# TaceoLabs/collaborative-circom

Hardware: AMD Instinct MI355X
Metric: Groth16 constraints/sec (BN254, 2^22 R1CS), one REP3 party's prove (higher is better)
Workload: dtype u32; 1 GPU; synthetic R1CS 2^22 constraints-domain BN254, REP3 co-groth16 (configs[2]); num_constraints=4194302, domain_size=4194304, nnz=12582906, msm=8 G1 + 2 G2 of ~2^22 points, ntt=12

## Files before the change

### collaborative-circom_amd/csrc/capi.hip

```cpp
#include "capi_internal.hpp"


template <int OP>
int32_t vec_binary(cg_ctx* ctx, int32_t curve, void* d_out, const void* d_a, const void* d_b, size_t n) {
    if (!ctx || !d_out || !d_a || !d_b) return fail(CG_ERR_ARG, "null argument");
    HIPCHK(hipSetDevice(ctx->device));
    return with_fr(curve, [&](auto tag) -> int {
        typedef decltype(tag) Fr;
        StatScope ss(ctx, TAG_VEC);
        return launch_vec_binary<Fr>(ctx->stream, OP, (Fr*)d_out, (const Fr*)d_a, (const Fr*)d_b, n);
    });
}

template <class F> struct CurveB;
template <> struct CurveB<Bn254Fq> { static Bn254Fq get() { Bn254Fq t = Bn254Fq::one(); return t + t + t; } };
template <> struct CurveB<Fp2<Bn254Fq>> { static Fp2<Bn254Fq> get() {
    Bn254Fq one = Bn254Fq::one(), three = one + one + one, nine = three + three + three;
    Fp2<Bn254Fq> xi = {nine, one}; Fp2<Bn254Fq> inv = fp_inverse(xi); return {inv.c0 * three, inv.c1 * three}; } };
#if CG_WITH_BLS
template <> struct CurveB<Bls381Fq> { static Bls381Fq get() { Bls381Fq t = Bls381Fq::one(); t = t + t; return t + t; } };
template <> struct CurveB<Fp2<Bls381Fq>> { static Fp2<Bls381Fq> get() { Bls381Fq f = CurveB<Bls381Fq>::get(); return {f, f}; } };
#endif

namespace {
// ... 124 lines not shown
}
int32_t cg_bases_release(cg_bases* b) {
    if (!b) return 0;
    hipSetDevice(b->device);
    hipDeviceSynchronize();
    hipFree(b->d_pts);
    if (b->d_pre) hipFree(b->d_pre);
    if (b->d_live) hipFree(b->d_live);
    if (b->compact) { hipFree(b->compact->d_pts); if (b->compact->d_pre) hipFree(b->compact->d_pre); delete b->compact; }
    delete b;
    return 0;
}
int32_t cg_bases_check_on_curve(cg_ctx* ctx, const cg_bases* b, uint64_t* n_bad, uint64_t* first_bad) {
    if (!ctx || !b || !n_bad) return fail(CG_ERR_ARG, "null argument");
    if (b->device != ctx->device) return fail(CG_ERR_ARG, "bases live on another device");
    HIPCHK(hipSetDevice(ctx->device));
    return with_group(b->curve, b->group, [&](auto ftag, auto) -> int {
        typedef decltype(ftag) F;
        unsigned long long* d = nullptr; unsigned long long h[2] = {0ull, ~0ull};
        HIPCHK(hip_malloc_flush((void**)&d, 16));
        HIPCHK(hipMemcpyAsync(d, h, 16, hipMemcpyHostToDevice, ctx->stream));
        int rc = check_on_curve_launch<F>(ctx->stream, (const Affine<F>*)b->d_pts, b->n, CurveB<F>::get(), d);
        if (rc) return rc;
        HIPCHK(hipMemcpyAsync(h, d, 16, hipMemcpyDeviceToHost, ctx->stream));
        HIPCHK(hipStreamSynchronize(ctx->stream));
        HIPCHK(hipFree(d));
        *n_bad = h[0]; if (first_bad) *first_bad = h[1];
        return 0;
    });
}
int32_t cg_bases_check_subgroup(cg_ctx* ctx, const cg_bases* b, uint64_t* n_bad, uint64_t* first_bad) {
    if (!ctx || !b || !n_bad) return fail(CG_ERR_ARG, "null argument");
    if (b->device != ctx->device) return fail(CG_ERR_ARG, "bases live on another device");
    *n_bad = 0; if (first_bad) *first_bad = ~0ull;
    if (b->curve == CG_BN254 && b->group == CG_G1) return 0;
    HIPCHK(hipSetDevice(ctx->device));
    return with_group(b->curve, b->group, [&](auto ftag, auto frtag) -> int {
        typedef decltype(ftag) F; typedef decltype(frtag) Fr;
        unsigned long long* d = nullptr; unsigned long long h[2] = {0ull, ~0ull};
        HIPCHK(hip_malloc_flush((void**)&d, 16));
        HIPCHK(hipMemcpyAsync(d, h, 16, hipMemcpyHostToDevice, ctx->stream));
        const FastSubgroup<F>* fast = fast_subgroup<F>();
        int rc = fast ? check_subgroup_fast_launch<F>(ctx->stream, (const Affine<F>*)b->d_pts, b->n, *fast, d)
                      : check_subgroup_launch<F, Fr>(ctx->stream, (const Affine<F>*)b->d_pts, b->n, d);
        if (rc) return rc;
        HIPCHK(hipMemcpyAsync(h, d, 16, hipMemcpyDeviceToHost, ctx->stream));
        HIPCHK(hipStreamSynchronize(ctx->stream));
        HIPCHK(hipFree(d));
        *n_bad = h[0]; if (first_bad) *first_bad = h[1];
        return 0;
    });
}
int32_t cg_bases_precompute(cg_ctx* ctx, cg_bases* b, int32_t c) {
    if (!ctx || !b) return fail(CG_ERR_ARG, "null argument");
    if (b->compact) return cg_bases_precompute(ctx, b->compact, c);
    const bool auto_window = c == 0;
    if (c == 0) c = b->n > ((size_t)3 << (b->group == CG_G1 ? 20 : 19)) ? 20 : (b->n <= ((size_t)1 << 18) ? 16 : 17);
    if (c < 8 || c > 22) return fail(CG_ERR_ARG, "precompute window must be 0 (auto) or in [8, 22]");
    if (b->device != ctx->device) return fail(CG_ERR_ARG, "bases live on another device");
    if (b->n > ((size_t)1 << 24)) return fail(CG_ERR_ARG, "precomputed tables support at most 2^24 points");
    HIPCHK(hipSetDevice(ctx->device));
    if (b->d_pre) { HIPCHK(hipStreamSynchronize(ctx->stream)); HIPCHK(hipFree(b->d_pre)); b->d_pre = nullptr; b->pre_c = b->pre_nwin = 0; }
    return with_group(b->curve, b->group, [&](auto ftag, auto frtag) -> int {
        typedef decltype(ftag) F; typedef decltype(frtag) Fr;
        const int nwin = Fr::Params::BITS / c + 1;
        const size_t n = std::max<size_t>(b->n, 1);
        const hipError_t e_pre = hip_malloc_flush(&b->d_pre, (size_t)nwin * n * sizeof(Affine<F>));
        if (e_pre == hipErrorOutOfMemory && auto_window) {
            (void)hipGetLastError(); b->d_pre = nullptr;
            return 0;
        }
        HIPCHK(e_pre);
        Affine<F>* tab = (Affine<F>*)b->d_pre;
        HIPCHK(hipMemcpyAsync(tab, b->d_pts, b->n * sizeof(Affine<F>), hipMemcpyDeviceToDevice, ctx->stream));
        for (int j = 1; j < nwin; j++) { int rc = precompute_window_launch<F>(ctx->stream, tab + (size_t)(j - 1) * b->n, tab + (size_t)j * b->n, b->n, c); if (rc) return rc; }
        HIPCHK(hipStreamSynchronize(ctx->stream));
        b->pre_c = c; b->pre_nwin = nwin;
        return 0;
    });
}
size_t cg_bases_len(const cg_bases* b) { return b ? b->n : 0; }

int32_t cg_bases_synth_multiples(cg_ctx* ctx, int32_t curve, int32_t group, uint64_t first, size_t n, cg_bases** out) {
    if (!ctx || !out) return fail(CG_ERR_ARG, "null argument");
    HIPCHK(hipSetDevice(ctx->device));
    return with_group(curve, group, [&](auto ftag, auto) -> int {
        typedef decltype(ftag) F;
        const uint32_t* src = curve == CG_BN254 ? (group == CG_G1 ? Bn254G1_GEN : Bn254G2_GEN) : (group == CG_G1 ? Bls381G1_GEN : Bls381G2_GEN);
        Affine<F> ga; memcpy(&ga, src, sizeof ga);
        const XYZZ<F> G = XYZZ<F>::from_affine(ga);
        int log_t = 0; while (((size_t)1 << (2 * log_t)) < n) log_t++;
        const size_t T = (size_t)1 << log_t, H = std::max<size_t>(1, (n + T - 1) >> log_t);
        std::vector<XYZZ<F>> lo(T), hi(H);
        uint32_t k[2] = {(uint32_t)first, (uint32_t)(first >> 32)};
        XYZZ<F> acc = xyzz_scalar_mul(G, k, 2);
        for (size_t j = 0; j < T; j++) { lo[j] = acc; acc = xyzz_add(acc, G); }
        uint32_t kt[2] = {(uint32_t)T, (uint32_t)((uint64_t)T >> 32)};
        const XYZZ<F> step = xyzz_scalar_mul(G, kt, 2);
        acc = XYZZ<F>::infinity();
        for (size_t j = 0; j < H; j++) { hi[j] = acc; acc = xyzz_add(acc, step); }
        XYZZ<F>*d_lo = nullptr, *d_hi = nullptr;
        HIPCHK(hip_malloc_flush((void**)&d_lo, T * sizeof(XYZZ<F>))); HIPCHK(hip_malloc_flush((void**)&d_hi, H * sizeof(XYZZ<F>)));
        HIPCHK(hipMemcpy(d_lo, lo.data(), T * sizeof(XYZZ<F>), hipMemcpyHostToDevice));
        HIPCHK(hipMemcpy(d_hi, hi.data(), H * sizeof(XYZZ<F>), hipMemcpyHostToDevice));
        cg_bases* b = new cg_bases{ctx->device, curve, group, n, sizeof(Affine<F>), nullptr};
        b->no_inf = first >= 1 && first + n > first;
        HIPCHK(hip_malloc_flush(&b->d_pts, std::max<size_t>(n * sizeof(Affine<F>), 16)));
        int rc = synth_points_launch<F>(ctx->stream, d_lo, d_hi, log_t, n, (Affine<F>*)b->d_pts);
        if (rc) return rc;
        HIPCHK(hipStreamSynchronize(ctx->stream));
        HIPCHK(hipFree(d_lo)); HIPCHK(hipFree(d_hi));
        *out = b;
        return 0;
    });
}
int32_t cg_bases_from_scalars(cg_ctx* ctx, int32_t curve, int32_t group, const void* d_scalars, size_t n, cg_bases** out) {
    if (!ctx || !out || (!d_scalars && n)) return fail(CG_ERR_ARG, "null argument");
    HIPCHK(hipSetDevice(ctx->device));
    return with_group(curve, group, [&](auto ftag, auto frtag) -> int {
        typedef decltype(ftag) F; typedef decltype(frtag) Fr;
        const uint32_t* src = curve == CG_BN254 ? (group == CG_G1 ? Bn254G1_GEN : Bn254G2_GEN) : (group == CG_G1 ? Bls381G1_GEN : Bls381G2_GEN);
        Affine<F> ga; memcpy(&ga, src, sizeof ga);
        const int nwin = (Fr::Params::BITS + 7) / 8;
        Affine<F>* d_tab = nullptr;
        HIPCHK(hip_malloc_flush((void**)&d_tab, (size_t)nwin * 255 * sizeof(Affine<F>)));
        cg_bases* b = new cg_bases{ctx->device, curve, group, n, sizeof(Affine<F>), nullptr};
        hipError_t e = hip_malloc_flush(&b->d_pts, std::max<size_t>(n * sizeof(Affine<F>), 16));
        if (e != hipSuccess) { hipFree(d_tab); delete b; return fail(CG_ERR_OOM, "cg_bases_from_scalars: out of device memory"); }
        int rc = fixed_base_mul_launch<F, Fr>(ctx->stream, ga, (const Fr*)d_scalars, n, d_tab, (Affine<F>*)b->d_pts);
        hipError_t e2 = hipStreamSynchronize(ctx->stream);
        hipFree(d_tab);
        if (rc || e2 != hipSuccess) { hipFree(b->d_pts); delete b; return rc ? rc : fail(CG_ERR_HIP, std::string("cg_bases_from_scalars: ") + hipGetErrorString(e2)); }
        *out = b;
        return 0;
    });
}
int32_t cg_bases_download(cg_ctx* ctx, const cg_bases* bases, size_t offset, size_t n, void* h_out_packed) {
    if (!ctx || !bases || !h_out_packed) return fail(CG_ERR_ARG, "null argument");
    if (offset + n > bases->n) return fail(CG_ERR_ARG, "slice out of range");
    HIPCHK(hipMemcpyAsync(h_out_packed, (const char*)bases->d_pts + offset * bases->pt_bytes, n * bases->pt_bytes, hipMemcpyDeviceToHost, ctx->stream));
    HIPCHK(hipStreamSynchronize(ctx->stream));
    return 0;
}

int32_t cg_ctx_set_option(cg_ctx* ctx, int32_t option, int64_t value) {
    if (!ctx) return fail(CG_ERR_ARG, "null ctx");
    switch (option) {
        case CG_OPT_MSM_CHUNK: return cg_msm_set_chunk(ctx, (int32_t)value);
        case CG_OPT_MSM_WINDOW: return cg_msm_set_window(ctx, (int32_t)value);
        case CG_OPT_MSM_SCATTER_CAP: return cg_msm_set_scatter_capacity(ctx, (int32_t)value);
        case CG_OPT_MSM_TABLE_ORDER: if (value < 0 || value > 2) break; ctx->table_order = (int)value; return 0;
        case CG_OPT_MSM_G2_AFTER: if (value < -1 || value > 64) break; ctx->g2_after = (int)value; return 0;
        case CG_OPT_MSM_G2_SLICES: if (value < 0 || value > 1) break; ctx->g2_slices = (int)value; return 0;
        case CG_OPT_MSM_REDUCE_BATCH: if (value < 0 || value > 3) break; ctx->red_batch = (int)value; return 0;
        case CG_OPT_MSM_ACC_SLOTS: if (value < 2 || value > cg_ctx::ACC_SLOTS_MAX) break; ctx->acc_slots = (int)value; return 0;
        case CG_OPT_MSM_WIDE_SMALL: if (value < 0 || value > 30 || (value > 1 && value < 10)) break; ctx->wide_small = (int)value; return 0;
        case CG_OPT_MSM_ONE_STREAM_LOG: if (value < 0 || value > 30) break; ctx->one_stream_log = (int)value; return 0;
        case CG_OPT_MSM_OFF_MAIN_LOG: if (value < 0 || value > 30) break; ctx->off_main_log = (int)value; return 0;
        case CG_OPT_MSM_SOLO_LOG: if (value < 0 || value > 30) break; ctx->solo_log = (int)value; return 0;
        default: return fail(CG_ERR_ARG, "cg_ctx_set_option: unknown option");
    }
    return fail(CG_ERR_ARG, "cg_ctx_set_option: value out of range");
}
int32_t cg_ctx_get_option(const cg_ctx* ctx, int32_t option, int64_t* value) {
    if (!ctx || !value) return fail(CG_ERR_ARG, "null argument");
    switch (option) {
        case CG_OPT_MSM_CHUNK: *value = ctx->msm_chunk; return 0;
        case CG_OPT_MSM_WINDOW: *value = ctx->msm_window; return 0;
        case CG_OPT_MSM_SCATTER_CAP: *value = ctx->scatter_cap; return 0;
        case CG_OPT_MSM_TABLE_ORDER: *value = ctx->table_order; return 0;
        case CG_OPT_MSM_G2_AFTER: *value = ctx->g2_after; return 0;
        case CG_OPT_MSM_G2_SLICES: *value = ctx->g2_slices; return 0;
        case CG_OPT_MSM_REDUCE_BATCH: *value = ctx->red_batch; return 0;
        case CG_OPT_MSM_ACC_SLOTS: *value = ctx->acc_slots; return 0;
        case CG_OPT_MSM_WIDE_SMALL: *value = ctx->wide_small; return 0;
        case CG_OPT_MSM_ONE_STREAM_LOG: *value = ctx->one_stream_log; return 0;
        case CG_OPT_MSM_OFF_MAIN_LOG: *value = ctx->off_main_log; return 0;
        case CG_OPT_MSM_SOLO_LOG: *value = ctx->solo_log; return 0;
        default: return fail(CG_ERR_ARG, "cg_ctx_get_option: unknown option");
    }
}
int32_t cg_set_option(int32_t option, int64_t value) {
    if (option < 1 || option >= CG_GOPT_COUNT) return fail(CG_ERR_ARG, "cg_set_option: unknown option");
    if (value < 0 || (option != CG_GOPT_COMPACT_MIN_LOG && value > 1) || value > 64) return fail(CG_ERR_ARG, "cg_set_option: value out of range");
    g_options.v[option].store(value); return 0;
}
int32_t cg_get_option(int32_t option, int64_t* value) {
    if (option < 1 || option >= CG_GOPT_COUNT || !value) return fail(CG_ERR_ARG, "cg_get_option: unknown option");
    *value = g_options.v[option].load(); return 0;
}
int32_t cg_vec_add_dev(cg_ctx* ctx, int32_t curve, void* o, const void* a, const void* b, size_t n) { return vec_binary<0>(ctx, curve, o, a, b, n); }
int32_t cg_vec_sub_dev(cg_ctx* ctx, int32_t curve, void* o, const void* a, const void* b, size_t n) { return vec_binary<1>(ctx, curve, o, a, b, n); }
int32_t cg_vec_mul_dev(cg_ctx* ctx, int32_t curve, void* o, const void* a, const void* b, size_t n) { return vec_binary<2>(ctx, curve, o, a, b, n); }

int32_t cg_vec_rep3_mul_local_dev(cg_ctx* ctx, int32_t curve, void* d_out, const void* d_aa, const void* d_ab, const void* d_ba, const void* d_bb, const void* d_mask, size_t n) {
    if (!ctx || !d_out || !d_aa || !d_ab || !d_ba || !d_bb) return fail(CG_ERR_ARG, "null argument");
    HIPCHK(hipSetDevice(ctx->device));
    return with_fr(curve, [&](auto tag) -> int {
        typedef decltype(tag) Fr;
        StatScope ss(ctx, TAG_VEC);
        return launch_rep3_mul_local<Fr>(ctx->stream, (Fr*)d_out, (const Fr*)d_aa, (const Fr*)d_ab, (const Fr*)d_ba, (const Fr*)d_bb, (const Fr*)d_mask, n);
    });
}
static int rand_draw_begin(cg_ctx* ctx, int32_t curve, const uint8_t* seed32, uint64_t word_pos, size_t n, void* d_out, double margin, int* slot_out) {
    int slot = -1;
    for (int i = 0; i < cg_ctx::RAND_DRAWS; i++) if (!ctx->rand_draw[i].live) { slot = i; break; }
    if (slot < 0) return fail(CG_ERR_ARG, "cg_chacha12_fr_rand_dev_begin: too many draws in flight (finish one first)");
    if (!ctx->rand_result) HIPCHK(hipHostMalloc((void**)&ctx->rand_result, sizeof(unsigned long long) * 2 * cg_ctx::RAND_DRAWS, hipHostMallocDefault));
    cg_ctx::RandDraw& d = ctx->rand_draw[slot];
    if (!d.ev) HIPCHK(hipEventCreateWithFlags(&d.ev, hipEventDisableTiming));
    return with_fr(curve, [&](auto tag) -> int {
        typedef decltype(tag) Fr;
        typedef typename Fr::Params P;
        StatScope ss(ctx, TAG_VEC);
        uint32_t key[8];
        for (int i = 0; i < 8; i++) key[i] = (uint32_t)seed32[4 * i] | (uint32_t)seed32[4 * i + 1] << 8 | (uint32_t)seed32[4 * i + 2] << 16 | (uint32_t)seed32[4 * i + 3] << 24;
        const double accept = (double)P::P[7] / (double)(1ull << (P::BITS - 224));
        const uint64_t n_cand = (uint64_t)(((double)n + margin) / accept) + 2;
        const uint64_t n_pairs = n_cand / 2 + 2;
        const uint64_t tiles = (n_pairs + 255) / 256;
        d.d_cand = d.d_small = nullptr;
        if (int rc = cg_dev_alloc(ctx, n_pairs * 64, &d.d_cand)) return rc;
        if (int rc = cg_dev_alloc(ctx, tiles * 4 + 16, &d.d_small)) { cg_dev_free(ctx, d.d_cand); return rc; }
        unsigned long long* h = ctx->rand_result + 2 * slot; h[0] = h[1] = 0;
        int rc = chacha12_fr_rand_launch(ctx->stream, key, P::P, P::BITS, word_pos, n_pairs, n, d.d_cand, (uint32_t*)((char*)d.d_small + 16), (unsigned long long*)d.d_small, d_out);
        hipError_t e = rc ? hipSuccess : hipMemcpyAsync(h, d.d_small, 2 * sizeof(unsigned long long), hipMemcpyDeviceToHost, ctx->stream);
        if (!rc && e == hipSuccess) e = hipEventRecord(d.ev, ctx->stream);
        if (rc || e != hipSuccess) { hipStreamSynchronize(ctx->stream); cg_dev_free(ctx, d.d_cand); cg_dev_free(ctx, d.d_small); if (rc) return rc; HIPCHK(e); }
        d.live = true; d.word_pos = word_pos; d.n = n;
        *slot_out = slot;
        return 0;
    });
}
static int rand_draw_finish(cg_ctx* ctx, int slot, bool* enough, uint64_t* word_pos_after) {
    cg_ctx::RandDraw& d = ctx->rand_draw[slot];
    hipError_t e = hipEventSynchronize(d.ev);
    { void* two[2] = {d.d_cand, d.d_small}; cg_dev_free_many(ctx, two, 2); }
    d.live = false;
    HIPCHK(e);
    const unsigned long long* h = ctx->rand_result + 2 * slot;
    *enough = h[0] >= d.n;
    if (*enough && word_pos_after) *word_pos_after = d.word_pos + 8 * ((uint64_t)h[1] + 1);
    return 0;
}
static int rand_draw_args(cg_ctx* ctx, const uint8_t* seed32, uint64_t word_pos, size_t n, void* d_out, const char* who) {
    if (!ctx || !seed32 || (n && !d_out)) return fail(CG_ERR_ARG, "null argument");
    if (n >= ((size_t)1 << 31) || word_pos > (~0ull >> 1)) return fail(CG_ERR_ARG, std::string(who) + ": size or position out of range");
    return 0;
}
int32_t cg_chacha12_fr_rand_dev(cg_ctx* ctx, int32_t curve, const uint8_t* seed32, uint64_t word_pos, size_t n, void* d_out, uint64_t* word_pos_after) {
    if (int rc = rand_draw_args(ctx, seed32, word_pos, n, d_out, "cg_chacha12_fr_rand_dev")) return rc;
    if (n == 0) { if (word_pos_after) *word_pos_after = word_pos; return 0; }
    HIPCHK(hipSetDevice(ctx->device));
    double margin = 8.0 * std::sqrt((double)n) + 64.0;
    for (int attempt = 0; attempt < 4; attempt++, margin *= 4.0) {
        int slot = -1; bool enough = false;
        if (int rc = rand_draw_begin(ctx, curve, seed32, word_pos, n, d_out, margin, &slot)) return rc;
        if (int rc = rand_draw_finish(ctx, slot, &enough, word_pos_after)) return rc;
        if (enough) return 0;
    }
    return fail(CG_ERR_HIP, "cg_chacha12_fr_rand_dev: too few accepted candidates");
}
int32_t cg_chacha12_fr_rand_dev_begin(cg_ctx* ctx, int32_t curve, const uint8_t* seed32, uint64_t word_pos, size_t n, void* d_out, int32_t* ticket) {
    if (!ticket) return fail(CG_ERR_ARG, "null argument");
    if (int rc = rand_draw_args(ctx, seed32, word_pos, n, d_out, "cg_chacha12_fr_rand_dev_begin")) return rc;
    if (n == 0) return fail(CG_ERR_ARG, "cg_chacha12_fr_rand_dev_begin: nothing to draw");
    HIPCHK(hipSetDevice(ctx->device));
    int slot = -1;
    if (int rc = rand_draw_begin(ctx, curve, seed32, word_pos, n, d_out, 12.0 * std::sqrt((double)n) + 64.0, &slot)) return rc;
    *ticket = slot;
    return 0;
}
int32_t cg_chacha12_fr_rand_dev_finish(cg_ctx* ctx, int32_t ticket, uint64_t* word_pos_after) {
    if (!ctx) return fail(CG_ERR_ARG, "null argument");
    if (ticket < 0 || ticket >= cg_ctx::RAND_DRAWS || !ctx->rand_draw[ticket].live) return fail(CG_ERR_ARG, "cg_chacha12_fr_rand_dev_finish: no such draw in flight");
    HIPCHK(hipSetDevice(ctx->device));
    bool enough = false;
    if (int rc = rand_draw_finish(ctx, ticket, &enough, word_pos_after)) return rc;
    if (!enough) return fail(CG_ERR_HIP, "cg_chacha12_fr_rand_dev_finish: too few accepted candidates (d_out is incomplete: draw again with cg_chacha12_fr_rand_dev)");
    return 0;
}
int32_t cg_vec_check_canonical_dev(cg_ctx* ctx, int32_t curve, const void* d_vec, size_t n, void* d_count) {
    if (!ctx || !d_vec || !d_count) return fail(CG_ERR_ARG, "null argument");
    HIPCHK(hipSetDevice(ctx->device));
    return with_fr(curve, [&](auto tag) -> int {
        typedef decltype(tag) Fr;
        StatScope ss(ctx, TAG_VEC);
        return launch_vec_count_noncanonical<Fr>(ctx->stream, (const Fr*)d_vec, n, (unsigned long long*)d_count);
    });
}
int32_t cg_vec_affine_dev(cg_ctx* ctx, int32_t curve, void* d_out, const void* d_a, size_t n, const void* h_c, const void* h_d) {
    if (!ctx || !d_out || !d_a || !h_c) return fail(CG_ERR_ARG, "null argument");
    HIPCHK(hipSetDevice(ctx->device));
    return with_fr(curve, [&](auto tag) -> int {
        typedef decltype(tag) Fr;
        Fr c, d = Fr::zero(); copy_in(c, h_c); if (h_d) copy_in(d, h_d);
        StatScope ss(ctx, TAG_VEC);
        return launch_vec_affine<Fr>(ctx->stream, (Fr*)d_out, (const Fr*)d_a, n, c, d);
    });
}
int32_t cg_vec_fill_dev(cg_ctx* ctx, int32_t curve, void* d_v, size_t n, const void* h_value) {
    if (!ctx || !d_v || !h_value) return fail(CG_ERR_ARG, "null argument");
    HIPCHK(hipSetDevice(ctx->device));
    return with_fr(curve, [&](auto tag) -> int {
        typedef decltype(tag) Fr;
        Fr v; copy_in(v, h_value);
        StatScope ss(ctx, TAG_VEC);
// ... 570 lines not shown
```

### collaborative-circom_amd/csrc/capi_msm.hip

```cpp
#include "capi_internal.hpp"

namespace {
int auto_window(size_t n, int bits) {
    const int lg = log2_floor(std::max<size_t>(n, 1));
    int c = lg <= 12 ? 8 : lg == 13 ? 13 : lg <= 18 ? 15 : 16;
    auto ok = [&](int w) { const int t = bits % w; return t != 0 && t >= w - 3 - (w >= 13 ? 6 : 0); };
    if (!ok(c)) for (int d : {1, -1, 2, -2, 3, -3}) { if (c + d >= 3 && c + d <= 17 && ok(c + d)) { c += d; break; } }
    return c;
}

template <class F>
Jacobian<F> msm_fold_windows(const XYZZ<F>* w, int nwin, int c) {
    XYZZ<F> acc = w[nwin - 1];
    for (int i = nwin - 2; i >= 0; i--) {
        for (int d = 0; d < c; d++) acc = xyzz_dbl(acc);
        acc = xyzz_add(acc, w[i]);
    }
    return xyzz_to_jacobian(acc);
}

int ticket_slot(cg_ctx* ctx) {
    for (size_t i = 0; i < ctx->tickets.size(); i++) if (!ctx->tickets[i].live) return (int)i;
    ctx->tickets.emplace_back();
    return (int)ctx->tickets.size() - 1;
// ... 10 lines not shown
int msm_begin_multi_impl_(cg_ctx* ctx, int nb, const cg_bases* const* bases, const size_t* offsets, size_t n, const void* const* d_scalars, int k, int* tickets_out, bool force_exact) {
    const uint32_t chunk_request = ctx ? ctx->msm_chunk : 0;
    if (!ctx || !bases || !tickets_out || (n && !d_scalars)) return fail(CG_ERR_ARG, "null argument");
    if (nb < 1 || nb > 16) return fail(CG_ERR_ARG, "number of base tables out of range");
    if (k < 1 || k > 8) return fail(CG_ERR_ARG, "k out of range");
    for (int b = 0; b < nb; b++) {
        if (!bases[b]) return fail(CG_ERR_ARG, "null bases");
        if ((offsets ? offsets[b] : 0) + n > bases[b]->n) return fail(CG_ERR_ARG, "bases slice out of range");
        if (bases[b]->device != ctx->device) return fail(CG_ERR_ARG, "bases live on another device");
        if (bases[b]->curve != bases[0]->curve) return fail(CG_ERR_ARG, "all tables of one call must be on the same curve");
    }
    HIPCHK(hipSetDevice(ctx->device));
    {
        bool any = false;
        for (int b = 0; b < nb; b++) any = any || bases[b]->compact != nullptr;
        if (any) {
            struct Grp { uint64_t sig; size_t off, cnt, caller_off; std::vector<int> members; };
            std::vector<Grp> groups;
            std::vector<size_t> off_c(nb), cnt_c(nb);
            for (int b = 0; b < nb; b++) {
                const size_t off = offsets ? offsets[b] : 0;
                uint64_t sig = 0; size_t o = off, cn = n;
                if (bases[b]->compact) {
                    const auto& lv = bases[b]->h_live;
                    o = (size_t)(std::lower_bound(lv.begin(), lv.end(), (uint32_t)off) - lv.begin());
                    cn = (size_t)(std::lower_bound(lv.begin(), lv.end(), (uint32_t)std::min<size_t>(off + n, 0xffffffffu)) - lv.begin()) - o;
                    sig = bases[b]->live_sig;
                }
                off_c[b] = o; cnt_c[b] = cn;
                bool placed = false;
                for (auto& g : groups) {
                    if (g.sig != sig || g.cnt != cn) continue;
                    if (sig != 0) {
                        if (g.off != o || g.caller_off != off) continue;
                        const auto& la = bases[g.members[0]]->h_live; const auto& lb = bases[b]->h_live;
                        if (memcmp(la.data() + o, lb.data() + o, cn * sizeof(uint32_t)) != 0) continue;
                    }
                    g.members.push_back(b); placed = true; break;
                }
                if (!placed) groups.push_back(Grp{sig, o, cn, off, {b}});
            }
            size_t need = 0;
            for (auto& g : groups) if (g.sig) need += align_up((size_t)k * g.cnt * 32);
            if (need > ctx->gather_cap) {
                HIPCHK(hipStreamSynchronize(ctx->stream)); HIPCHK(hipStreamSynchronize(ctx->sortst));
                if (ctx->gather_buf) HIPCHK(hipFree(ctx->gather_buf));
                ctx->gather_buf = nullptr; ctx->gather_cap = 0;
                HIPCHK(hip_malloc_flush(&ctx->gather_buf, need)); ctx->gather_cap = need;
            }
            if (ctx->sorts_unordered) { for (int j = 0; j < 2; j++) HIPCHK(hipStreamWaitEvent(ctx->stream, ctx->ev_sorted[j], 0)); ctx->sorts_unordered = false; }
            size_t used = 0;
            for (auto& g : groups) {
                std::vector<const cg_bases*> gb; std::vector<size_t> go; std::vector<const void*> gs(k);
                const int first = g.members[0];
                for (int m : g.members) { gb.push_back(bases[m]->compact ? bases[m]->compact : bases[m]); go.push_back(bases[m]->compact ? off_c[m] : (offsets ? offsets[m] : 0)); }
                if (g.sig) {
                    const size_t off = offsets ? offsets[first] : 0;
                    for (int j = 0; j < k; j++) {
                        void* dst = (char*)ctx->gather_buf + used + (size_t)j * g.cnt * 32;
                        int rc = with_fr(bases[first]->curve, [&](auto tag) -> int {
                            typedef decltype(tag) Fr;
                            return launch_vec_gather_idx<Fr>(ctx->stream, (Fr*)dst, (const Fr*)d_scalars[j], bases[first]->d_live + g.off, g.cnt, (uint32_t)off);
                        });
                        if (rc) return rc;
                        gs[j] = dst;
                    }
                    used += align_up((size_t)k * g.cnt * 32);
                } else for (int j = 0; j < k; j++) gs[j] = d_scalars[j];
                std::vector<int> tk(g.members.size());
                int rc = msm_begin_multi_impl(ctx, (int)g.members.size(), gb.data(), go.data(), g.cnt, gs.data(), k, tk.data(), true);
                if (rc) return rc;
                for (size_t i = 0; i < g.members.size(); i++) tickets_out[g.members[i]] = tk[i];
            }
            return 0;
        }
    }
    {
        bool mixed = false;
        for (int b = 1; b < nb; b++) mixed = mixed || bases[b]->pre_c != bases[0]->pre_c;
        if (mixed) {
            std::vector<char> done(nb, 0);
            for (int b = 0; b < nb; b++) {
                if (done[b]) continue;
                std::vector<const cg_bases*> gb; std::vector<size_t> go; std::vector<int> idx;
                for (int m = b; m < nb; m++) if (!done[m] && bases[m]->pre_c == bases[b]->pre_c) { gb.push_back(bases[m]); go.push_back(offsets ? offsets[m] : 0); idx.push_back(m); done[m] = 1; }
                std::vector<int> tk(idx.size());
                int rc = msm_begin_multi_impl(ctx, (int)idx.size(), gb.data(), go.data(), n, d_scalars, k, tk.data(), force_exact);
                if (rc) return rc;
                for (size_t i = 0; i < idx.size(); i++) tickets_out[idx[i]] = tk[i];
            }
            return 0;
        }
    }
    const int curve = bases[0]->curve;
    const bool shared = bases[0]->pre_c != 0;
    if (shared && n > ((size_t)1 << 24)) return fail(CG_ERR_ARG, "precomputed-table MSM supports at most 2^24 points per call");
    int bits = 0;
    { int rc = with_fr(curve, [&](auto tag) -> int { bits = decltype(tag)::Params::BITS; return 0; }); if (rc) return rc; }
    const int c = shared ? bases[0]->pre_c : (n ? (ctx->msm_window ? ctx->msm_window : auto_window(n, bits)) : 2);
    const int nwin = bits / c + 1;
    if (shared && nwin != bases[0]->pre_nwin) return fail(CG_ERR_ARG, "internal: window count mismatch");
    if ((uint64_t)nwin * n >= ((uint64_t)1 << 32))
        return fail(CG_ERR_ARG, "MSM of more than 2^32 / windows points in one call (about 2^27): pass the table in slices and add the partial sums");
    uint32_t cap = 0;
    if (n && !force_exact && ctx->scatter_cap >= 0) {
        if (ctx->scatter_cap > 0) cap = (uint32_t)ctx->scatter_cap;
        else {
            const int t = bits % c;
            const double nbk = (double)((size_t)1 << (c - 1));
            const double top = t == 0 ? (double)n : (double)n / (double)((size_t)1 << std::min(c - 1, t));
            const double avg = shared ? (double)(nwin - 1) * (double)n / nbk + top : std::max((double)n / nbk, top);
            const double want = 1.25 * avg + 6.0 * std::sqrt(avg) + 16.0;
            if (want <= 4096.0) { cap = 16; while ((double)cap < want) cap <<= 1; }
        }
    }
    const MsmGeom geom = msm_geom(std::max<size_t>(n, 1), c, nwin, shared, 0, chunk_request);
    const int nsums = geom.ngroups;
    std::vector<int> slots(nb);
    size_t acc_bytes = 0;
    for (int b = 0; b < nb; b++) {
        slots[b] = ticket_slot(ctx);
        MsmTicket& t = ctx->tickets[slots[b]];
        t.live = true;
        t.curve = curve; t.group = bases[b]->group; t.k = k; t.c = c; t.nwin = nwin; t.nsums = nsums; t.plain_fold = shared && !geom.bitsum && !geom.grid; t.bit_fold = geom.bitsum;
        t.grid_fold = geom.grid; t.log_l = geom.log_l; t.log_h = geom.log_h; t.gc = geom.gc; t.gr = geom.gr;
        t.optimistic = cap != 0; t.bases = bases[b]; t.offset = offsets ? offsets[b] : 0; t.n = n; t.scalars.assign(d_scalars, d_scalars + (n ? k : 0));
        if (!t.h_flags) HIPCHK(hipHostMalloc((void**)&t.h_flags, 8 * sizeof(uint32_t), hipHostMallocDefault));
        for (int i = 0; i < 8; i++) t.h_flags[i] = 0;
        int rc = with_coord_field(curve, t.group, [&](auto ftag) -> int {
            typedef decltype(ftag) F;
            const size_t need = (size_t)k * nsums * sizeof(XYZZ<F>);
            if (t.pinned_bytes < need) {
                if (t.h_pinned) HIPCHK(hipHostFree(t.h_pinned));
                t.h_pinned = nullptr; t.pinned_bytes = 0;
                HIPCHK(hipHostMalloc(&t.h_pinned, need, hipHostMallocDefault));
                t.pinned_bytes = need;
            }
            if (n == 0) { XYZZ<F>* h = (XYZZ<F>*)t.h_pinned; for (int i = 0; i < k * nsums; i++) h[i] = XYZZ<F>::infinity(); }
            else acc_bytes = std::max(acc_bytes, msm_acc_scratch_bytes<F>(n, c, nwin, shared, chunk_request));
            return 0;
        });
        if (rc) return rc;
        if (!t.done) HIPCHK(hipEventCreateWithFlags(&t.done, hipEventDisableTiming));
    }
    if (n) {
        StatScope ss(ctx, TAG_MSM);
        const size_t sort_bytes = align_up(cap ? msm_sort_direct_scratch_bytes(n, c, nwin, shared ? 1 : 0, cap) : msm_sort_scratch_bytes(n, c, nwin));
        const size_t acc_slot = align_up(acc_bytes);
        const int nsched = k > 1 ? 2 : 1;
        const int acc_slots_min = std::min((int)cg_ctx::ACC_SLOTS_MAX, std::max(2, ctx->acc_slots));
        const int red_batch = ctx->red_batch;
        const uint64_t wide_max = ctx->wide_small == 0 ? 0 : (uint64_t)1 << (ctx->wide_small == 1 ? 20 : ctx->wide_small);
        const bool small_call = k <= 2 && (uint64_t)nwin * n <= wide_max;
        bool single_field = true;
        for (int b = 1; b < nb; b++) single_field = single_field && bases[b]->group == bases[0]->group;
        const int acc_slots = red_batch || small_call ? std::min((int)cg_ctx::ACC_SLOTS_MAX, std::max(acc_slots_min, red_batch >= 2 || small_call ? nb * k : nb + 1)) : acc_slots_min;
        const bool wide = k <= 2 && nb * k <= std::min(acc_slots, (int)ACC_MAX_SETS) && (uint64_t)nwin * n <= wide_max;
        const bool solo = wide && small_call && single_field && ctx->solo_log > 0 && (uint64_t)nwin * n <= ((uint64_t)1 << ctx->solo_log);
        const bool one_stream = solo || (small_call && ctx->one_stream_log > 0 && (uint64_t)nwin * n <= ((uint64_t)1 << ctx->one_stream_log));
        const hipStream_t sortst = one_stream ? ctx->stream : ctx->sortst, auxst = one_stream ? ctx->stream : ctx->aux;
        { int rc = solo ? ensure_main_stream_block(ctx, ctx->solo_arena, nsched * sort_bytes + (size_t)acc_slots * acc_slot) : ensure_arena(ctx, nsched * sort_bytes + (size_t)acc_slots * acc_slot); if (rc) return rc; }
        char* const arena_base = solo ? ctx->solo_arena.base : ctx->arena.base;
        char* acc_scratch = arena_base + nsched * sort_bytes;
        if (!solo) {
        HIPCHK(hipEventRecord(ctx->ev_in, ctx->stream));
        HIPCHK(hipStreamWaitEvent(sortst, ctx->ev_in, 0));
        for (int rs = 0; rs < 2; rs++) for (int i = 0; i < 2; i++) if (ctx->merged_pending[rs][i]) { HIPCHK(hipStreamWaitEvent(sortst, ctx->ev_merged[rs][i], 0)); ctx->merged_pending[rs][i] = false; }
        }
        std::vector<MsmSortPtrs> sps(k);
        auto launch_sort = [&](int j) -> int {
            const int ss_ = j % nsched;
            if (j < 4 && ctx->comp_after[j]) HIPCHK(hipStreamWaitEvent(sortst, ctx->comp_after[j], 0));
            if (j >= nsched && !solo) {
                HIPCHK(hipStreamWaitEvent(sortst, ctx->ev_sched_free[ss_], 0));
                for (int rs = 0; rs < 2; rs++) if (ctx->merged_pending[rs][ss_]) HIPCHK(hipStreamWaitEvent(sortst, ctx->ev_merged[rs][ss_], 0));
            }
            hipEvent_t evs[2]; hipEvent_t* pev = nullptr;
            if (ctx->stats_on) { const int i0 = ev_open(ctx, TAG_SORT); evs[0] = ctx->ev_live[i0].a; evs[1] = ctx->ev_live[i0].b; pev = evs; }
            char* sort_scratch = arena_base + (size_t)ss_ * sort_bytes;
            int rc = with_fr(curve, [&](auto tag) -> int {
                typedef decltype(tag) Fr;
                return cap ? msm_sort_direct_launch<Fr>(sortst, (const Fr*)d_scalars[j], n, c, nwin, shared ? 1 : 0, cap, sort_scratch, sort_bytes, &sps[j], pev)
                           : msm_sort_launch<Fr>(sortst, (const Fr*)d_scalars[j], n, c, nwin, shared ? 1 : 0, sort_scratch, sort_bytes, &sps[j], pev);
            });
            if (rc) return rc;
            if (cap) for (int b = 0; b < nb; b++) HIPCHK(hipMemcpyAsync(ctx->tickets[slots[b]].h_flags + j, sps[j].overflow, 4, hipMemcpyDeviceToHost, sortst));
            if (!solo) HIPCHK(hipEventRecord(ctx->ev_sorted[ss_], sortst));
            return 0;
        };
        int iter = 0;
        { int rc = launch_sort(0); if (rc) return rc; }
        struct PendSet { MsmRedSet set; int slot, sched, table, comp; };
        std::vector<PendSet> pend[2];
        int tables_of_group[2] = {0, 0};
        for (int b = 0; b < nb; b++) tables_of_group[bases[b]->group == CG_G1 ? 0 : 1]++;
        std::vector<int> comps_left(nb, k);
        hipStream_t red_stream[2] = {auxst, auxst};
        hipStream_t acc_stream[2] = {ctx->stream, ctx->stream};
        hipEvent_t last_acc[2] = {nullptr, nullptr};
        auto flush = [&](int gi) -> int {
            std::vector<PendSet>& pd = pend[gi];
            if (pd.empty()) return 0;
            hipStream_t rst = red_stream[gi];
            hipEvent_t ea = ctx->ev_acc[pd.back().slot];
            if (!solo) {
                HIPCHK(hipEventRecord(ea, acc_stream[gi]));
                if (rst != acc_stream[gi]) HIPCHK(hipStreamWaitEvent(rst, ea, 0));
                last_acc[gi] = ea;
            }
            hipEvent_t evs[2]; hipEvent_t* pev = nullptr;
            if (ctx->stats_on) { const int i2 = ev_open(ctx, TAG_REDUCE); evs[0] = ctx->ev_live[i2].a; evs[1] = ctx->ev_live[i2].b; pev = evs; }
            hipEvent_t evm[2]; int nm = 0; bool seen[2] = {false, false};
            std::vector<MsmRedSet> sets;
            const int rs = rst == sortst ? 1 : 0;
            for (const PendSet& ps : pd) { sets.push_back(ps.set); if (!solo && !seen[ps.sched]) { seen[ps.sched] = true; evm[nm++] = ctx->ev_merged[rs][ps.sched]; } }
            int rc = with_coord_field(curve, gi == 0 ? CG_G1 : CG_G2, [&](auto ftag) -> int {
                typedef decltype(ftag) F;
                return msm_reduce_batch<F>(rst, sets.data(), (int)sets.size(), n, c, nwin, shared, sps[pd[0].comp].cap, evm, nm, pev, chunk_request);
            });
            if (rc) return rc;
            if (!solo) for (const PendSet& ps : pd) {
                HIPCHK(hipEventRecord(ctx->ev_red[ps.slot], rst));
                ctx->slot_busy[ps.slot] = true; ctx->aux_pending = true; ctx->last_slot = ps.slot; ctx->merged_pending[rs][ps.sched] = true;
            }
            for (const PendSet& ps : pd) if (--comps_left[ps.table] == 0) HIPCHK(hipEventRecord(ctx->tickets[slots[ps.table]].done, rst));
            pd.clear();
            return 0;
        };
        auto acc_set = [&](int b, int j, char* scratch) -> MsmAccSet {
            const char* pts = (const char*)(shared ? bases[b]->d_pre : bases[b]->d_pts) + (offsets ? offsets[b] : 0) * bases[b]->pt_bytes;
            return MsmAccSet{pts, shared ? bases[b]->n : 0, sps[j].sorted, sps[j].offsets, sps[j].counts, scratch, !bases[b]->no_inf};
        };
        auto red_set = [&](int b, int j, char* scratch) -> MsmRedSet {
            const MsmTicket& t = ctx->tickets[slots[b]];
            const size_t pinned_stride = (size_t)(t.group == CG_G1 ? 4 : 8) * (bases[b]->pt_bytes / (t.group == CG_G1 ? 2 : 4));
            return MsmRedSet{scratch, sps[j].offsets, sps[j].counts, (char*)t.h_pinned + (size_t)j * nsums * pinned_stride};
        };
        const bool off_main = wide && !one_stream && ctx->off_main_log > 0 && (uint64_t)nwin * n <= ((uint64_t)1 << ctx->off_main_log);
        if (wide) {
            if (k == 2) { int rc = launch_sort(1); if (rc) return rc; }
            if (off_main) { acc_stream[0] = sortst; acc_stream[1] = auxst; }
            if (!solo) for (int j = 0; j < k; j++) HIPCHK(hipStreamWaitEvent(acc_stream[1], ctx->ev_sorted[j], 0));
            red_stream[0] = sortst;
            for (int gi : {1, 0}) {
                std::vector<MsmAccSet> sets;
                for (int j = 0; j < k; j++) for (int b = 0; b < nb; b++) {
                    if ((bases[b]->group == CG_G1 ? 0 : 1) != gi) continue;
                    const int slot = iter++ % acc_slots;
                    if (!solo && ctx->slot_busy[slot]) HIPCHK(hipStreamWaitEvent(acc_stream[gi], ctx->ev_red[slot], 0));
                    char* scratch = acc_scratch + (size_t)slot * acc_slot;
                    sets.push_back(acc_set(b, j, scratch));
                    pend[gi].push_back(PendSet{red_set(b, j, scratch), slot, j, b, j});
                }
                if (sets.empty()) continue;
                hipEvent_t evs[2]; hipEvent_t* pev = nullptr;
                if (ctx->stats_on) { const int i1 = ev_open(ctx, gi == 0 ? TAG_ACC_G1 : TAG_ACC_G2); evs[0] = ctx->ev_live[i1].a; evs[1] = ctx->ev_live[i1].b; pev = evs; }
                int rc = with_coord_field(curve, gi == 0 ? CG_G1 : CG_G2, [&](auto ftag) -> int {
                    typedef decltype(ftag) F;
                    return msm_accumulate_batch<F>(acc_stream[gi], sets.data(), (int)sets.size(), n, c, nwin, shared, sps[0].cap, pev, chunk_request, false);
                });
                if (rc) return rc;
                if (gi == 0 && !solo) HIPCHK(hipStreamWaitEvent(sortst, ctx->ev_sorted[k - 1], 0));
                { int rc2 = flush(gi); if (rc2) return rc2; }
            }
            if (off_main && last_acc[1]) HIPCHK(hipStreamWaitEvent(sortst, last_acc[1], 0));
            if (off_main) ctx->sorts_unordered = true;
            if (!solo) for (int j = 0; j < k; j++) HIPCHK(hipEventRecord(ctx->ev_sched_free[j], off_main ? sortst : ctx->stream));
        }
        auto do_acc = [&](int b, int j) -> int {
            const MsmSortPtrs& sp = sps[j];
            MsmTicket& t = ctx->tickets[slots[b]];
            const int gi = t.group == CG_G1 ? 0 : 1;
            hipEvent_t evs[2]; hipEvent_t* pev = nullptr;
            if (ctx->stats_on) { const int i1 = ev_open(ctx, t.group == CG_G1 ? TAG_ACC_G1 : TAG_ACC_G2); evs[0] = ctx->ev_live[i1].a; evs[1] = ctx->ev_live[i1].b; pev = evs; }
            const int slot = iter++ % acc_slots;
            for (int g2 = 0; g2 < 2; g2++) {
                bool held = false;
                for (const PendSet& ps : pend[g2]) held = held || ps.slot == slot;
                if (held) { int rc = flush(g2); if (rc) return rc; }
            }
            if (ctx->slot_busy[slot]) HIPCHK(hipStreamWaitEvent(ctx->stream, ctx->ev_red[slot], 0));
            char* scratch = acc_scratch + (size_t)slot * acc_slot;
            const MsmAccSet as = acc_set(b, j, scratch);
            int rc = with_coord_field(curve, t.group, [&](auto ftag) -> int {
                typedef decltype(ftag) F;
                return msm_accumulate_batch<F>(ctx->stream, &as, 1, n, c, nwin, shared, sp.cap, pev, chunk_request, ctx->g2_slices != 0);
            });
            if (rc) return rc;
            pend[gi].push_back(PendSet{red_set(b, j, scratch), slot, j % nsched, b, j});
            return 0;
        };
        if (wide) {}
        else if (k <= 2 && ctx->table_order == 2) {
            if (k == 2) { int rc = launch_sort(1); if (rc) return rc; }
            std::vector<std::pair<int, int>> g1o, g2o, order;
            for (int j = 0; j < k; j++) for (int bi = 0; bi < nb; bi++) {
                const int b = (j & 1) ? nb - 1 - bi : bi;
                (bases[b]->group == CG_G1 ? g1o : g2o).push_back({b, j});
            }
            const size_t at = ctx->g2_after < 0 ? g1o.size() : std::min<size_t>((size_t)ctx->g2_after, g1o.size());
            order.insert(order.end(), g1o.begin(), g1o.begin() + at); order.insert(order.end(), g2o.begin(), g2o.end()); order.insert(order.end(), g1o.begin() + at, g1o.end());
            bool waited[2] = {false, false};
            int left[2] = {(int)g1o.size(), (int)g2o.size()}, left_sched[2] = {0, 0};
            for (auto& pr : order) left_sched[pr.second]++;
            for (size_t i = 0; i < order.size(); i++) {
                const int b = order[i].first, j = order[i].second, gi = bases[b]->group == CG_G1 ? 0 : 1;
                if (!waited[j]) { HIPCHK(hipStreamWaitEvent(ctx->stream, ctx->ev_sorted[j], 0)); waited[j] = true; }
                { int rc = do_acc(b, j); if (rc) return rc; }
                const bool last_of_field = --left[gi] == 0;
                const bool comp_changes = i + 1 == order.size() || order[i + 1].second != j || (bases[order[i + 1].first]->group == CG_G1 ? 0 : 1) != gi;
                if (red_batch == 0 || (red_batch == 1 && comp_changes) || (last_of_field && red_batch != 3) || (int)pend[gi].size() == RED_MAX_SETS) { int rc3 = flush(gi); if (rc3) return rc3; }
                if (--left_sched[j] == 0) HIPCHK(hipEventRecord(ctx->ev_sched_free[j], ctx->stream));
            }
        } else
        for (int j = 0; j < k; j++) {
            HIPCHK(hipStreamWaitEvent(ctx->stream, ctx->ev_sorted[j % nsched], 0));
            if (j + 1 < k && nsched == 2 && j + 1 < nsched) { int rc = launch_sort(j + 1); if (rc) return rc; }
            int left_in_comp[2] = {tables_of_group[0], tables_of_group[1]};
            for (int bi = 0; bi < nb; bi++) {
                const int b = (ctx->table_order >= 1 && (j & 1)) ? nb - 1 - bi : bi;
                const int gi = bases[b]->group == CG_G1 ? 0 : 1;
                { int rc = do_acc(b, j); if (rc) return rc; }
                const bool last_here = --left_in_comp[gi] == 0;
                if (red_batch == 0 || (red_batch == 1 && last_here) || (last_here && j == k - 1 && red_batch != 3) || (int)pend[gi].size() == RED_MAX_SETS) { int rc3 = flush(gi); if (rc3) return rc3; }
            }
            HIPCHK(hipEventRecord(ctx->ev_sched_free[j % nsched], ctx->stream));
            if (j + 2 < k && nsched == 2) {
                for (int g2 = 0; g2 < 2; g2++) { int rc = flush(g2); if (rc) return rc; }
                int rc = launch_sort(j + 2); if (rc) return rc;
            }
        }
        for (int g2 = 0; g2 < 2; g2++) { int rc = flush(g2); if (rc) return rc; }
    }
    for (int b = 0; b < nb; b++) { if (n == 0) HIPCHK(hipEventRecord(ctx->tickets[slots[b]].done, ctx->stream)); tickets_out[b] = slots[b]; }
    return 0;
}

int msm_begin_impl(cg_ctx* ctx, const cg_bases* bases, size_t offset, size_t n, const void* const* d_scalars, int k, int* ticket_out) {
    if (!ticket_out) return fail(CG_ERR_ARG, "null argument");
    return msm_begin_multi_impl(ctx, 1, &bases, &offset, n, d_scalars, k, ticket_out);
}

int msm_end_impl(cg_ctx* ctx, int ticket, void* h_out);
int msm_end_impl(cg_ctx* ctx, int ticket, void* h_out) {
    if (!ctx || !h_out) return fail(CG_ERR_ARG, "null argument");
    if (ticket < 0 || ticket >= (int)ctx->tickets.size() || !ctx->tickets[ticket].live) return fail(CG_ERR_ARG, "bad MSM ticket");
    MsmTicket& t = ctx->tickets[ticket];
    HIPCHK(hipEventSynchronize(t.done));
    t.live = false;
    if (t.optimistic) {
        bool over = false;
        for (int j = 0; j < t.k; j++) over = over || t.h_flags[j] != 0;
        if (over) {
            const cg_bases* b = t.bases; const size_t off = t.offset, n = t.n; const int k = t.k;
            std::vector<const void*> sc = t.scalars;
            int t2 = -1;
            int rc = msm_begin_multi_impl(ctx, 1, &b, &off, n, sc.data(), k, &t2, true);
            if (rc) return rc;
            return msm_end_impl(ctx, t2, h_out);
        }
    }
    return with_group64(t.curve, t.group, [&](auto ftag, auto) -> int {
        typedef decltype(ftag) F;
        typedef cg64::Xyzz<F> X;
        const X* h = (const X*)t.h_pinned;
        cg64::Jac<F>* out = (cg64::Jac<F>*)h_out;
        for (int j = 0; j < t.k; j++) {
            const X* hs = h + (size_t)j * t.nsums;
            X acc;
            if (t.grid_fold) {
                std::vector<X> U((size_t)t.log_l + t.log_h + 1, X::inf());
                size_t at = 0;
                for (int kk = 0; kk <= t.log_l; kk++) for (uint32_t g = 0; g < t.gc; g++) U[kk] = cg64::add(U[kk], hs[at++]);
                for (int kk = 0; kk < t.log_h; kk++) for (uint32_t g = 0; g < t.gr; g++) U[t.log_l + kk] = cg64::add(U[t.log_l + kk], hs[at++]);
                acc = U.back();
                for (size_t i = U.size() - 1; i-- > 0;) acc = cg64::add(cg64::dbl(acc), U[i]);
            } else if (t.bit_fold) {
                acc = hs[t.nsums - 1];
                for (int i = t.nsums - 2; i >= 0; i--) acc = cg64::add(cg64::dbl(acc), hs[i]);
            } else if (t.plain_fold) { acc = hs[0]; for (int i = 1; i < t.nsums; i++) acc = cg64::add(acc, hs[i]); }
            else {
                acc = hs[t.nsums - 1];
                for (int i = t.nsums - 2; i >= 0; i--) { for (int d = 0; d < t.c; d++) acc = cg64::dbl(acc); acc = cg64::add(acc, hs[i]); }
            }
            const cg64::Jac<F> r = cg64::to_jac(acc);
            memcpy(out + j, &r, sizeof r);
        }
        return 0;
    });
}

}

extern "C" {
int32_t cg_msm_set_scatter_capacity(cg_ctx* ctx, int32_t cap) {
    if (!ctx) return fail(CG_ERR_ARG, "null ctx");
    if (cap > 65536) return fail(CG_ERR_ARG, "capacity out of range");
    ctx->scatter_cap = cap;
    return 0;
}
int32_t cg_msm_set_chunk(cg_ctx* ctx, int32_t entries_per_lane) {
    if (!ctx) return fail(CG_ERR_ARG, "null ctx");
    if (entries_per_lane < 0 || entries_per_lane > 4096) return fail(CG_ERR_ARG, "chunk length out of range");
    ctx->msm_chunk = (uint32_t)entries_per_lane;
    return 0;
}
int32_t cg_msm_set_window(cg_ctx* ctx, int32_t c) {
    if (!ctx) return fail(CG_ERR_ARG, "null ctx");
    if (c != 0 && (c < 2 || c > 20)) return fail(CG_ERR_ARG, "window size must be 0 (auto) or in [2, 20]");
    ctx->msm_window = c;
    return 0;
}
int32_t cg_msm_scalars_after(cg_ctx* ctx, int32_t component, cg_ctx* owner, int32_t copy_ticket) {
    if (!ctx || !owner || component < 0 || component >= 4) return fail(CG_ERR_ARG, "bad argument");
    if (copy_ticket < 0 || !owner->copy_ev[copy_ticket % cg_ctx::COPY_TICKETS]) return fail(CG_ERR_ARG, "bad copy ticket");
    const int slot = copy_ticket % cg_ctx::COPY_TICKETS;
    ctx->comp_after[component] = owner->copy_id[slot] == (uint32_t)copy_ticket ? owner->copy_ev[slot] : nullptr;
    return 0;
}
int32_t cg_msm_dev_begin(cg_ctx* ctx, const cg_bases* bases, size_t offset, size_t n, const void* const* d_scalars, int32_t k, int32_t* ticket) {
    const int rc = msm_begin_impl(ctx, bases, offset, n, d_scalars, k, ticket);
    if (ctx) for (hipEvent_t& e : ctx->comp_after) e = nullptr;
    return rc;
}
int32_t cg_msm_dev_begin_multi(cg_ctx* ctx, int32_t n_tables, const cg_bases* const* bases, const size_t* offsets, size_t n,
                               const void* const* d_scalars, int32_t k, int32_t* tickets) {
    const int rc = msm_begin_multi_impl(ctx, n_tables, bases, offsets, n, d_scalars, k, tickets);
    if (ctx) for (hipEvent_t& e : ctx->comp_after) e = nullptr;
    return rc;
}
int32_t cg_msm_end(cg_ctx* ctx, int32_t ticket, void* h_out_jacobian) { return msm_end_impl(ctx, ticket, h_out_jacobian); }
int32_t cg_msm_dev(cg_ctx* ctx, const cg_bases* bases, size_t offset, size_t n, const void* const* d_scalars, int32_t k, void* h_out) {
    int32_t t = -1;
    int rc = msm_begin_impl(ctx, bases, offset, n, d_scalars, k, &t);
    if (rc) return rc;
    return msm_end_impl(ctx, t, h_out);
}
int32_t cg_msm(cg_ctx* ctx, const cg_bases* bases, size_t offset, size_t n, const void* const* h_scalars, int32_t k, void* h_out) {
    if (!ctx || !bases || !h_scalars) return fail(CG_ERR_ARG, "null argument");
    if (k < 1 || k > 8) return fail(CG_ERR_ARG, "k out of range");
    HIPCHK(hipSetDevice(ctx->device));
    std::vector<void*> d(k, nullptr);
    const size_t bytes = std::max<size_t>(n * 32, 16);
    for (int j = 0; j < k; j++) {
        HIPCHK(hip_malloc_flush(&d[j], bytes));
        if (n) HIPCHK(hipMemcpyAsync(d[j], h_scalars[j], n * 32, hipMemcpyHostToDevice, ctx->stream));
    }
    int rc = cg_msm_dev(ctx, bases, offset, n, (const void* const*)d.data(), k, h_out);
    hipStreamSynchronize(ctx->stream);
    for (int j = 0; j < k; j++) hipFree(d[j]);
    return rc;
}

int32_t cg_msm_schedule_dev(cg_ctx* ctx, int32_t curve, const void* d_scalars, size_t n, int32_t c, int32_t shared, int32_t path, uint32_t cap,
                            uint32_t* h_counts, uint32_t* h_offsets, uint32_t* h_sorted, int32_t* path_taken, uint32_t* overflow) {
    if (!ctx || !d_scalars || !h_counts || !h_offsets || !h_sorted || !path_taken || !overflow) return fail(CG_ERR_ARG, "null argument");
    if (c < 2 || c > 22) return fail(CG_ERR_ARG, "cg_msm_schedule_dev: window size out of range (2 .. 22)");
    if (n == 0) return fail(CG_ERR_ARG, "cg_msm_schedule_dev: no scalars");
    if (shared < 0 || shared > 1 || path < 0 || path > CG_MSM_PATH_DIRECT) return fail(CG_ERR_ARG, "cg_msm_schedule_dev: shared is 0 or 1, path 0 .. 4");
    int bits = 0;
    { int rc = with_fr(curve, [&](auto tag) -> int { bits = decltype(tag)::Params::BITS; return 0; }); if (rc) return rc; }
    const int nwin = bits / c + 1;
    if (shared && n > ((size_t)1 << 24)) return fail(CG_ERR_ARG, "cg_msm_schedule_dev: one bucket set takes at most 2^24 points (the window shares the entry with the index)");
    if ((uint64_t)nwin * n >= ((uint64_t)1 << 32)) return fail(CG_ERR_ARG, "cg_msm_schedule_dev: schedule positions are 32-bit");
    const bool direct = path == CG_MSM_PATH_DIRECT;
    const size_t nbuckets = (size_t)(shared ? 1 : nwin) << (c - 1);
    if (direct && (cap < 1 || (uint64_t)nbuckets * cap >= ((uint64_t)1 << 32))) return fail(CG_ERR_ARG, "cg_msm_schedule_dev: the one-pass scatter takes 1 <= cap < 2^32 / buckets");
    const size_t sorted_len = direct ? nbuckets * cap : (size_t)nwin * n;
    const size_t bytes = align_up(direct ? msm_sort_direct_scratch_bytes(n, c, nwin, shared, cap) : msm_sort_scratch_bytes(n, c, nwin));
    HIPCHK(hipSetDevice(ctx->device));
    char* scratch = nullptr;
    HIPCHK(hip_malloc_flush(&scratch, bytes));
    MsmSortPtrs sp{};
    uint32_t ov = 0;
    int rc = [&]() -> int {
        HIPCHK(hipMemsetAsync(scratch, 0xFF, bytes, ctx->stream));
        int r = with_fr(curve, [&](auto tag) -> int {
// ... 21 lines not shown
```

### collaborative-circom_amd/csrc/capi_streams.hip

```cpp
#include "capi_internal.hpp"

extern "C" {
namespace {
std::mutex g_stream_pool_mu;
constexpr int HWQ = 4;
struct StreamClassPool { std::vector<std::pair<hipStream_t, int>> idle; int created = 0; int out[HWQ] = {0, 0, 0, 0}; };
std::map<std::pair<int, int>, StreamClassPool> g_stream_pool;
std::map<hipStream_t, int> g_stream_slot;
thread_local int g_group_depth = 0;
thread_local std::map<int, std::array<uint8_t, 3>> g_group_used_by_device;
#define g_group_used (g_group_used_by_device[device])
int new_stream(int cls, hipStream_t* out) {
    if (cls == 0) { HIPCHK(hipStreamCreateWithFlags(out, hipStreamNonBlocking)); return 0; }
    int prio_least = 0, prio_greatest = 0;
    HIPCHK(hipDeviceGetStreamPriorityRange(&prio_least, &prio_greatest));
    HIPCHK(hipStreamCreateWithPriority(out, hipStreamNonBlocking, cls > 0 ? prio_greatest : prio_least));
    return 0;
}
int measured_pipe(int device, int cls, hipStream_t st);
thread_local int g_group_rot = 0;
}
}
int pooled_stream(int device, int cls, hipStream_t* out, int want) {
    std::lock_guard<std::mutex> l(g_stream_pool_mu);
// ... 33 lines not shown
        }
        hipStream_t st = nullptr;
        if (int rc = new_stream(cls, &st)) return rc;
        const int model = p.created++ % HWQ, seen = measured_pipe(device, cls, st);
        const int slot = seen >= 0 ? seen : model;
        g_stream_slot[st] = slot; p.idle.push_back({st, slot});
    }
    return fail(CG_ERR_HIP, "internal: stream pool");
}
namespace {
void park_stream(int device, int cls, hipStream_t st) {
    if (!st) return;
    std::lock_guard<std::mutex> l(g_stream_pool_mu);
    StreamClassPool& p = g_stream_pool[{device, cls}];
    auto it = g_stream_slot.find(st);
    if (it == g_stream_slot.end()) { hipStreamDestroy(st); return; }
    if (p.out[it->second] > 0) p.out[it->second]--;
    if (p.idle.size() < 32) p.idle.push_back({st, it->second}); else { g_stream_slot.erase(it); hipStreamDestroy(st); }
}
}
int make_copy_streams(cg_ctx* c, int want_h2d, int want_d2h) {
    { int rc = pooled_stream(c->device, c->prio_copy, &c->h2d, want_h2d); if (rc) return rc; }
    { int rc = pooled_stream(c->device, c->prio_copy, &c->d2h, want_d2h); if (rc) return rc; }
    HIPCHK(hipEventCreateWithFlags(&c->ev_copy_order, hipEventDisableTiming));
    return 0;
}
extern "C" {

__global__ void k_probe_spin(unsigned long long ticks) { const unsigned long long t0 = wall_clock64(); while (wall_clock64() - t0 < ticks) { } }
namespace {
unsigned long long probe_ticks() {
    static std::atomic<unsigned long long> cached[64] = {};
    int dev = 0; if (hipGetDevice(&dev) != hipSuccess || dev < 0 || dev >= 64) { (void)hipGetLastError(); return 12000ull; }
    unsigned long long t = cached[dev].load(std::memory_order_relaxed);
    if (!t) {
        int khz = 0;
        if (hipDeviceGetAttribute(&khz, hipDeviceAttributeWallClockRate, dev) != hipSuccess || khz <= 0) { (void)hipGetLastError(); khz = 100000; }
        t = (unsigned long long)khz * 120ull / 1000ull;
        cached[dev].store(t, std::memory_order_relaxed);
    }
    return t;
}
bool streams_share_queue(hipStream_t a, hipStream_t b) {
    if (!a || !b || a == b) return false;
    double best = 1e9;
    for (int rep = 0; rep < 2 && best > 190.0; rep++) {
        if (hipStreamSynchronize(a) != hipSuccess || hipStreamSynchronize(b) != hipSuccess) { (void)hipGetLastError(); return false; }
        const auto t0 = std::chrono::steady_clock::now();
        hipLaunchKernelGGL(k_probe_spin, dim3(1), dim3(64), 0, a, probe_ticks());
        hipLaunchKernelGGL(k_probe_spin, dim3(1), dim3(64), 0, b, probe_ticks());
        if (hipStreamSynchronize(a) != hipSuccess || hipStreamSynchronize(b) != hipSuccess) { (void)hipGetLastError(); return false; }
        best = std::min(best, std::chrono::duration<double, std::micro>(std::chrono::steady_clock::now() - t0).count());
    }
    return best > 190.0 && best < 420.0;
}
struct PipeRefs { hipStream_t low[HWQ] = {nullptr, nullptr, nullptr, nullptr}, high[HWQ] = {nullptr, nullptr, nullptr, nullptr}; bool ok = false; int attempts = 0; };
std::map<int, PipeRefs> g_pipe_refs;
std::mutex g_pipe_mu;
double spin_pair_us(hipStream_t a, hipStream_t b) {
    double best = 1e9;
    for (int rep = 0; rep < 3; rep++) {
        if (hipStreamSynchronize(a) != hipSuccess || hipStreamSynchronize(b) != hipSuccess) { (void)hipGetLastError(); return -1.0; }
        const auto t0 = std::chrono::steady_clock::now();
        hipLaunchKernelGGL(k_probe_spin, dim3(1), dim3(64), 0, a, probe_ticks());
        hipLaunchKernelGGL(k_probe_spin, dim3(1), dim3(64), 0, b, probe_ticks());
        if (hipStreamSynchronize(a) != hipSuccess || hipStreamSynchronize(b) != hipSuccess) { (void)hipGetLastError(); return -1.0; }
        best = std::min(best, std::chrono::duration<double, std::micro>(std::chrono::steady_clock::now() - t0).count());
    }
    return best;
}
int coupled_reference(const hipStream_t* refs, hipStream_t st) {
    int found = -1;
    for (int i = 0; i < HWQ; i++) {
        const double us = spin_pair_us(refs[i], st);
        if (us < 0 || us > 420.0) return -1;
        if (us >= 152.0) { if (found >= 0) return -1; found = i; }
    }
    return found;
}
int measured_pipe(int device, int cls, hipStream_t st) {
    static const bool off = tune_env("CG_NO_PIPE_MAP") != nullptr || tune_env("CG_NO_STREAM_PROBE") != nullptr;
    if (off || !global_option(CG_GOPT_STREAM_PROBES) || cls < -1 || cls > 1) return -1;
    std::lock_guard<std::mutex> l(g_pipe_mu);
    PipeRefs& r = g_pipe_refs[device];
    if (!r.ok && r.attempts < 3) {
        r.attempts++;
        for (hipStream_t& x : r.low) if (x) { hipStreamDestroy(x); x = nullptr; }
        for (hipStream_t& x : r.high) if (x) { hipStreamDestroy(x); x = nullptr; }
        bool ok = true;
        for (int i = 0; i < HWQ && ok; i++) ok = new_stream(-1, &r.low[i]) == 0;
        for (int i = 0; i < HWQ && ok; i++) ok = new_stream(1, &r.high[i]) == 0;
        for (int i = 0; i < HWQ && ok; i++) for (int j = i + 1; j < HWQ && ok; j++) {
            const double a = spin_pair_us(r.low[i], r.low[j]), b = spin_pair_us(r.high[i], r.high[j]);
            ok = a > 0 && a < 152.0 && b > 0 && b < 152.0;
        }
        hipStream_t matched[HWQ] = {nullptr, nullptr, nullptr, nullptr};
        for (int j = 0; j < HWQ && ok; j++) {
            const int pipe = coupled_reference(r.low, r.high[j]);
            ok = pipe >= 0 && !matched[pipe];
            if (ok) matched[pipe] = r.high[j];
        }
        if (ok) for (int i = 0; i < HWQ; i++) r.high[i] = matched[i];
        r.ok = ok;
        if (getenv("CG_DEBUG_STREAMS")) fprintf(stderr, "pipe map of device %d: %s\n", device, ok ? "references in place" : "not available (the pool keeps its creation-order model)");
    }
    if (!r.ok) return -1;
    int pipe = coupled_reference(cls == -1 ? r.high : r.low, st);
    if (pipe < 0) pipe = coupled_reference(cls == -1 ? r.high : r.low, st);
    return pipe;
}
thread_local std::vector<hipStream_t> g_group_busy[3];
int separate_stream(int device, int cls, hipStream_t* moving, std::vector<hipStream_t> fixed) {
    static const bool off = tune_env("CG_NO_STREAM_PROBE") != nullptr;
    if (off || !global_option(CG_GOPT_STREAM_PROBES)) return 0;
    std::vector<hipStream_t> rejected;
    for (int tries = 0; tries < 6; tries++) {
        bool clash = false;
        for (hipStream_t f : fixed) clash = clash || streams_share_queue(f, *moving);
        if (!clash) break;
        if (getenv("CG_DEBUG_STREAMS")) fprintf(stderr, "stream probe: class %d stream shares a hardware queue with another stream of its context: replaced (try %d)\n", cls, tries);
        rejected.push_back(*moving);
        hipStream_t st = nullptr;
        if (int rc = pooled_stream(device, cls, &st)) { for (hipStream_t r : rejected) park_stream(device, cls, r); return rc; }
        *moving = st;
    }
    for (hipStream_t r : rejected) park_stream(device, cls, r);
    return 0;
}
}

int32_t cg_stream_group_begin(void) {
    static std::atomic<int> groups{0};
    if (g_group_depth++ == 0) { g_group_used_by_device.clear(); for (auto& v : g_group_busy) v.clear(); g_group_rot = groups.fetch_add(1) % HWQ; }
    return 0;
}
int32_t cg_stream_group_end(void) { if (g_group_depth > 0) g_group_depth--; return 0; }
int32_t cg_ctx_create(int32_t device, cg_ctx** out) { return cg_ctx_create_ex(device, 0, out); }
int32_t cg_ctx_create_ex(int32_t device, uint32_t flags, cg_ctx** out) {
    if (!out) return fail(CG_ERR_ARG, "null out");
    int count = 0;
    if (hipGetDeviceCount(&count) != hipSuccess || count == 0)
        return fail(CG_ERR_NODEVICE, "no HIP device visible: this backend has no CPU fallback");
    if (device < 0 || device >= count) return fail(CG_ERR_ARG, "device index out of range");
    HIPCHK(hipSetDevice(device));
    {
        int ws = 0; HIPCHK(hipDeviceGetAttribute(&ws, hipDeviceAttributeWarpSize, device));
        if (ws != 64) return fail(CG_ERR_NODEVICE, "device " + std::to_string(device) + " has " + std::to_string(ws) + "-lane wavefronts: this backend is written for wave64 (gfx950)");
    }
    cg_ctx* c = new cg_ctx();
    c->device = device;
    {
        auto seed = [](const char* name, int lo, int hi, int& field) { if (const char* e = tune_env(name)) { const int v = atoi(e); if (v >= lo && v <= hi) field = v; } };
        seed("CG_MSM_TABLE_ORDER", 0, 2, c->table_order); seed("CG_MSM_G2_AFTER", -1, 64, c->g2_after); seed("CG_MSM_G2_SLICES", 0, 1, c->g2_slices);
        seed("CG_MSM_REDUCE_BATCH", 0, 3, c->red_batch); seed("CG_MSM_ACC_SLOTS", 2, cg_ctx::ACC_SLOTS_MAX, c->acc_slots); seed("CG_MSM_WIDE_SMALL", 0, 30, c->wide_small); seed("CG_MSM_ONE_STREAM_LOG", 0, 30, c->one_stream_log); seed("CG_MSM_OFF_MAIN_LOG", 0, 30, c->off_main_log); seed("CG_MSM_SOLO_LOG", 0, 30, c->solo_log);
    }
    if (flags & 1u) { c->prio_main = 1; c->prio_copy = 1; c->prio_side = 0; }
    else if (flags & 2u) { static const int bulk_cls = tune_env("CG_BULK_CLASS") ? atoi(tune_env("CG_BULK_CLASS")) : -1; c->prio_main = bulk_cls; c->prio_side = 0; }
    const bool piped = g_group_depth > 0;
    auto pipe = [&](int k) { return piped ? (k + g_group_rot) % HWQ : -1; };
    const int w_main = (flags & 1u) ? pipe(0) : (flags & 2u) ? pipe(1) : pipe(0), w_aux = (flags & 1u) ? pipe(1) : (flags & 2u) ? pipe(3) : pipe(1), w_sort = (flags & 1u) ? pipe(0) : pipe(2);
    const int w_join = (flags & 1u) ? pipe(3) : (flags & 2u) ? pipe(2) : pipe(3);
    { int rc = pooled_stream(device, c->prio_main, &c->stream, w_main); if (rc) return rc; }
    if (flags & 1u) { int rc = make_copy_streams(c, pipe(3), pipe(2)); if (rc) return rc; }
    { int rc = pooled_stream(device, c->prio_side, &c->aux, w_aux); if (rc) return rc; }
    { int rc = pooled_stream(device, c->prio_side, &c->sortst, w_sort); if (rc) return rc; }
    { int rc = pooled_stream(device, -1, &c->joinst, w_join); if (rc) return rc; }
    {
        static std::mutex probe_mu;
        std::lock_guard<std::mutex> probing(probe_mu);
        const bool grp = g_group_depth > 0;
        auto others = [&](int cls, std::initializer_list<hipStream_t> own) {
            std::vector<hipStream_t> v;
            for (hipStream_t o : own) if (o) v.push_back(o);
            if (grp && cls >= -1 && cls <= 1) for (hipStream_t o : g_group_busy[cls + 1]) if (v.size() < (size_t)HWQ - 1) v.push_back(o);
            return v;
        };
        auto placed = [&](int cls, hipStream_t st) { if (grp && cls >= -1 && cls <= 1) g_group_busy[cls + 1].push_back(st); };
        if (int rc = separate_stream(device, c->prio_main, &c->stream, others(c->prio_main, {}))) return rc;
        placed(c->prio_main, c->stream);
        if (int rc = separate_stream(device, c->prio_side, &c->aux, others(c->prio_side, {c->prio_side == c->prio_main ? c->stream : nullptr}))) return rc;
        placed(c->prio_side, c->aux);
        if (int rc = separate_stream(device, c->prio_side, &c->sortst, others(c->prio_side, {c->aux, c->prio_side == c->prio_main ? c->stream : nullptr}))) return rc;
        placed(c->prio_side, c->sortst);
        if (c->h2d) {
            if (int rc = separate_stream(device, c->prio_copy, &c->h2d, others(c->prio_copy, {c->prio_copy == c->prio_main ? c->stream : nullptr}))) return rc;
            placed(c->prio_copy, c->h2d);
            if (int rc = separate_stream(device, c->prio_copy, &c->d2h, others(c->prio_copy, {c->h2d, c->prio_copy == c->prio_main ? c->stream : nullptr}))) return rc;
            placed(c->prio_copy, c->d2h);
        }
        if (int rc = separate_stream(device, -1, &c->joinst, others(-1, {c->prio_main == -1 ? c->stream : nullptr}))) return rc;
        placed(-1, c->joinst);
    }
    for (hipEvent_t& e : c->park_ev) HIPCHK(hipEventCreateWithFlags(&e, hipEventDisableTiming));
    HIPCHK(hipEventCreateWithFlags(&c->ev_in, hipEventDisableTiming));
    for (int i = 0; i < 2; i++) { HIPCHK(hipEventCreateWithFlags(&c->ev_sorted[i], hipEventDisableTiming)); HIPCHK(hipEventCreateWithFlags(&c->ev_sched_free[i], hipEventDisableTiming)); for (int rs = 0; rs < 2; rs++) HIPCHK(hipEventCreateWithFlags(&c->ev_merged[rs][i], hipEventDisableTiming)); }
    for (int i = 0; i < cg_ctx::ACC_SLOTS_MAX; i++) { HIPCHK(hipEventCreateWithFlags(&c->ev_acc[i], hipEventDisableTiming)); HIPCHK(hipEventCreateWithFlags(&c->ev_red[i], hipEventDisableTiming)); }
    *out = c;
    return 0;
}
int32_t cg_ctx_destroy(cg_ctx* ctx) {
    if (!ctx) return 0;
    hipSetDevice(ctx->device);
    hipStreamSynchronize(ctx->stream);
    hipStreamSynchronize(ctx->aux);
    hipStreamSynchronize(ctx->sortst);
    for (int i = 0; i < cg_ctx::ACC_SLOTS_MAX; i++) { hipEventDestroy(ctx->ev_acc[i]); hipEventDestroy(ctx->ev_red[i]); }
    for (hipEvent_t e : ctx->mark_ev) if (e) hipEventDestroy(e);
    for (auto& d : ctx->rand_draw) { if (d.live) { cg_dev_free(ctx, d.d_cand); cg_dev_free(ctx, d.d_small); d.live = false; } if (d.ev) hipEventDestroy(d.ev); }
    if (ctx->rand_result) hipHostFree(ctx->rand_result);
    for (int i = 0; i < 2; i++) { hipEventDestroy(ctx->ev_sorted[i]); hipEventDestroy(ctx->ev_sched_free[i]); for (int rs = 0; rs < 2; rs++) hipEventDestroy(ctx->ev_merged[rs][i]); }
    hipEventDestroy(ctx->ev_in);
    if (ctx->h2d) {
        hipStreamSynchronize(ctx->h2d); hipStreamSynchronize(ctx->d2h);
        for (hipEvent_t e : ctx->copy_ev) if (e) hipEventDestroy(e);
        if (ctx->ev_peer) hipEventDestroy(ctx->ev_peer);
        hipEventDestroy(ctx->ev_copy_order);
        park_stream(ctx->device, ctx->prio_copy, ctx->h2d); park_stream(ctx->device, ctx->prio_copy, ctx->d2h);
    }
    park_stream(ctx->device, ctx->prio_side, ctx->aux);
    park_stream(ctx->device, ctx->prio_side, ctx->sortst);
    if (ctx->joinst) { hipStreamSynchronize(ctx->joinst); for (hipEvent_t e : ctx->park_ev) if (e) hipEventDestroy(e); park_stream(ctx->device, -1, ctx->joinst); }
    for (auto& kv : ctx->twiddles) shared_twiddles_release(ctx->device, kv.first);
    for (auto& kv : ctx->cosets) { hipFree(kv.second.lo); hipFree(kv.second.hi); }
    for (auto& t : ctx->tickets) { if (t.h_pinned) hipHostFree(t.h_pinned); if (t.h_flags) hipHostFree(t.h_flags); if (t.done) hipEventDestroy(t.done); }
    if (ctx->arena.base) hipFree(ctx->arena.base);
    if (ctx->ntt_arena.base) hipFree(ctx->ntt_arena.base);
    if (ctx->solo_arena.base) hipFree(ctx->solo_arena.base);
    for (void* p : ctx->retired) hipFree(p);
    if (ctx->gather_buf) hipFree(ctx->gather_buf);
    for (auto& p : ctx->ev_live) { if (p.a) hipEventDestroy(p.a); if (p.b) hipEventDestroy(p.b); }
    for (auto& p : ctx->ev_free) { if (p.a) hipEventDestroy(p.a); if (p.b) hipEventDestroy(p.b); }
    if (ctx->owns_stream) park_stream(ctx->device, ctx->prio_main, ctx->stream);
    delete ctx;
    return 0;
}
int32_t cg_ctx_sync(cg_ctx* ctx) {
    if (!ctx) return fail(CG_ERR_ARG, "null ctx");
    HIPCHK(hipStreamSynchronize(ctx->sortst)); HIPCHK(hipStreamSynchronize(ctx->stream)); HIPCHK(hipStreamSynchronize(ctx->aux));
    if (ctx->h2d) { HIPCHK(hipStreamSynchronize(ctx->h2d)); HIPCHK(hipStreamSynchronize(ctx->d2h)); }
    return 0;
}
void* cg_ctx_stream(cg_ctx* ctx) { return ctx ? (void*)ctx->stream : nullptr; }
int32_t cg_ctx_set_stream(cg_ctx* ctx, void* hip_stream) {
    if (!ctx) return fail(CG_ERR_ARG, "null ctx");
    HIPCHK(hipStreamSynchronize(ctx->sortst));
    HIPCHK(hipStreamSynchronize(ctx->stream));
    HIPCHK(hipStreamSynchronize(ctx->aux));
    if (ctx->owns_stream) park_stream(ctx->device, ctx->prio_main, ctx->stream);
    ctx->stream = (hipStream_t)hip_stream;
    ctx->owns_stream = false;
    return 0;
}

}
```

### collaborative-circom_amd/csrc/fr_impl.hpp

```cpp
#pragma once
#include "launchers.hpp"
#include "ntt_kernels.hpp"
#include "vec_kernels.hpp"
#include "plonk_kernels.hpp"
#include "r1cs_kernels.hpp"
#include "plonk_setup_kernels.hpp"
#include "msm_sort_kernels.hpp"

namespace cg {

template <class Fr> int launch_vec_binary(hipStream_t st, int op, Fr* out, const Fr* a, const Fr* b, size_t n) {
    if (!n) return 0;
    if (op == 0) hipLaunchKernelGGL((k_vec_binary<Fr, 0>), dim3(grid_for(n)), dim3(256), 0, st, out, a, b, n);
    else if (op == 1) hipLaunchKernelGGL((k_vec_binary<Fr, 1>), dim3(grid_for(n)), dim3(256), 0, st, out, a, b, n);
    else hipLaunchKernelGGL((k_vec_binary<Fr, 2>), dim3(grid_for(n)), dim3(256), 0, st, out, a, b, n);
    HIPCHK(hipGetLastError());
    return 0;
}
template <class Fr> int launch_rep3_mul_local(hipStream_t st, Fr* out, const Fr* aa, const Fr* ab, const Fr* ba, const Fr* bb, const Fr* mask, size_t n) {
    if (!n) return 0;
    hipLaunchKernelGGL((k_rep3_mul_local<Fr>), dim3(grid_for(n)), dim3(256), 0, st, out, aa, ab, ba, bb, mask, n);
    HIPCHK(hipGetLastError());
    return 0;
}
// ... 46 lines not shown
    HIPCHK(hipGetLastError());
    return 0;
}
template <class Fr> int launch_plonk_additions(hipStream_t st, const uint32_t* order, size_t n, const uint32_t* ids, const Fr* coeffs, const Fr* pub, uint32_t n_inputs, int pc,
                                               Fr* ext_a, Fr* ext_b, size_t n_priv) {
    if (!n) return 0;
    hipLaunchKernelGGL((k_plonk_additions<Fr>), dim3(grid_for(n)), dim3(256), 0, st, order, n, ids, coeffs, pub, n_inputs, pc, ext_a, ext_b, n_priv);
    HIPCHK(hipGetLastError());
    return 0;
}
#define CG_PLONK_LAUNCH(NAME, KERNEL, ARGS)                                                                                  \
    template <class Fr> int NAME(hipStream_t st, const ARGS<Fr>& g, size_t n) {                                             \
        if (!n) return 0;                                                                                                   \
        hipLaunchKernelGGL((KERNEL<Fr>), dim3(grid_for(n)), dim3(256), 0, st, g, n);                                         \
        HIPCHK(hipGetLastError());                                                                                          \
        return 0;                                                                                                           \
    }
CG_PLONK_LAUNCH(launch_plonk_r2_factors, k_plonk_r2_factors, PlonkR2Args)
CG_PLONK_LAUNCH(launch_plonk_r3_blind, k_plonk_r3_blind, PlonkBlindArgs)
CG_PLONK_LAUNCH(launch_plonk_r3_perm, k_plonk_r3_perm, PlonkPermArgs)
CG_PLONK_LAUNCH(launch_plonk_r3_gate, k_plonk_r3_gate, PlonkGateArgs)
CG_PLONK_LAUNCH(launch_plonk_mul4_tail, k_plonk_mul4_tail, PlonkMul4Args)
CG_PLONK_LAUNCH(launch_plonk_r3_t, k_plonk_r3_t, PlonkTArgs)
CG_PLONK_LAUNCH(launch_plonk_r3_divide, k_plonk_r3_divide, PlonkDivArgs)
#undef CG_PLONK_LAUNCH
template <class Fr, int OP> int launch_prefix_op(hipStream_t st, Fr* out, const Fr* in, size_t n, Fr* scratch) {
    const size_t tile = (size_t)256 * SCAN_ITEMS, ntiles = (n + tile - 1) / tile;
    hipLaunchKernelGGL((k_prefix_tiles<Fr, OP>), dim3((unsigned)ntiles), dim3(256), 0, st, out, in, n, scratch);
    if (ntiles > 1) {
        hipLaunchKernelGGL((k_prefix_totals<Fr, OP>), dim3(1), dim3(256), 0, st, scratch, ntiles);
        hipLaunchKernelGGL((k_prefix_fixup<Fr, OP>), dim3(grid_for(n)), dim3(256), 0, st, out, n, scratch);
    }
    HIPCHK(hipGetLastError());
    return 0;
}
template <class Fr> int launch_prefix_scan(hipStream_t st, int op, Fr* out, const Fr* in, size_t n, Fr* scratch) {
    if (!n) return 0;
    return op == 0 ? launch_prefix_op<Fr, 0>(st, out, in, n, scratch) : launch_prefix_op<Fr, 1>(st, out, in, n, scratch);
}
template <class Fr> int launch_vec_inverse(hipStream_t st, Fr* out, const Fr* in, size_t n) {
    if (!n) return 0;
    const size_t lanes = (n + INV_ITEMS - 1) / INV_ITEMS;
    hipLaunchKernelGGL((k_vec_inverse<Fr>), dim3((unsigned)((lanes + 127) / 128)), dim3(128), 0, st, out, in, n);
    HIPCHK(hipGetLastError());
    return 0;
}
template <class Fr> int launch_spmv_csr(hipStream_t st, const uint32_t* row_ptr, const uint32_t* col, const Fr* coeff, size_t n_rows, const Fr* pub,
                                        uint32_t n_inputs, int party, const Fr* wit_a, const Fr* wit_b, Fr* out_a, Fr* out_b) {
    if (!n_rows) return 0;
    if (n_rows <= ((size_t)1 << 13)) hipLaunchKernelGGL((k_spmv_csr_wave<Fr>), dim3(grid_for(n_rows * 64)), dim3(256), 0, st, row_ptr, col, coeff, n_rows, pub, n_inputs, party, wit_a, wit_b, out_a, out_b);
    else hipLaunchKernelGGL((k_spmv_csr<Fr>), dim3(grid_for(n_rows)), dim3(256), 0, st, row_ptr, col, coeff, n_rows, pub, n_inputs, party, wit_a, wit_b, out_a, out_b);
    HIPCHK(hipGetLastError());
    return 0;
}
template <class Fr> int launch_r1cs_check(hipStream_t st, const R1csMat& A, const R1csMat& B, const R1csMat& C, size_t n_rows, size_t nnz_total, int form, const Fr* w,
                                          unsigned long long* result) {
    static const unsigned long long init[2] = {0ull, ~0ull};
    HIPCHK(hipMemcpyAsync(result, init, sizeof init, hipMemcpyHostToDevice, st));
    if (!n_rows) return 0;
    const bool wave = form == 2 || (form == 0 && (n_rows <= ((size_t)1 << 13) || nnz_total / n_rows >= 96));
    if (wave) hipLaunchKernelGGL((k_r1cs_check_wave<Fr>), dim3(grid_for(n_rows * 64)), dim3(256), 0, st, A, B, C, n_rows, w, result);
    else hipLaunchKernelGGL((k_r1cs_check<Fr>), dim3(grid_for(n_rows)), dim3(256), 0, st, A, B, C, n_rows, w, result);
    HIPCHK(hipGetLastError());
    return 0;
}
template <class Fr> int launch_qap_columns(hipStream_t st, const uint32_t* col_ptr, const uint32_t* row, const Fr* coeff, size_t n_cols, const Fr* L, Fr* out, uint32_t long_min) {
    if (!n_cols) return 0;
    hipLaunchKernelGGL((k_qap_columns<Fr>), dim3(grid_for(n_cols)), dim3(256), 0, st, col_ptr, row, coeff, n_cols, L, out, long_min ? long_min : QAP_LONG_COLUMN);
    HIPCHK(hipGetLastError());
    return 0;
}
template <class Fr> int launch_plonk_gate_count(hipStream_t st, const R1csMat& A, const R1csMat& B, const R1csMat& C, size_t n_rows, uint32_t* counts, uint32_t* offsets, uint32_t* tile_sums) {
    const size_t total = n_rows + 1, ntiles = (total + SCAN_TILE - 1) / SCAN_TILE;
    HIPCHK(hipMemsetAsync(counts + n_rows, 0, 4, st));
    if (n_rows) hipLaunchKernelGGL((k_plonk_gate_count<Fr>), dim3(grid_for(n_rows)), dim3(256), 0, st, A, B, C, n_rows, counts);
    hipLaunchKernelGGL(k_scan_tile_sums, dim3((unsigned)ntiles), dim3(256), 0, st, counts, tile_sums, total, 0xffffffffu);
    hipLaunchKernelGGL(k_scan_exclusive, dim3(1), dim3(1024), 0, st, tile_sums, tile_sums, ntiles);
    hipLaunchKernelGGL(k_scan_tiles, dim3((unsigned)ntiles), dim3(256), 0, st, counts, tile_sums, offsets, total, 0xffffffffu);
    HIPCHK(hipGetLastError());
    return 0;
}
template <class Fr> int launch_plonk_gate_emit(hipStream_t st, const R1csMat& A, const R1csMat& B, const R1csMat& C, size_t n_rows, uint32_t n_wires, uint32_t n_public,
                                               const uint32_t* counts, const uint32_t* offsets, size_t n_constraints, size_t n, const PlonkGateOut& o) {
    for (int i = 0; i < 5; i++) if (n > n_constraints) HIPCHK(hipMemsetAsync((Fr*)o.q[i] + n_constraints, 0, (n - n_constraints) * sizeof(Fr), st));
    if (n_rows + n_public) hipLaunchKernelGGL((k_plonk_gate_emit<Fr>), dim3(grid_for(n_rows + n_public)), dim3(256), 0, st, A, B, C, n_rows, n_wires, n_public, counts, offsets, o);
    HIPCHK(hipGetLastError());
    return 0;
}
template <class Fr> int launch_plonk_sigma_labels(hipStream_t st, const uint32_t* prev, const Fr* wpow, int log_n, const Fr& k1, const Fr& k2, Fr* sigma) {
    hipLaunchKernelGGL((k_plonk_sigma_labels<Fr>), dim3(grid_for((size_t)3 << log_n)), dim3(256), 0, st, prev, wpow, log_n, k1, k2, sigma);
    HIPCHK(hipGetLastError());
    return 0;
}
template <class Fr> int launch_build_twiddles_lazy(hipStream_t st, void* tw, size_t m, int log_m, const Fr* lo, const Fr* hi, int log_lo, const Fr& c32) {
    if (m > 1) hipLaunchKernelGGL((k_build_twiddles_lazy<Fr>), dim3(grid_for(m / 2)), dim3(256), 0, st, tw, m / 2, log_m, lo, hi, log_lo, c32);
    HIPCHK(hipGetLastError());
    return 0;
}
template <class Fr> int launch_ntt_ct_pass(hipStream_t st, bool first, NttVecs src, NttVecs dst, int nvec, size_t n, int log_m, int s0, int k, int t, const void* tw) {
    static PerDeviceOnce attr_set;
    if (attr_set.pending()) {
        HIPCHK(hipFuncSetAttribute((const void*)k_ntt_ct_pass<Fr, true>, hipFuncAttributeMaxDynamicSharedMemorySize, 36 << NTT_TILE_LOG));
        HIPCHK(hipFuncSetAttribute((const void*)k_ntt_ct_pass<Fr, false>, hipFuncAttributeMaxDynamicSharedMemorySize, 36 << NTT_TILE_LOG));
        attr_set.mark();
    }
    const int E = 1 << (k + t);
    if (first) hipLaunchKernelGGL((k_ntt_ct_pass<Fr, true>), dim3((unsigned)(n / E), nvec), dim3(NTT_THREADS), (size_t)E * 36, st, src, dst, log_m, s0, k, t, tw);
    else hipLaunchKernelGGL((k_ntt_ct_pass<Fr, false>), dim3((unsigned)(n / E), nvec), dim3(NTT_THREADS), (size_t)E * 36, st, src, dst, log_m, s0, k, t, tw);
    HIPCHK(hipGetLastError());
    return 0;
}
template <class Fr> int launch_build_twiddles_lazy_natural(hipStream_t st, void* tw, size_t m, const Fr* lo, const Fr* hi, int log_lo, const Fr& c32) {
    if (m > 1) hipLaunchKernelGGL((k_build_twiddles_lazy_natural<Fr>), dim3(grid_for(m / 2)), dim3(256), 0, st, tw, m / 2, lo, hi, log_lo, c32);
    HIPCHK(hipGetLastError());
    return 0;
}
template <class Fr> int launch_ntt_dit_pass(hipStream_t st, bool first, bool last, NttVecs out, NttVecs tmp, int nvec, size_t n, int log_m, int s0, int k, int t, const void* tw,
                                            const Fr* c_lo, const Fr* c_hi, int log_lo, const Fr& c32) {
    static PerDeviceOnce attr_set;
    if (attr_set.pending()) {
        HIPCHK(hipFuncSetAttribute((const void*)k_ntt_dit_pass<Fr, true, true>, hipFuncAttributeMaxDynamicSharedMemorySize, 36 << NTT_TILE_LOG));
        HIPCHK(hipFuncSetAttribute((const void*)k_ntt_dit_pass<Fr, true, false>, hipFuncAttributeMaxDynamicSharedMemorySize, 36 << NTT_TILE_LOG));
        HIPCHK(hipFuncSetAttribute((const void*)k_ntt_dit_pass<Fr, false, true>, hipFuncAttributeMaxDynamicSharedMemorySize, 36 << NTT_TILE_LOG));
        HIPCHK(hipFuncSetAttribute((const void*)k_ntt_dit_pass<Fr, false, false>, hipFuncAttributeMaxDynamicSharedMemorySize, 36 << NTT_TILE_LOG));
        attr_set.mark();
    }
    const int E = 1 << (k + t);
    const dim3 grid((unsigned)(n / E), nvec); const size_t lds = (size_t)E * 36;
    if (first && last) hipLaunchKernelGGL((k_ntt_dit_pass<Fr, true, true>), grid, dim3(NTT_THREADS), lds, st, out, tmp, log_m, s0, k, t, tw, c_lo, c_hi, log_lo, c32);
    else if (first) hipLaunchKernelGGL((k_ntt_dit_pass<Fr, true, false>), grid, dim3(NTT_THREADS), lds, st, out, tmp, log_m, s0, k, t, tw, c_lo, c_hi, log_lo, c32);
    else if (last) hipLaunchKernelGGL((k_ntt_dit_pass<Fr, false, true>), grid, dim3(NTT_THREADS), lds, st, out, tmp, log_m, s0, k, t, tw, c_lo, c_hi, log_lo, c32);
    else hipLaunchKernelGGL((k_ntt_dit_pass<Fr, false, false>), grid, dim3(NTT_THREADS), lds, st, out, tmp, log_m, s0, k, t, tw, c_lo, c_hi, log_lo, c32);
    HIPCHK(hipGetLastError());
    return 0;
}
template <class Fr> int launch_bitrev_finish_lazy(hipStream_t st, NttVecs dst, NttVecs src, int nvec, size_t n, int log_m, const Fr* scale, const Fr* c_lo, const Fr* c_hi, int log_lo) {
    if (log_m >= 2 * BITREV_B_LAZY)
        hipLaunchKernelGGL((k_bitrev_finish_lazy<Fr>), dim3((unsigned)(n >> (2 * BITREV_B_LAZY)), nvec), dim3(256), 0, st, dst, src, log_m, scale, c_lo, c_hi, log_lo);
    else
        hipLaunchKernelGGL((k_bitrev_finish_lazy_small<Fr>), dim3(grid_for(n), nvec), dim3(256), 0, st, dst, src, log_m, scale, c_lo, c_hi, log_lo);
    HIPCHK(hipGetLastError());
    return 0;
}

inline bool msm_sort_use_partition(size_t n, int c, int nwin, int shared, bool any_size = false) {
    const size_t nbuckets = (size_t)(shared ? 1 : nwin) << (c - 1);
    const size_t nregions = (nbuckets + ((size_t)1 << PART_REGION_LOG) - 1) >> PART_REGION_LOG;
    return (any_size || (size_t)nwin * n >= ((size_t)1 << 21)) && nregions >= 8 && nregions <= PART_MAX_REGIONS;
}
template <class Fr> int msm_sort_launch(hipStream_t st, const Fr* d_scalars, size_t n, int c, int nwin, int shared, char* scratch, size_t scratch_bytes, MsmSortPtrs* out, hipEvent_t* evs,
                                        int force) {
    if (force != 0 && force != CG_MSM_PATH_GENERAL && force != CG_MSM_PATH_SMALL && force != CG_MSM_PATH_PARTITION) return fail(CG_ERR_ARG, "msm_sort_launch: not a path of the dense schedule");
    const size_t nbuckets = (size_t)(shared ? 1 : nwin) << (c - 1);
    size_t off = 0;
    auto take = [&](size_t bytes) { void* p = scratch + off; off += align_up(bytes); return p; };
    int32_t* digits = (int32_t*)take((size_t)nwin * n * 4);
    uint32_t* sorted = (uint32_t*)take((size_t)nwin * n * 4);
    uint32_t* counts = (uint32_t*)take(nbuckets * 4);
    uint32_t* cursors = (uint32_t*)take(nbuckets * 4);
    uint32_t* offsets = (uint32_t*)take(nbuckets * 4);
    const size_t ntiles = (nbuckets + SCAN_TILE - 1) / SCAN_TILE;
    uint32_t* tile_sums = (uint32_t*)take(ntiles * 4);
    const size_t entries = (size_t)nwin * n;
    const bool no_small = !global_option(CG_GOPT_SORT_SMALL);
    const bool small_fits = shared && nbuckets <= SORT_SMALL_MAX_BUCKETS && entries <= SORT_SMALL_MAX_ENTRIES && n <= (1u << 24);
    if (force == CG_MSM_PATH_SMALL && (!small_fits || no_small))
        return fail(CG_ERR_ARG, "the one-workgroup schedule takes one shared bucket set of at most 2^13 buckets and at most 2^15 entries, with CG_GOPT_SORT_SMALL on");
    if (force == CG_MSM_PATH_PARTITION && !msm_sort_use_partition(n, c, nwin, shared, true)) return fail(CG_ERR_ARG, "the partition sort takes 8 to 4096 regions of 512 buckets");
    static PerDeviceOnce attr_small; static std::atomic<bool> small_unavailable{false};
    const bool may_small = shared && !no_small && (force == 0 || force == CG_MSM_PATH_SMALL);
    if (may_small && !small_unavailable.load(std::memory_order_relaxed) && attr_small.pending()) {
        if (hipFuncSetAttribute((const void*)k_msm_sort_small<Fr>, hipFuncAttributeMaxDynamicSharedMemorySize, (int)((2 * SORT_SMALL_MAX_BUCKETS + 1024) * 4)) == hipSuccess) attr_small.mark();
        else { (void)hipGetLastError(); small_unavailable.store(true); }
    }
    const bool small = may_small && !small_unavailable.load(std::memory_order_relaxed) && small_fits;
    if (force == CG_MSM_PATH_SMALL && !small) return fail(CG_ERR_HIP, "the one-workgroup schedule is not available on this device");
    const bool partition = !small && (force == CG_MSM_PATH_PARTITION || (force == 0 && msm_sort_use_partition(n, c, nwin, shared)));
    uint64_t* items = nullptr; uint32_t* region_total = nullptr; uint32_t* region_cursor = nullptr; uint32_t* total_items = nullptr;
    if (partition) {
        items = (uint64_t*)take(entries * 8);
        region_total = (uint32_t*)take(PART_MAX_REGIONS * 4);
        region_cursor = (uint32_t*)take(PART_MAX_REGIONS * 4);
        total_items = (uint32_t*)take(4);
    }
    if (off > scratch_bytes) return fail(CG_ERR_ARG, "msm_sort_launch: the layout of the schedule exceeds its scratch");
    if (evs) HIPCHK(hipEventRecord(evs[0], st));
    if (small) {
        const size_t lds = (2 * nbuckets + 1024) * 4;
        hipLaunchKernelGGL((k_msm_sort_small<Fr>), dim3(1), dim3(1024), lds, st, d_scalars, (uint32_t)n, c, nwin, counts, offsets, sorted);
        if (evs) HIPCHK(hipEventRecord(evs[1], st));
        HIPCHK(hipGetLastError());
        out->sorted = sorted; out->offsets = offsets; out->counts = counts; out->cap = 0; out->overflow = nullptr; out->path = CG_MSM_PATH_SMALL;
        return 0;
    }
    HIPCHK(hipMemsetAsync(counts, 0, align_up(nbuckets * 4) * 2, st));
    if (partition) {
        const size_t ptiles = (entries + PART_TILE - 1) / PART_TILE;
        const uint32_t nregions = (uint32_t)((nbuckets + ((size_t)1 << PART_REGION_LOG) - 1) >> PART_REGION_LOG);
        const unsigned itiles = (unsigned)(((entries + ITEM_TILE - 1) / ITEM_TILE + 7) / 8 * 8);
        HIPCHK(hipMemsetAsync(region_total, 0, nregions * 4, st));
        hipLaunchKernelGGL((k_msm_digits_only<Fr>), dim3(grid_for(n)), dim3(256), 0, st, d_scalars, n, c, nwin, digits);
        hipLaunchKernelGGL(k_part_hist, dim3((unsigned)ptiles), dim3(256), nregions * 4, st, digits, n, c, nwin, shared, nregions, region_total);
        hipLaunchKernelGGL(k_part_region_scan, dim3(1), dim3(1024), 0, st, region_total, nregions, region_cursor, total_items);
        const bool staged = global_option(CG_GOPT_SORT_STAGING) != 0;
        if (staged && nregions <= STAGE_MAX_REGIONS) {
            static PerDeviceOnce attr_set;
            if (attr_set.pending()) {
                HIPCHK(hipFuncSetAttribute((const void*)k_part_scatter_staged, hipFuncAttributeMaxDynamicSharedMemorySize, (int)part_staged_lds(STAGE_MAX_REGIONS)));
                HIPCHK(hipFuncSetAttribute((const void*)k_items_scatter_staged, hipFuncAttributeMaxDynamicSharedMemorySize, (int)ITEMS_STAGED_LDS));
                attr_set.mark();
            }
            hipLaunchKernelGGL(k_part_scatter_staged, dim3((unsigned)ptiles), dim3(STAGE_THREADS), part_staged_lds(nregions), st, digits, n, c, nwin, shared, nregions, region_cursor, items);
        } else
        hipLaunchKernelGGL(k_part_scatter, dim3((unsigned)ptiles), dim3(256), nregions * 4, st, digits, n, c, nwin, shared, nregions, region_cursor, items);
        hipLaunchKernelGGL(k_items_hist, dim3(itiles), dim3(256), 0, st, items, total_items, counts);
        hipLaunchKernelGGL(k_scan_tile_sums, dim3((unsigned)ntiles), dim3(256), 0, st, counts, tile_sums, nbuckets, 0xffffffffu);
        hipLaunchKernelGGL(k_scan_exclusive, dim3(1), dim3(1024), 0, st, tile_sums, tile_sums, ntiles);
        hipLaunchKernelGGL(k_scan_tiles, dim3((unsigned)ntiles), dim3(256), 0, st, counts, tile_sums, offsets, nbuckets, 0xffffffffu);
        if (staged && nregions <= STAGE_MAX_REGIONS) hipLaunchKernelGGL(k_items_scatter_staged, dim3(itiles), dim3(STAGE_THREADS), ITEMS_STAGED_LDS, st, items, total_items, offsets, cursors, sorted);
        else hipLaunchKernelGGL(k_items_scatter, dim3(itiles), dim3(256), 0, st, items, total_items, offsets, cursors, sorted);
        if (evs) HIPCHK(hipEventRecord(evs[1], st));
        HIPCHK(hipGetLastError());
        out->sorted = sorted; out->offsets = offsets; out->counts = counts; out->cap = 0; out->overflow = nullptr;
        out->path = staged && nregions <= STAGE_MAX_REGIONS ? CG_MSM_PATH_PARTITION : CG_MSM_PATH_PARTITION_UNSTAGED;
        return 0;
    }
    hipLaunchKernelGGL((k_msm_digits<Fr>), dim3(grid_for(n)), dim3(256), 0, st, d_scalars, n, c, nwin, shared, digits, counts);
    hipLaunchKernelGGL(k_scan_tile_sums, dim3((unsigned)ntiles), dim3(256), 0, st, counts, tile_sums, nbuckets, 0xffffffffu);
    hipLaunchKernelGGL(k_scan_exclusive, dim3(1), dim3(1024), 0, st, tile_sums, tile_sums, ntiles);
    hipLaunchKernelGGL(k_scan_tiles, dim3((unsigned)ntiles), dim3(256), 0, st, counts, tile_sums, offsets, nbuckets, 0xffffffffu);
    hipLaunchKernelGGL(k_msm_scatter, dim3(grid_for((size_t)nwin * n)), dim3(256), 0, st, digits, n, c, nwin, shared, offsets, cursors, sorted);
    if (evs) HIPCHK(hipEventRecord(evs[1], st));
    HIPCHK(hipGetLastError());
    out->sorted = sorted; out->offsets = offsets; out->counts = counts; out->cap = 0; out->overflow = nullptr; out->path = CG_MSM_PATH_GENERAL;
    return 0;
}
template <class Fr> int msm_sort_direct_launch(hipStream_t st, const Fr* d_scalars, size_t n, int c, int nwin, int shared, uint32_t cap, char* scratch, size_t scratch_bytes,
                                               MsmSortPtrs* out, hipEvent_t* evs, int force) {
    if (force != 0 && force != CG_MSM_PATH_DIRECT) return fail(CG_ERR_ARG, "msm_sort_direct_launch: the one-pass scatter is the only path here");
    if (cap < 1) return fail(CG_ERR_ARG, "the one-pass scatter takes a capacity of at least one entry per bucket");
    const size_t nbuckets = (size_t)(shared ? 1 : nwin) << (c - 1);
    size_t off = 0;
    auto take = [&](size_t bytes) { void* p = scratch + off; off += align_up(bytes); return p; };
    uint32_t* sorted = (uint32_t*)take(nbuckets * cap * 4);
    uint32_t* counts = (uint32_t*)take(nbuckets * 4);
    uint32_t* offsets = (uint32_t*)take(nbuckets * 4);
    const size_t ntiles = (nbuckets + SCAN_TILE - 1) / SCAN_TILE;
    uint32_t* tile_sums = (uint32_t*)take(ntiles * 4);
    uint32_t* overflow = (uint32_t*)take(4);
    if (off > scratch_bytes) return fail(CG_ERR_ARG, "msm_sort_direct_launch: the layout of the schedule exceeds its scratch");
    if (evs) HIPCHK(hipEventRecord(evs[0], st));
    HIPCHK(hipMemsetAsync(counts, 0, nbuckets * 4, st));
    HIPCHK(hipMemsetAsync(overflow, 0, 4, st));
    hipLaunchKernelGGL((k_msm_scatter_direct<Fr>), dim3(grid_for(n)), dim3(256), 0, st, d_scalars, n, c, nwin, shared, cap, counts, sorted, overflow);
    hipLaunchKernelGGL(k_scan_tile_sums, dim3((unsigned)ntiles), dim3(256), 0, st, counts, tile_sums, nbuckets, cap);
    hipLaunchKernelGGL(k_scan_exclusive, dim3(1), dim3(1024), 0, st, tile_sums, tile_sums, ntiles);
    hipLaunchKernelGGL(k_scan_tiles, dim3((unsigned)ntiles), dim3(256), 0, st, counts, tile_sums, offsets, nbuckets, cap);
    if (evs) HIPCHK(hipEventRecord(evs[1], st));
    HIPCHK(hipGetLastError());
    out->sorted = sorted; out->offsets = offsets; out->counts = counts; out->cap = cap; out->overflow = overflow; out->path = CG_MSM_PATH_DIRECT;
    return 0;
}

}

#define CG_INSTANTIATE_FR(Fr)                                                                                              \
    namespace cg {                                                                                                         \
    template decltype(launch_vec_binary<Fr>) launch_vec_binary<Fr>;                                                        \
    template decltype(launch_rep3_mul_local<Fr>) launch_rep3_mul_local<Fr>;                                                \
    template decltype(launch_distribute_powers<Fr>) launch_distribute_powers<Fr>;                                          \
    template decltype(launch_vec_count_noncanonical<Fr>) launch_vec_count_noncanonical<Fr>;                                \
    template decltype(launch_vec_fill<Fr>) launch_vec_fill<Fr>;                                                            \
    template decltype(launch_vec_gather_idx<Fr>) launch_vec_gather_idx<Fr>;                                                \
    template decltype(launch_vec_affine<Fr>) launch_vec_affine<Fr>;                                                        \
    template decltype(launch_vec_gather_strided<Fr>) launch_vec_gather_strided<Fr>;                                        \
    template decltype(launch_vec_lincomb<Fr>) launch_vec_lincomb<Fr>;                                                      \
    template decltype(launch_shamir_share<Fr>) launch_shamir_share<Fr>;                                                    \
    template decltype(launch_plonk_r2_factors<Fr>) launch_plonk_r2_factors<Fr>;                                            \
    template decltype(launch_prefix_scan<Fr>) launch_prefix_scan<Fr>;                                                      \
    template decltype(launch_vec_inverse<Fr>) launch_vec_inverse<Fr>;                                                      \
    template decltype(launch_plonk_additions<Fr>) launch_plonk_additions<Fr>;                                              \
    template decltype(launch_plonk_r3_blind<Fr>) launch_plonk_r3_blind<Fr>;                                                \
    template decltype(launch_plonk_r3_perm<Fr>) launch_plonk_r3_perm<Fr>;                                                  \
    template decltype(launch_plonk_r3_gate<Fr>) launch_plonk_r3_gate<Fr>;                                                  \
    template decltype(launch_plonk_mul4_tail<Fr>) launch_plonk_mul4_tail<Fr>;                                              \
    template decltype(launch_plonk_r3_t<Fr>) launch_plonk_r3_t<Fr>;                                                        \
    template decltype(launch_plonk_r3_divide<Fr>) launch_plonk_r3_divide<Fr>;                                              \
    template decltype(launch_spmv_csr<Fr>) launch_spmv_csr<Fr>;                                                            \
    template decltype(launch_r1cs_check<Fr>) launch_r1cs_check<Fr>;                                                        \
    template decltype(launch_qap_columns<Fr>) launch_qap_columns<Fr>;                                                      \
    template decltype(launch_plonk_gate_count<Fr>) launch_plonk_gate_count<Fr>;                                            \
    template decltype(launch_plonk_gate_emit<Fr>) launch_plonk_gate_emit<Fr>;                                              \
    template decltype(launch_plonk_sigma_labels<Fr>) launch_plonk_sigma_labels<Fr>;                                        \
    template decltype(launch_build_twiddles_lazy<Fr>) launch_build_twiddles_lazy<Fr>;                                      \
    template decltype(launch_ntt_ct_pass<Fr>) launch_ntt_ct_pass<Fr>;                                                      \
    template decltype(launch_build_twiddles_lazy_natural<Fr>) launch_build_twiddles_lazy_natural<Fr>;                      \
    template decltype(launch_ntt_dit_pass<Fr>) launch_ntt_dit_pass<Fr>;                                                    \
    template decltype(launch_bitrev_finish_lazy<Fr>) launch_bitrev_finish_lazy<Fr>;                                        \
    template decltype(msm_sort_launch<Fr>) msm_sort_launch<Fr>;                                                            \
    template decltype(msm_sort_direct_launch<Fr>) msm_sort_direct_launch<Fr>;                                              \
    }
```

### collaborative-circom_amd/csrc/launchers.hpp

```cpp
#pragma once
#include "common.hpp"

namespace cg {

template <class F> struct Affine;
template <class F> struct XYZZ;
template <class F> struct FastSubgroup;
struct NttVecs;
template <class F> struct PlonkR2Args;
template <class F> struct PlonkBlindArgs;
template <class F> struct PlonkPermArgs;
template <class F> struct PlonkGateArgs;
template <class F> struct PlonkMul4Args;
template <class F> struct PlonkTArgs;
template <class F> struct PlonkDivArgs;

constexpr int SCAN_TILE = 2048;
constexpr int PART_TILE = 16384;
constexpr int PART_REGION_LOG = 9;
constexpr int PART_MAX_REGIONS = 4096;
struct MsmSortPtrs { const uint32_t* sorted; const uint32_t* offsets; const uint32_t* counts; uint32_t cap; const uint32_t* overflow; int path; };
inline size_t msm_sort_scratch_bytes(size_t n, int c, int nwin) {
    const size_t nbuckets = (size_t)nwin << (c - 1);
    const size_t entries = (size_t)nwin * n;
    return 2 * align_up(entries * 4) + 3 * align_up(nbuckets * 4) + align_up(((nbuckets + SCAN_TILE - 1) / SCAN_TILE) * 4) +
           align_up(entries * 8) + 2 * align_up(PART_MAX_REGIONS * 4) + 256;
}
inline size_t msm_sort_direct_scratch_bytes(size_t n, int c, int nwin, int shared, uint32_t cap) {
    const size_t nbuckets = (size_t)(shared ? 1 : nwin) << (c - 1);
    return align_up(nbuckets * cap * 4) + 2 * align_up(nbuckets * 4) + align_up(((nbuckets + SCAN_TILE - 1) / SCAN_TILE) * 4) + 256;
}
template <class Fr> int msm_sort_launch(hipStream_t st, const Fr* d_scalars, size_t n, int c, int nwin, int shared, char* scratch, size_t scratch_bytes, MsmSortPtrs* out, hipEvent_t* evs,
                                        int force = 0);
template <class Fr> int msm_sort_direct_launch(hipStream_t st, const Fr* d_scalars, size_t n, int c, int nwin, int shared, uint32_t cap, char* scratch, size_t scratch_bytes,
                                               MsmSortPtrs* out, hipEvent_t* evs, int force = 0);

template <class F> int msm_accumulate_batch(hipStream_t st, const MsmAccSet* sets, int nsets, size_t n, int c, int nwin, bool shared, uint32_t cap, hipEvent_t* evs, uint32_t chunk_request, bool g2_slices);
template <class F> int msm_reduce_batch(hipStream_t st2, const MsmRedSet* sets, int nsets, size_t n, int c, int nwin, bool shared, uint32_t cap, hipEvent_t* ev_merged, int n_merged,
                                        hipEvent_t* evs, uint32_t chunk_request);
template <class F> size_t msm_acc_scratch_bytes(size_t n, int c, int nwin, bool shared, uint32_t chunk_request);
template <class F> int precompute_window_launch(hipStream_t st, const Affine<F>* d_src, Affine<F>* d_dst, size_t n, int c);
template <class F> int check_on_curve_launch(hipStream_t st, const Affine<F>* d_pts, size_t n, const F& b, unsigned long long* d_counters);
template <class F, class Fr> int check_subgroup_launch(hipStream_t st, const Affine<F>* d_pts, size_t n, unsigned long long* d_counters);
template <class F> int check_subgroup_fast_launch(hipStream_t st, const Affine<F>* d_pts, size_t n, const FastSubgroup<F>& c, unsigned long long* d_counters);
template <class F> int pack_bases_launch(hipStream_t st, const uint8_t* d_raw, size_t n, size_t stride, long inf_off, Affine<F>* d_dst);
template <class F> int gather_points_launch(hipStream_t st, Affine<F>* d_dst, const Affine<F>* d_src, const uint32_t* d_idx, size_t n);
template <class F> int synth_points_launch(hipStream_t st, const XYZZ<F>* d_lo, const XYZZ<F>* d_hi, int log_t, size_t n, Affine<F>* d_out);
template <class F, class Fr> int fixed_base_mul_launch(hipStream_t st, const Affine<F>& g, const Fr* d_scalars, size_t n, Affine<F>* d_tab, Affine<F>* d_out);

template <class Fr> int launch_vec_binary(hipStream_t st, int op, Fr* out, const Fr* a, const Fr* b, size_t n);
template <class Fr> int launch_rep3_mul_local(hipStream_t st, Fr* out, const Fr* aa, const Fr* ab, const Fr* ba, const Fr* bb, const Fr* mask, size_t n);
template <class Fr> int launch_vec_count_noncanonical(hipStream_t st, const Fr* v, size_t n, unsigned long long* n_bad);
template <class Fr> int launch_distribute_powers(hipStream_t st, Fr* v, size_t n, const Fr* lo, const Fr* hi, int log_lo);
template <class Fr> int launch_vec_affine(hipStream_t st, Fr* out, const Fr* a, size_t n, const Fr& c, const Fr& d);
template <class Fr> int launch_vec_lincomb(hipStream_t st, Fr* out, long long out_off, long long out_stride, size_t n, const LincombArgs<Fr>& a);
template <class Fr> int launch_shamir_share(hipStream_t st, const Fr* secrets, const Fr* coeffs, long long coeff_off, long long coeff_stride, size_t n, int degree,
                                            const ShareOuts<Fr>& o, long long out_off, long long out_stride);
template <class Fr> int launch_vec_gather_idx(hipStream_t st, Fr* out, const Fr* in, const uint32_t* idx, size_t n, uint32_t base);
template <class Fr> int launch_vec_fill(hipStream_t st, Fr* v, size_t n, const Fr& value);
template <class Fr> int launch_vec_gather_strided(hipStream_t st, Fr* out, const Fr* in, size_t n, size_t offset, size_t stride);
template <class Fr> int launch_prefix_scan(hipStream_t st, int op, Fr* out, const Fr* in, size_t n, Fr* scratch);
template <class Fr> int launch_vec_inverse(hipStream_t st, Fr* out, const Fr* in, size_t n);
template <class Fr> int launch_spmv_csr(hipStream_t st, const uint32_t* row_ptr, const uint32_t* col, const Fr* coeff, size_t n_rows, const Fr* pub,
                                        uint32_t n_inputs, int party, const Fr* wit_a, const Fr* wit_b, Fr* out_a, Fr* out_b);
struct R1csMat { const uint32_t* row_ptr; const uint32_t* col; const void* coeff; };
constexpr uint32_t QAP_LONG_COLUMN = 64;
template <class Fr> int launch_r1cs_check(hipStream_t st, const R1csMat& A, const R1csMat& B, const R1csMat& C, size_t n_rows, size_t nnz_total, int form, const Fr* w,
                                          unsigned long long* result);
template <class Fr> int launch_qap_columns(hipStream_t st, const uint32_t* col_ptr, const uint32_t* row, const Fr* coeff, size_t n_cols, const Fr* L, Fr* out, uint32_t long_min);
struct PlonkGateOut {
    uint32_t* map[3];
    void* q[5];
    uint32_t* add_ids;
    void* add_f;
};
template <class Fr> int launch_plonk_gate_count(hipStream_t st, const R1csMat& A, const R1csMat& B, const R1csMat& C, size_t n_rows, uint32_t* counts, uint32_t* offsets, uint32_t* tile_sums);
template <class Fr> int launch_plonk_gate_emit(hipStream_t st, const R1csMat& A, const R1csMat& B, const R1csMat& C, size_t n_rows, uint32_t n_wires, uint32_t n_public,
                                               const uint32_t* counts, const uint32_t* offsets, size_t n_constraints, size_t n, const PlonkGateOut& o);
template <class Fr> int launch_plonk_sigma_labels(hipStream_t st, const uint32_t* prev, const Fr* wpow, int log_n, const Fr& k1, const Fr& k2, Fr* sigma);
template <class Fr> int launch_plonk_additions(hipStream_t st, const uint32_t* order, size_t n, const uint32_t* ids, const Fr* coeffs, const Fr* pub, uint32_t n_inputs, int pc,
                                               Fr* ext_a, Fr* ext_b, size_t n_priv);
template <class Fr> int launch_plonk_r2_factors(hipStream_t st, const PlonkR2Args<Fr>& g, size_t n);
template <class Fr> int launch_plonk_r3_blind(hipStream_t st, const PlonkBlindArgs<Fr>& g, size_t n);
template <class Fr> int launch_plonk_r3_perm(hipStream_t st, const PlonkPermArgs<Fr>& g, size_t n);
template <class Fr> int launch_plonk_r3_gate(hipStream_t st, const PlonkGateArgs<Fr>& g, size_t n);
template <class Fr> int launch_plonk_mul4_tail(hipStream_t st, const PlonkMul4Args<Fr>& g, size_t n);
template <class Fr> int launch_plonk_r3_t(hipStream_t st, const PlonkTArgs<Fr>& g, size_t n);
template <class Fr> int launch_plonk_r3_divide(hipStream_t st, const PlonkDivArgs<Fr>& g, size_t n);
template <class Fr> int launch_build_twiddles_lazy(hipStream_t st, void* tw, size_t m, int log_m, const Fr* lo, const Fr* hi, int log_lo, const Fr& c32);
template <class Fr> int launch_build_twiddles_lazy_natural(hipStream_t st, void* tw, size_t m, const Fr* lo, const Fr* hi, int log_lo, const Fr& c32);
template <class Fr> int launch_ntt_ct_pass(hipStream_t st, bool first, NttVecs src, NttVecs dst, int nvec, size_t n, int log_m, int s0, int k, int t, const void* tw);
template <class Fr> int launch_ntt_dit_pass(hipStream_t st, bool first, bool last, NttVecs out, NttVecs tmp, int nvec, size_t n, int log_m, int s0, int k, int t, const void* tw,
                                            const Fr* c_lo, const Fr* c_hi, int log_lo, const Fr& c32);
template <class Fr> int launch_bitrev_finish_lazy(hipStream_t st, NttVecs dst, NttVecs src, int nvec, size_t n, int log_m, const Fr* scale, const Fr* c_lo, const Fr* c_hi, int log_lo);

int chacha12_fr_rand_launch(hipStream_t st, const uint32_t* key8, const uint32_t* mod8, int modulus_bits, uint64_t word_pos, uint64_t n_pairs, uint64_t n,
                            void* d_cand, uint32_t* d_tiles, unsigned long long* d_result, void* d_out);

}
```

### collaborative-circom_amd/csrc/msm_impl.hpp

```cpp
#pragma once
#include <cstdlib>
#include "launchers.hpp"
#include "msm_kernels.hpp"

namespace cg {

constexpr int bitsum_items() { return BITSUM_ITEMS; }
inline int bitsum_items_for(uint32_t nb) { return nb <= 1024u ? 1 : BITSUM_ITEMS; }
inline uint32_t bitsum_groups(uint32_t nb) { const uint32_t it = (uint32_t)bitsum_items_for(nb); return std::max<uint32_t>(1, (nb / 2 + 256 * it - 1) / (256 * it)); }

template <class F> struct IsFp2 { static constexpr bool value = false; };
template <class B> struct IsFp2<Fp2<B>> { static constexpr bool value = true; };
template <class F> constexpr size_t acc_resident_lanes() { return IsFp2<F>::value ? 0 : (size_t)256 * (sizeof(F) == 32 ? 3 : 2) * 256; }

template <class F>
MsmGeom msm_geom_of(size_t n, int c, int nwin, bool shared, uint32_t chunk_request) {
    MsmGeom g = msm_geom(n, c, nwin, shared, acc_resident_lanes<F>(), chunk_request, IsFp2<F>::value);
    g.bit_groups = bitsum_groups(g.nb);
    return g;
}

template <class F>
struct AccScratch {
    typedef typename BucketOf<F>::type B;
    B* buckets; B* cont; uint32_t* cont_bucket; B* partials; XYZZ<F>* wsums;
    size_t bytes;
    AccScratch(char* scratch, const MsmGeom& g) {
        size_t off = 0;
        auto take = [&](size_t size) { void* p = scratch ? scratch + off : nullptr; off += align_up(size); return p; };
        buckets = (B*)take(g.nbuckets * sizeof(B));
        cont = (B*)take((size_t)g.nchunks * sizeof(B));
        cont_bucket = (uint32_t*)take((size_t)g.nchunks * 4);
        partials = (B*)take(std::max({(size_t)g.nsets * g.segs, (size_t)64 * g.bit_groups, g.grid_partials()}) * sizeof(B));
        wsums = (XYZZ<F>*)take((size_t)std::max(g.ngroups, 64) * sizeof(XYZZ<F>));
        bytes = off;
    }
};
template <class F>
size_t msm_acc_scratch_bytes(size_t n, int c, int nwin, bool shared, uint32_t chunk_request) {
    return AccScratch<F>(nullptr, msm_geom_of<F>(n, c, nwin, shared, chunk_request)).bytes;
}

template <class F>
int msm_accumulate_batch(hipStream_t st, const MsmAccSet* sets, int nsets, size_t n, int c, int nwin, bool shared, uint32_t cap, hipEvent_t* evs, uint32_t chunk_request, bool g2_slices) {
    if (nsets < 1 || nsets > ACC_MAX_SETS) return fail(CG_ERR_ARG, "internal: accumulation batch size");
    const MsmGeom g = msm_geom_of<F>(n, c, nwin, shared, chunk_request);
    typedef typename BucketOf<F>::type B;
    AccSets<F> S{};
    for (int i = 0; i < nsets; i++) {
        const AccScratch<F> sc(sets[i].scratch, g);
        S.bases[i] = (const Affine<F>*)sets[i].bases; S.sorted[i] = sets[i].sorted; S.offsets[i] = sets[i].offsets; S.counts[i] = sets[i].counts;
        S.buckets[i] = sc.buckets; S.cont[i] = sc.cont; S.cont_bucket[i] = sc.cont_bucket;
        S.table_stride[i] = (uint32_t)sets[i].table_stride; S.may_have_inf[i] = sets[i].may_have_inf ? 1u : 0u;
    }
    const ptrdiff_t stride = nsets > 1 ? sets[1].scratch - sets[0].scratch : 0;
    bool one_fill = stride > 0 && (size_t)(nsets - 1) * (size_t)stride + g.nbuckets * sizeof(B) <= ((size_t)8 << 20);
    for (int i = 2; i < nsets && one_fill; i++) one_fill = sets[i].scratch - sets[i - 1].scratch == stride;
    if (one_fill) HIPCHK(hipMemsetAsync(S.buckets[0], 0, (size_t)(nsets - 1) * (size_t)stride + g.nbuckets * sizeof(B), st));
    else for (int i = 0; i < nsets; i++) HIPCHK(hipMemsetAsync(S.buckets[i], 0, g.nbuckets * sizeof(B), st));
    if (evs) HIPCHK(hipEventRecord(evs[0], st));
    auto launch_acc = [&](auto kern, int T, size_t lds) -> int {
        if (lds > 0) { if (int rc = ensure_dynamic_lds((const void*)kern, lds)) return rc; }
        for (int i = 0; i < nsets; i++)
            hipLaunchKernelGGL(kern, dim3((g.nchunks + T - 1) / T), dim3(T), lds, st, S.bases[i], S.sorted[i], S.offsets[i], S.counts[i],
                               (uint32_t)g.nbuckets, g.chunk_len, g.nchunks, S.table_stride[i], cap, S.buckets[i], S.cont[i], S.cont_bucket[i], S.may_have_inf[i]);
        return 0;
    };
    auto launch_pf = [&](auto kern, int T, size_t lds) -> int {
        if (lds > 0) { if (int rc = ensure_dynamic_lds((const void*)kern, lds)) return rc; }
        const uint32_t groups = (g.nchunks + T - 1) / T;
        const uint32_t slice = lds > 0 && g2_slices ? 256u * (uint32_t)std::max<size_t>(1, ((size_t)160 << 10) / lds) : groups;
        for (uint32_t first = 0; first < groups; first += slice)
            hipLaunchKernelGGL(kern, dim3(std::min(slice, groups - first), (unsigned)nsets), dim3(T), lds, st, S, (uint32_t)g.nbuckets, g.chunk_len, g.nchunks, first * (uint32_t)T);
        return 0;
    };
    constexpr bool g2 = IsFp2<F>::value;
    constexpr int MINW1 = sizeof(F) == 32 ? 3 : 2;
    const size_t lds2 = g2 ? (size_t)128 * 4 * sizeof(typename LazyOf<F>::type) : 0;
    int rc_acc;
    if (cap == 0) {
        if constexpr (!g2) rc_acc = launch_pf(k_msm_accumulate_pf<F, RegAcc29<F>, 256, MINW1>, 256, 0);
        else rc_acc = launch_pf(k_msm_accumulate_pf<F, LdsAcc29<F>, 128, 1>, 128, lds2);
    } else if constexpr (!g2) rc_acc = launch_acc(k_msm_accumulate<F, RegAcc29<F>, 256>, 256, 0);
    else rc_acc = launch_acc(k_msm_accumulate<F, LdsAcc29<F>, 128>, 128, lds2);
    if (rc_acc) return rc_acc;
    if (evs) HIPCHK(hipEventRecord(evs[1], st));
    HIPCHK(hipGetLastError());
    return 0;
}

template <class F>
int msm_reduce_batch(hipStream_t st2, const MsmRedSet* sets, int nsets, size_t n, int c, int nwin, bool shared, uint32_t cap, hipEvent_t* ev_merged, int n_merged,
                     hipEvent_t* evs, uint32_t chunk_request) {
    if (nsets < 1 || nsets > RED_MAX_SETS) return fail(CG_ERR_ARG, "internal: reduction batch size");
    const MsmGeom g = msm_geom_of<F>(n, c, nwin, shared, chunk_request);
    typedef typename BucketOf<F>::type B;
    RedSets<B> S{};
    XYZZ<F>* wsums[RED_MAX_SETS];
    const bool direct_out = !global_option(CG_GOPT_MSM_STAGED_OUT);
    for (int i = 0; i < nsets; i++) {
        const AccScratch<F> sc(sets[i].scratch, g);
        S.buckets[i] = sc.buckets; S.cont[i] = sc.cont; S.cont_bucket[i] = sc.cont_bucket; S.partials[i] = sc.partials;
        wsums[i] = direct_out ? (XYZZ<F>*)sets[i].h_out : sc.wsums; S.wsums[i] = wsums[i];
        S.offsets[i] = sets[i].offsets; S.counts[i] = sets[i].counts;
    }
    const unsigned ys = (unsigned)nsets;
    if (evs) HIPCHK(hipEventRecord(evs[0], st2));
    auto merged = [&]() -> int { for (int i = 0; i < n_merged; i++) HIPCHK(hipEventRecord(ev_merged[i], st2)); return 0; };
    auto deliver = [&](size_t count) -> int {
        if (evs) HIPCHK(hipEventRecord(evs[1], st2));
        HIPCHK(hipGetLastError());
        if (!direct_out) for (int i = 0; i < nsets; i++) HIPCHK(hipMemcpyAsync(sets[i].h_out, wsums[i], count * sizeof(XYZZ<F>), hipMemcpyDeviceToHost, st2));
        return 0;
    };
#ifdef CG_DEBUG_KNOBS
    static const int skip_reduce = getenv("CG_DEBUG_NO_REDUCE") ? atoi(getenv("CG_DEBUG_NO_REDUCE")) : 0;
#else
    constexpr int skip_reduce = 0;
#endif
    auto fake_reduce = [&]() -> int {
        for (int i = 0; i < nsets; i++) HIPCHK(hipMemsetAsync(wsums[i], 0, (size_t)g.ngroups * sizeof(XYZZ<F>), st2));
        return deliver((size_t)g.ngroups);
    };
    if (skip_reduce == 1) { if (int rc = merged()) return rc; return fake_reduce(); }
    hipLaunchKernelGGL((k_msm_merge_direct<B>), dim3((unsigned)((g.nbuckets + 63) / 64), ys), dim3(64), 0, st2, S, (uint32_t)g.nbuckets, g.chunk_len, g.nchunks, cap);
    hipLaunchKernelGGL((k_msm_merge_cont_l1<B>), dim3((g.nchunks + 63) / 64, ys), dim3(64), 0, st2, S, g.nchunks);
    hipLaunchKernelGGL((k_msm_merge_cont<B>), dim3((g.nchunks + 63) / 64, ys), dim3(64), 0, st2, S, g.nchunks);
    if (int rc = merged()) return rc;
    if (skip_reduce == 2) return fake_reduce();
    if (g.bitsum) {
        static PerDeviceOnce attr_set2;
        if (attr_set2.pending()) {
            HIPCHK(hipFuncSetAttribute((const void*)k_msm_bitsum_partial<B, bitsum_items()>, hipFuncAttributeMaxDynamicSharedMemorySize, (int)(256 * sizeof(B))));
            HIPCHK(hipFuncSetAttribute((const void*)k_msm_bitsum_partial<B, 1>, hipFuncAttributeMaxDynamicSharedMemorySize, (int)(256 * sizeof(B))));
            HIPCHK(hipFuncSetAttribute((const void*)k_msm_bitsum_final<F, B>, hipFuncAttributeMaxDynamicSharedMemorySize, (int)(64 * sizeof(B))));
            attr_set2.mark();
        }
        if (bitsum_items_for(g.nb) == 1) hipLaunchKernelGGL((k_msm_bitsum_partial<B, 1>), dim3((unsigned)(c * g.bit_groups), ys), dim3(256), 256 * sizeof(B), st2, S, g.nb, g.bit_groups);
        else hipLaunchKernelGGL((k_msm_bitsum_partial<B, bitsum_items()>), dim3((unsigned)(c * g.bit_groups), ys), dim3(256), 256 * sizeof(B), st2, S, g.nb, g.bit_groups);
        hipLaunchKernelGGL((k_msm_bitsum_final<F, B>), dim3((unsigned)c, ys), dim3(64), 64 * sizeof(B), st2, S, g.bit_groups);
        return deliver((size_t)c);
    }
    if (g.grid) {
        static PerDeviceOnce attr_set3;
        if (attr_set3.pending()) {
            HIPCHK(hipFuncSetAttribute((const void*)k_msm_grid_partial<B>, hipFuncAttributeMaxDynamicSharedMemorySize, (int)(256 * sizeof(B))));
            HIPCHK(hipFuncSetAttribute((const void*)k_msm_grid_bitsum<F, B, BITSUM_ITEMS>, hipFuncAttributeMaxDynamicSharedMemorySize, (int)(256 * sizeof(B))));
            attr_set3.mark();
        }
        const uint32_t H = 1u << g.log_h, L = 1u << g.log_l;
        hipLaunchKernelGGL((k_msm_grid_partial<B>), dim3((H / GRID_TR) * (L / GRID_TC), ys), dim3(256), 256 * sizeof(B), st2, S, (uint32_t)g.log_l, g.nb);
        hipLaunchKernelGGL((k_msm_grid_bitsum<F, B, BITSUM_ITEMS>), dim3((unsigned)g.ngroups, ys), dim3(256), 256 * sizeof(B), st2, S, (uint32_t)g.log_l, (uint32_t)g.log_h, g.gc, g.gr);
        return deliver((size_t)g.ngroups);
    }
    const size_t nseg_threads = (size_t)g.nsets * g.segs;
    hipLaunchKernelGGL((k_msm_reduce_segments<B>), dim3((unsigned)((nseg_threads + 63) / 64), ys), dim3(64), 0, st2, S, g.nb, g.seg_len, g.nsets);
    constexpr int WT = sizeof(B) > 160 ? 128 : 256;
    {
        static PerDeviceOnce attr_set;
        if (attr_set.pending()) { HIPCHK(hipFuncSetAttribute((const void*)k_msm_window_sum<F, B, WT>, hipFuncAttributeMaxDynamicSharedMemorySize, (int)(WT * sizeof(B)))); attr_set.mark(); }
    }
    hipLaunchKernelGGL((k_msm_window_sum<F, B, WT>), dim3(g.ngroups, ys), dim3(WT), WT * sizeof(B), st2, S, g.group_segs);
    return deliver((size_t)g.ngroups);
}

template <class F>
int pack_bases_launch(hipStream_t st, const uint8_t* d_raw, size_t n, size_t stride, long inf_off, Affine<F>* d_dst) {
    hipLaunchKernelGGL((k_pack_bases<F>), dim3(grid_for(n)), dim3(256), 0, st, d_raw, n, stride, inf_off, d_dst);
    HIPCHK(hipGetLastError());
    return 0;
}
template <class F>
int gather_points_launch(hipStream_t st, Affine<F>* d_dst, const Affine<F>* d_src, const uint32_t* d_idx, size_t n) {
    if (n) hipLaunchKernelGGL((k_gather_points<F>), dim3(grid_for(n)), dim3(256), 0, st, d_dst, d_src, d_idx, n);
    HIPCHK(hipGetLastError());
    return 0;
}
template <class F>
int check_on_curve_launch(hipStream_t st, const Affine<F>* d_pts, size_t n, const F& b, unsigned long long* d_counters) {
    if (n) hipLaunchKernelGGL((k_check_on_curve<F>), dim3(grid_for(n)), dim3(256), 0, st, d_pts, n, b, d_counters, d_counters + 1);
    HIPCHK(hipGetLastError());
    return 0;
}
template <class F, class Fr>
int check_subgroup_launch(hipStream_t st, const Affine<F>* d_pts, size_t n, unsigned long long* d_counters) {
    if (n) hipLaunchKernelGGL((k_check_subgroup<F, typename Fr::Params>), dim3((unsigned)std::min<size_t>((n + 127) / 128, 8192)), dim3(128), 0, st, d_pts, n, d_counters, d_counters + 1);
    HIPCHK(hipGetLastError());
    return 0;
}
template <class F>
int check_subgroup_fast_launch(hipStream_t st, const Affine<F>* d_pts, size_t n, const FastSubgroup<F>& c, unsigned long long* d_counters) {
    if (n) hipLaunchKernelGGL((k_check_subgroup_fast<F>), dim3((unsigned)std::min<size_t>((n + 127) / 128, 8192)), dim3(128), 0, st, d_pts, n, c, d_counters, d_counters + 1);
    HIPCHK(hipGetLastError());
    return 0;
}
template <class F>
int precompute_window_launch(hipStream_t st, const Affine<F>* d_src, Affine<F>* d_dst, size_t n, int c) {
    constexpr int K = sizeof(F) >= 64 ? 2 : 4;
    if (n) hipLaunchKernelGGL((k_precompute_window<F, K>), dim3((unsigned)std::min<size_t>(((n + K - 1) / K + 255) / 256, 65535)), dim3(256), 0, st, d_src, d_dst, n, c);
    HIPCHK(hipGetLastError());
    return 0;
}
template <class F>
int synth_points_launch(hipStream_t st, const XYZZ<F>* d_lo, const XYZZ<F>* d_hi, int log_t, size_t n, Affine<F>* d_out) {
    if (n) hipLaunchKernelGGL((k_synth_points<F>), dim3(grid_for(n)), dim3(256), 0, st, d_lo, d_hi, log_t, n, d_out);
    HIPCHK(hipGetLastError());
    return 0;
}

template <class F, class Fr>
int fixed_base_mul_launch(hipStream_t st, const Affine<F>& g, const Fr* d_scalars, size_t n, Affine<F>* d_tab, Affine<F>* d_out) {
    const int nwin = (Fr::Params::BITS + 7) / 8;
// ... 23 lines not shown
```

### collaborative-circom_amd/csrc/msm_kernels.hpp

```cpp
#pragma once
#include <type_traits>
#include "common.hpp"
#include "subgroup.hpp"
#include "curve.hpp"
#include "lazy29.hpp"
#include "vec_kernels.hpp"
#include "msm_sort_kernels.hpp"

namespace cg {

template <class A>
__device__ __forceinline__ A ld_struct(const A* p) {
    static_assert(sizeof(A) % 16 == 0, "");
    A r;
    const uint4* q = reinterpret_cast<const uint4*>(p);
    uint4* d = reinterpret_cast<uint4*>(&r);
    _Pragma("unroll") for (int i = 0; i < (int)(sizeof(A) / 16); i++) d[i] = q[i];
    return r;
}
template <class A>
__device__ __forceinline__ void st_struct(A* p, const A& r) {
    uint4* q = reinterpret_cast<uint4*>(p);
    const uint4* d = reinterpret_cast<const uint4*>(&r);
    _Pragma("unroll") for (int i = 0; i < (int)(sizeof(A) / 16); i++) q[i] = d[i];
// ... 181 lines not shown
    const L R = mul(y2, acc.get(3)) - acc.get(1);
    if (L::maybe_zero_mod_p(P) && L::is_zero_mod_p(P.norm())) { acc_madd_same_x(acc, x2f, y2f, R, negate); return; }
    const L PP = sqr(P);
    const L PPP = mul(P, PP);
    const L Q = mul(acc.get(0), PP);
    acc.set(2, mul(acc.get(2), PP));
    acc.set(3, mul(acc.get(3), PPP));
    const L X3 = (sqr(R) - PPP - Q.dbl()).norm();
    acc.set(1, (mul(R, Q - X3) - mul(acc.get(1), PPP)).norm());
    acc.set(0, X3);
}
template <class F, class Acc>
__device__ __forceinline__ void acc_madd_lazy(Acc& acc, const F& x2f, const F& y2f, bool negate) {
    typedef typename LazyOf<F>::type L;
    L x2 = L::template unpack<LazyShift<L>::value>(x2f), y2 = L::template unpack<LazyShift<L>::value>(y2f);
    if (negate) y2 = y2.neg();
    if (acc.inf) {
        const L one = L::one_small();
        const L ys = L::unpack_small(y2f);
        acc.set(0, L::unpack_small(x2f)); acc.set(1, negate ? ys.neg().norm() : ys); acc.set(2, one); acc.set(3, one); acc.inf = false;
        return;
    }
    if constexpr (HasColEngine<L>::value) { acc_madd_lazy_cols<F>(acc, x2f, y2f, x2, y2, negate); return; }
    L P = L::mul(x2, acc.get(2)) - acc.get(0);
    L R = L::mul(y2, acc.get(3)) - acc.get(1);
    if (L::maybe_zero_mod_p(P) && L::is_zero_mod_p(P.norm())) { acc_madd_same_x(acc, x2f, y2f, R, negate); return; }
    L PP = L::sqr(P);
    L PPP = L::mul(P, PP);
    L Q = L::mul(acc.get(0), PP);
    acc.set(2, L::mul(acc.get(2), PP));
    acc.set(3, L::mul(acc.get(3), PPP));
    L X3 = (L::sqr(R) - PPP - Q.dbl()).norm();
    acc.set(1, L::mul_sub(R, Q - X3, acc.get(1), PPP));
    acc.set(0, X3);
}
template <class F, class Acc>
__device__ __forceinline__ void acc_flush_lazy(Acc& acc, XYZZL<F>* dst) {
    XYZZL<F> r = bk_inf<XYZZL<F>>();
    if (!acc.inf) { r.c[0] = acc.get(0); r.c[1] = acc.get(1); r.c[2] = acc.get(2); r.c[3] = acc.get(3); }
    st_struct(dst, r);
    acc.inf = true;
}
template <class F, class Acc>
__device__ __forceinline__ void acc_madd(Acc& acc, const F& x2, const F& y2, bool negate) { acc_madd_lazy<F>(acc, x2, y2, negate); }
template <class F, class Acc>
__device__ __forceinline__ void acc_store(Acc& acc, XYZZL<F>* dst) { acc_flush_lazy<F>(acc, dst); }

template <class F, class Acc, int THREADS, int MINW = 1>
__global__ void __launch_bounds__(THREADS, MINW) k_msm_accumulate(const Affine<F>* __restrict__ bases, const uint32_t* __restrict__ sorted,
                                                            const uint32_t* __restrict__ offsets, const uint32_t* __restrict__ counts,
                                                            uint32_t nbuckets, uint32_t chunk_len, uint32_t nchunks, uint32_t table_stride, uint32_t cap,
                                                            typename BucketOf<F>::type* __restrict__ buckets, typename BucketOf<F>::type* __restrict__ cont,
                                                            uint32_t* __restrict__ cont_bucket, uint32_t may_have_inf) {
    extern __shared__ uint4 acc_lds[];
    const uint32_t q = blockIdx.x * THREADS + threadIdx.x;
    if (q >= nchunks) return;
    const uint32_t capc = cap ? cap : 0xffffffffu;
    const uint32_t total = offsets[nbuckets - 1] + min(counts[nbuckets - 1], capc);
    uint32_t pos = q * chunk_len;
    if (pos >= total) { cont_bucket[q] = 0xffffffffu; return; }
    const uint32_t end = min(pos + chunk_len, total);
    uint32_t lo = 0, hi = nbuckets - 1;
    while (lo < hi) { uint32_t mid = (lo + hi + 1) >> 1; if (offsets[mid] <= pos) lo = mid; else hi = mid - 1; }
    uint32_t b = lo;
    uint32_t bend = offsets[b] + min(counts[b], capc);
    uint32_t kidx = pos - offsets[b];
    bool continuation = offsets[b] != pos;
    cont_bucket[q] = continuation ? b : 0xffffffffu;
    Acc acc;
    acc.init(reinterpret_cast<typename Acc::LdsT*>(acc_lds), threadIdx.x, THREADS);
    while (pos < end) {
        if (pos == bend) {
            if (continuation) { acc_store<F>(acc, cont + q); continuation = false; } else acc_store<F>(acc, buckets + b);
            do { b++; } while (counts[b] == 0);
            bend = offsets[b] + min(counts[b], capc);
            kidx = 0;
        }
        const uint32_t e = sorted[cap ? (size_t)b * cap + kidx : (size_t)pos];
        pos++; kidx++;
        const size_t at = table_stride ? (size_t)((e >> 24) & 0x7fu) * table_stride + (e & 0xffffffu) : (size_t)(e & 0x7fffffffu);
        Affine<F> p = ld_struct(bases + at);
        if (may_have_inf && p.is_inf()) continue;
        acc_madd(acc, p.x, p.y, (e >> 31) != 0);
    }
    if (continuation) acc_store<F>(acc, cont + q); else acc_store<F>(acc, buckets + b);
}

template <class F>
struct AccSets {
    const Affine<F>* bases[ACC_MAX_SETS];
    const uint32_t* sorted[ACC_MAX_SETS]; const uint32_t* offsets[ACC_MAX_SETS]; const uint32_t* counts[ACC_MAX_SETS];
    typename BucketOf<F>::type* buckets[ACC_MAX_SETS]; typename BucketOf<F>::type* cont[ACC_MAX_SETS]; uint32_t* cont_bucket[ACC_MAX_SETS];
    uint32_t table_stride[ACC_MAX_SETS]; uint32_t may_have_inf[ACC_MAX_SETS];
};
template <class F, class Acc, int THREADS, int MINW>
__global__ void __launch_bounds__(THREADS, MINW) k_msm_accumulate_pf(const AccSets<F> S, uint32_t nbuckets, uint32_t chunk_len, uint32_t nchunks, uint32_t first_chunk) {
    const Affine<F>* __restrict__ bases = S.bases[blockIdx.y]; const uint32_t* __restrict__ sorted = S.sorted[blockIdx.y];
    const uint32_t* __restrict__ offsets = S.offsets[blockIdx.y]; const uint32_t* __restrict__ counts = S.counts[blockIdx.y];
    typename BucketOf<F>::type* __restrict__ buckets = S.buckets[blockIdx.y]; typename BucketOf<F>::type* __restrict__ cont = S.cont[blockIdx.y];
    uint32_t* __restrict__ cont_bucket = S.cont_bucket[blockIdx.y];
    const uint32_t table_stride = S.table_stride[blockIdx.y], may_have_inf = S.may_have_inf[blockIdx.y];
    extern __shared__ uint4 acc_lds[];
    const uint32_t q = first_chunk + blockIdx.x * THREADS + threadIdx.x;
    if (q >= nchunks) return;
    const uint32_t total = offsets[nbuckets - 1] + counts[nbuckets - 1];
    uint32_t pos = q * chunk_len;
    if (pos >= total) { cont_bucket[q] = 0xffffffffu; return; }
    const uint32_t end = min(pos + chunk_len, total);
    uint32_t lo = 0, hi = nbuckets - 1;
    while (lo < hi) { uint32_t mid = (lo + hi + 1) >> 1; if (offsets[mid] <= pos) lo = mid; else hi = mid - 1; }
    uint32_t b = lo;
    auto end_of = [&](uint32_t bb) -> uint32_t { return bb + 1 < nbuckets ? offsets[bb + 1] : total; };
    uint32_t bend = end_of(b), bend_next = end_of(b + 1);
    bool continuation = offsets[b] != pos;
    cont_bucket[q] = continuation ? b : 0xffffffffu;
    Acc acc;
    acc.init(reinterpret_cast<typename Acc::LdsT*>(acc_lds), threadIdx.x, THREADS);
    auto quad = [&](uint32_t at4) -> uint4 { return *reinterpret_cast<const uint4*>(sorted + at4); };
    uint4 cur = quad(pos & ~3u);
    for (uint32_t k = 0; k < (pos & 3u); k++) { cur.x = cur.y; cur.y = cur.z; cur.z = cur.w; }
    while (pos < end) {
        if (pos == bend) {
            if (continuation) { acc_store<F>(acc, cont + q); continuation = false; } else acc_store<F>(acc, buckets + b);
            b++; bend = bend_next; bend_next = end_of(b + 1);
            while (bend == pos) { b++; bend = bend_next; bend_next = end_of(b + 1); }
        }
        const uint32_t e = cur.x;
        const size_t at = table_stride ? (size_t)((e >> 24) & 0x7fu) * table_stride + (e & 0xffffffu) : (size_t)(e & 0x7fffffffu);
        Affine<F> p = ld_struct(bases + at);
        cur.x = cur.y; cur.y = cur.z; cur.z = cur.w;
        if (((pos + 1) & 3u) == 0 && pos + 1 < end) cur = quad(pos + 1);
        const bool neg = (e >> 31) != 0;
        pos++;
        if (may_have_inf && p.is_inf()) continue;
        acc_madd(acc, p.x, p.y, neg);
    }
    if (continuation) acc_store<F>(acc, cont + q); else acc_store<F>(acc, buckets + b);
}

constexpr uint32_t MERGE_DIRECT_MAX = 12;
template <class B>
struct RedSets {
    B* buckets[RED_MAX_SETS]; B* cont[RED_MAX_SETS]; uint32_t* cont_bucket[RED_MAX_SETS];
    const uint32_t* offsets[RED_MAX_SETS]; const uint32_t* counts[RED_MAX_SETS];
    B* partials[RED_MAX_SETS]; void* wsums[RED_MAX_SETS];
};
template <class B>
__global__ void __launch_bounds__(64) k_msm_merge_direct(const RedSets<B> S, uint32_t nbuckets, uint32_t chunk_len, uint32_t nchunks, uint32_t cap) {
    B* __restrict__ buckets = S.buckets[blockIdx.y]; const B* __restrict__ cont = S.cont[blockIdx.y]; uint32_t* __restrict__ cont_bucket = S.cont_bucket[blockIdx.y];
    const uint32_t* __restrict__ offsets = S.offsets[blockIdx.y]; const uint32_t* __restrict__ counts = S.counts[blockIdx.y];
    const uint32_t b = blockIdx.x * blockDim.x + threadIdx.x;
    if (b >= nbuckets) return;
    const uint32_t cnt = cap ? min(counts[b], cap) : counts[b];
    if (cnt == 0) return;
    const uint32_t first = offsets[b], last = first + cnt - 1;
    const uint32_t q0 = first / chunk_len + 1, q1 = last / chunk_len;
    if (q0 > q1 || q1 - q0 >= MERGE_DIRECT_MAX || q1 >= nchunks) return;
    B acc = ld_struct(buckets + b);
    for (uint32_t q = q0; q <= q1; q++) { acc = bk_add_inl(acc, ld_struct(cont + q)); cont_bucket[q] = 0xffffffffu; }
    st_struct(buckets + b, acc);
}
constexpr uint32_t MERGE_GROUP = 64;
template <class B>
__global__ void __launch_bounds__(64) k_msm_merge_cont_l1(const RedSets<B> S, uint32_t nchunks) {
    B* __restrict__ cont = S.cont[blockIdx.y]; const uint32_t* __restrict__ cont_bucket = S.cont_bucket[blockIdx.y];
    const uint32_t q = blockIdx.x * blockDim.x + threadIdx.x;
    if (q >= nchunks) return;
    const uint32_t b = cont_bucket[q];
    if (b == 0xffffffffu) return;
    const bool run_start = q == 0 || cont_bucket[q - 1] != b;
    if (!run_start && (q % MERGE_GROUP) != 0) return;
    const uint32_t next_head = (q / MERGE_GROUP + 1) * MERGE_GROUP;
    if (q + 1 >= nchunks || q + 1 >= next_head || cont_bucket[q + 1] != b) return;
    B acc = ld_struct(cont + q);
    for (uint32_t r = q + 1; r < nchunks && r < next_head && cont_bucket[r] == b; r++) acc = bk_add_inl(acc, ld_struct(cont + r));
    st_struct(cont + q, acc);
}
template <class B>
__global__ void __launch_bounds__(64) k_msm_merge_cont(const RedSets<B> S, uint32_t nchunks) {
    B* __restrict__ buckets = S.buckets[blockIdx.y]; const B* __restrict__ cont = S.cont[blockIdx.y]; const uint32_t* __restrict__ cont_bucket = S.cont_bucket[blockIdx.y];
    const uint32_t q = blockIdx.x * blockDim.x + threadIdx.x;
    if (q >= nchunks) return;
    const uint32_t b = cont_bucket[q];
    if (b == 0xffffffffu) return;
    if (q > 0 && cont_bucket[q - 1] == b) return;
    B acc = bk_add_inl(ld_struct(buckets + b), ld_struct(cont + q));
    for (uint32_t r = (q / MERGE_GROUP + 1) * MERGE_GROUP; r < nchunks && cont_bucket[r] == b; r += MERGE_GROUP) acc = bk_add_inl(acc, ld_struct(cont + r));
    st_struct(buckets + b, acc);
}

template <class B>
__device__ __forceinline__ B bk_mul_small(const B& p, uint32_t k) {
    B r = bk_inf<B>();
    if (k == 0) return r;
    for (int i = 31 - __builtin_clz(k); i >= 0; i--) {
        r = bk_dbl(r);
        if ((k >> i) & 1u) r = bk_add(r, p);
    }
    return r;
}

template <class B>
__global__ void __launch_bounds__(64) k_msm_reduce_segments(const RedSets<B> S, uint32_t nb, uint32_t seg_len, int nwin) {
    const B* __restrict__ buckets = S.buckets[blockIdx.y]; B* __restrict__ partials = S.partials[blockIdx.y];
    const uint32_t segs = nb / seg_len;
    const size_t t = (size_t)blockIdx.x * blockDim.x + threadIdx.x;
    if (t >= (size_t)nwin * segs) return;
    const uint32_t w = (uint32_t)(t / segs), seg = (uint32_t)(t % segs);
    const uint32_t lo = seg * seg_len;
    const B* Bk = buckets + (size_t)w * nb;
    B run = bk_inf<B>(), acc = bk_inf<B>();
    for (uint32_t b = lo + seg_len; b-- > lo;) {
        run = bk_add_inl(run, ld_struct(Bk + b));
        acc = bk_add_inl(acc, run);
    }
    acc = bk_add(acc, bk_mul_small(run, lo));
    st_struct(partials + t, acc);
}

template <class F, class B, int THREADS>
__global__ void __launch_bounds__(THREADS) k_msm_window_sum(const RedSets<B> S, uint32_t segs) {
    const B* __restrict__ partials = S.partials[blockIdx.y]; XYZZ<F>* __restrict__ window_sums = (XYZZ<F>*)S.wsums[blockIdx.y];
    extern __shared__ uint4 lds_raw[];
    B* sh = reinterpret_cast<B*>(lds_raw);
    const B* P = partials + (size_t)blockIdx.x * segs;
    B acc = bk_inf<B>();
    for (uint32_t s = threadIdx.x; s < segs; s += THREADS) acc = bk_add_inl(acc, ld_struct(P + s));
    sh[threadIdx.x] = acc;
    __syncthreads();
    for (int off = THREADS / 2; off >= 1; off >>= 1) {
        if ((int)threadIdx.x < off) { acc = bk_add_inl(sh[threadIdx.x], sh[threadIdx.x + off]); }
        __syncthreads();
        if ((int)threadIdx.x < off) sh[threadIdx.x] = acc;
        __syncthreads();
    }
    if (threadIdx.x == 0) st_struct(window_sums + blockIdx.x, bk_to_xyzz<F>(sh[0]));
}

template <class B, int ITEMS>
__global__ void __launch_bounds__(256) k_msm_bitsum_partial(const RedSets<B> S, uint32_t nb, uint32_t groups) {
    const B* __restrict__ buckets = S.buckets[blockIdx.y]; B* __restrict__ partials = S.partials[blockIdx.y];
    extern __shared__ uint4 lds_raw[];
    B* sh = reinterpret_cast<B*>(lds_raw);
    const uint32_t k = blockIdx.x / groups, g = blockIdx.x % groups;
    const uint32_t j0 = (g * 256u + threadIdx.x) * ITEMS;
    B acc = bk_inf<B>();
    for (uint32_t i = 0; i < (uint32_t)ITEMS; i++) {
        const uint32_t j = j0 + i;
        const uint64_t w = (((uint64_t)j >> k) << (k + 1)) | ((uint64_t)1 << k) | (j & (((uint32_t)1 << k) - 1u));
        if (w >= 1 && w <= nb) acc = bk_add_inl(acc, ld_struct(buckets + (w - 1)));
    }
    sh[threadIdx.x] = acc;
    __syncthreads();
    for (int off = 128; off >= 1; off >>= 1) {
        if ((int)threadIdx.x < off) acc = bk_add_inl(sh[threadIdx.x], sh[threadIdx.x + off]);
        __syncthreads();
        if ((int)threadIdx.x < off) sh[threadIdx.x] = acc;
        __syncthreads();
    }
    if (threadIdx.x == 0) st_struct(partials + blockIdx.x, sh[0]);
}
template <class F, class B>
__global__ void __launch_bounds__(64) k_msm_bitsum_final(const RedSets<B> S, uint32_t groups) {
    const B* __restrict__ partials = S.partials[blockIdx.y]; XYZZ<F>* __restrict__ bit_sums = (XYZZ<F>*)S.wsums[blockIdx.y];
    extern __shared__ uint4 lds_raw[];
    B* sh = reinterpret_cast<B*>(lds_raw);
    const B* P = partials + (size_t)blockIdx.x * groups;
    B acc = bk_inf<B>();
    for (uint32_t s = threadIdx.x; s < groups; s += 64) acc = bk_add_inl(acc, ld_struct(P + s));
    sh[threadIdx.x] = acc;
    __syncthreads();
    for (int off = 32; off >= 1; off >>= 1) {
        if ((int)threadIdx.x < off) acc = bk_add_inl(sh[threadIdx.x], sh[threadIdx.x + off]);
        __syncthreads();
        if ((int)threadIdx.x < off) sh[threadIdx.x] = acc;
        __syncthreads();
    }
    if (threadIdx.x == 0) st_struct(bit_sums + blockIdx.x, bk_to_xyzz<F>(sh[0]));
}

template <class B>
__global__ void __launch_bounds__(256) k_msm_grid_partial(const RedSets<B> S, uint32_t log_l, uint32_t nb) {
    const B* __restrict__ buckets = S.buckets[blockIdx.y];
    B* __restrict__ colpart = S.partials[blockIdx.y]; B* __restrict__ rowpart = colpart + (size_t)((nb >> log_l) / GRID_TR) * ((size_t)1 << log_l);
    extern __shared__ uint4 lds_raw[];
    B* sh = reinterpret_cast<B*>(lds_raw);
    const uint32_t L = 1u << log_l, ncb = L / GRID_TC;
    const uint32_t cb = blockIdx.x % ncb, rb = blockIdx.x / ncb, t = threadIdx.x;
    const B* tile = buckets + (size_t)rb * GRID_TR * L + (size_t)cb * GRID_TC;
    constexpr uint32_t RPQ = GRID_TR / 4;
    constexpr uint32_t SEGS = 256 / GRID_TR, CPS = GRID_TC / SEGS;
    {
        const uint32_t col = t & 63u, rq = t >> 6;
        B acc = ld_struct(tile + (size_t)(rq * RPQ) * L + col);
        for (uint32_t i = 1; i < RPQ; i++) acc = bk_add_inl(acc, ld_struct(tile + (size_t)(rq * RPQ + i) * L + col));
        sh[t] = acc;
        __syncthreads();
        for (int off = 128; off >= 64; off >>= 1) {
            if ((int)t < off) acc = bk_add_inl(sh[t], sh[t + off]);
            __syncthreads();
            if ((int)t < off) sh[t] = acc;
            __syncthreads();
        }
        if (t < 64) st_struct(colpart + (size_t)rb * L + (size_t)cb * GRID_TC + t, acc);
        __syncthreads();
    }
    {
// ... 166 lines not shown
```

### collaborative-circom_amd/csrc/msm_sort_kernels.hpp

```cpp
#pragma once
#include "field.hpp"
#include "launchers.hpp"
#include "vec_kernels.hpp"

namespace cg {

template <class Fr>
__global__ void __launch_bounds__(256) k_msm_digits(const Fr* __restrict__ scalars, size_t n, int c, int nwin, int shared,
                                                    int32_t* __restrict__ digits, uint32_t* __restrict__ counts) {
    const uint32_t nb = 1u << (c - 1);
    const uint32_t mask = (1u << c) - 1;
    for (size_t i = (size_t)blockIdx.x * blockDim.x + threadIdx.x; i < n; i += (size_t)gridDim.x * blockDim.x) {
        Fr s = ld_fp(scalars + i).from_mont();
        uint32_t carry = 0;
        for (int w = 0; w < nwin; w++) {
            uint32_t d = (s.v[0] & mask) + carry;
            _Pragma("unroll") for (int l = 0; l < Fr::N; l++) {
                uint64_t two = ((uint64_t)(l + 1 < Fr::N ? s.v[l + 1] : 0u) << 32) | s.v[l];
                s.v[l] = (uint32_t)(two >> c);
            }
            int32_t dig;
            if (d > nb) { dig = (int32_t)d - (int32_t)(1u << c); carry = 1; } else { dig = (int32_t)d; carry = 0; }
            digits[(size_t)w * n + i] = dig;
            if (dig != 0) atomicAdd(&counts[(shared ? 0 : (size_t)w * nb) + (uint32_t)(dig < 0 ? -dig : dig) - 1], 1u);
        }
    }
}

static __global__ void __launch_bounds__(256) k_scan_tile_sums(const uint32_t* __restrict__ in, uint32_t* __restrict__ tile_sums, size_t total, uint32_t cap) {
    __shared__ uint32_t red[256];
    const size_t base = (size_t)blockIdx.x * SCAN_TILE;
    uint32_t s = 0;
    for (int k = 0; k < SCAN_TILE / 256; k++) { size_t i = base + (size_t)k * 256 + threadIdx.x; if (i < total) s += min(in[i], cap); }
    red[threadIdx.x] = s;
    __syncthreads();
    for (int off = 128; off >= 1; off >>= 1) { if ((int)threadIdx.x < off) red[threadIdx.x] += red[threadIdx.x + off]; __syncthreads(); }
    if (threadIdx.x == 0) tile_sums[blockIdx.x] = red[0];
}
static __global__ void __launch_bounds__(1024) k_scan_exclusive(const uint32_t* in, uint32_t* out, size_t total) {
    __shared__ uint32_t part[1024];
    const size_t chunk = (total + 1023) / 1024;
    const size_t lo = (size_t)threadIdx.x * chunk, hi = lo + chunk < total ? lo + chunk : total;
    uint32_t s = 0;
    for (size_t i = lo; i < hi; i++) s += in[i];
    part[threadIdx.x] = s;
    __syncthreads();
    for (int off = 1; off < 1024; off <<= 1) {
        uint32_t v = threadIdx.x >= (unsigned)off ? part[threadIdx.x - off] : 0;
        __syncthreads();
        part[threadIdx.x] += v;
        __syncthreads();
    }
    uint32_t run = threadIdx.x ? part[threadIdx.x - 1] : 0;
    for (size_t i = lo; i < hi; i++) { uint32_t v = in[i]; out[i] = run; run += v; }
}
static __global__ void __launch_bounds__(256) k_scan_tiles(const uint32_t* __restrict__ in, const uint32_t* __restrict__ tile_base, uint32_t* __restrict__ out, size_t total, uint32_t cap) {
    __shared__ uint32_t part[256];
    const size_t base = (size_t)blockIdx.x * SCAN_TILE + (size_t)threadIdx.x * (SCAN_TILE / 256);
    uint32_t v[SCAN_TILE / 256]; uint32_t s = 0;
    for (int k = 0; k < SCAN_TILE / 256; k++) { size_t i = base + k; v[k] = i < total ? min(in[i], cap) : 0; s += v[k]; }
    part[threadIdx.x] = s;
    __syncthreads();
    for (int off = 1; off < 256; off <<= 1) {
        uint32_t t = threadIdx.x >= (unsigned)off ? part[threadIdx.x - off] : 0;
        __syncthreads();
        part[threadIdx.x] += t;
        __syncthreads();
    }
    uint32_t run = tile_base[blockIdx.x] + (threadIdx.x ? part[threadIdx.x - 1] : 0);
    for (int k = 0; k < SCAN_TILE / 256; k++) { size_t i = base + k; if (i < total) out[i] = run; run += v[k]; }
}

static __global__ void __launch_bounds__(256) k_msm_scatter(const int32_t* __restrict__ digits, size_t n, int c, int nwin, int shared, const uint32_t* __restrict__ offsets,
                                                     uint32_t* __restrict__ cursors, uint32_t* __restrict__ sorted) {
    const uint32_t nb = 1u << (c - 1);
    const size_t total = (size_t)nwin * n;
    for (size_t idx = (size_t)blockIdx.x * blockDim.x + threadIdx.x; idx < total; idx += (size_t)gridDim.x * blockDim.x) {
        const int32_t dig = digits[idx];
        if (dig == 0) continue;
        const size_t w = idx / n;
        const uint32_t i = (uint32_t)(idx - w * n);
        const size_t bucket = (shared ? 0 : w * nb) + (uint32_t)(dig < 0 ? -dig : dig) - 1;
        const uint32_t pos = offsets[bucket] + atomicAdd(&cursors[bucket], 1u);
        sorted[pos] = (shared ? ((uint32_t)w << 24) | i : i) | (dig < 0 ? 0x80000000u : 0u);
    }
}

constexpr uint32_t SORT_SMALL_MAX_BUCKETS = 1u << 13, SORT_SMALL_MAX_ENTRIES = 1u << 15;
template <class Fr>
__global__ void __launch_bounds__(1024) k_msm_sort_small(const Fr* __restrict__ scalars, uint32_t n, int c, int nwin,
                                                         uint32_t* __restrict__ counts, uint32_t* __restrict__ offsets, uint32_t* __restrict__ sorted) {
    extern __shared__ uint32_t sort_lds[];
    const uint32_t nb = 1u << (c - 1), mask = (1u << c) - 1, t = threadIdx.x;
    uint32_t* cnt = sort_lds; uint32_t* cur = sort_lds + nb; uint32_t* part = sort_lds + 2 * nb;
    for (uint32_t b = t; b < nb; b += 1024) cnt[b] = 0;
    __syncthreads();
    auto digits_of = [&](uint32_t i, auto&& f) {
        Fr s = ld_fp(scalars + i).from_mont();
        uint32_t carry = 0;
        for (int w = 0; w < nwin; w++) {
            const uint32_t d = (s.v[0] & mask) + carry;
            _Pragma("unroll") for (int l = 0; l < Fr::N; l++) {
                const uint64_t two = ((uint64_t)(l + 1 < Fr::N ? s.v[l + 1] : 0u) << 32) | s.v[l];
                s.v[l] = (uint32_t)(two >> c);
            }
            if (d > nb) { carry = 1; if (d != (1u << c)) f((uint32_t)w, (1u << c) - d - 1, true); }
            else { carry = 0; if (d) f((uint32_t)w, d - 1, false); }
        }
    };
    for (uint32_t i = t; i < n; i += 1024) digits_of(i, [&](uint32_t, uint32_t b, bool) { atomicAdd(&cnt[b], 1u); });
    __syncthreads();
    const uint32_t chunk = (nb + 1023) / 1024, lo = min(t * chunk, nb), hi = min(lo + chunk, nb);
    uint32_t mine = 0;
    for (uint32_t b = lo; b < hi; b++) mine += cnt[b];
    part[t] = mine;
    __syncthreads();
    for (uint32_t off = 1; off < 1024; off <<= 1) {
        const uint32_t v = t >= off ? part[t - off] : 0;
        __syncthreads();
        part[t] += v;
        __syncthreads();
    }
    uint32_t run = part[t] - mine;
    for (uint32_t b = lo; b < hi; b++) { const uint32_t k = cnt[b]; offsets[b] = run; cur[b] = run; counts[b] = k; run += k; }
    __syncthreads();
    for (uint32_t i = t; i < n; i += 1024)
        digits_of(i, [&](uint32_t w, uint32_t b, bool neg) { sorted[atomicAdd(&cur[b], 1u)] = (w << 24) | i | (neg ? 0x80000000u : 0u); });
}


__device__ __forceinline__ bool part_decode(int32_t dig, size_t w, uint32_t i, uint32_t nb, int shared, uint32_t* bucket, uint32_t* payload) {
    if (dig == 0) return false;
    *bucket = (uint32_t)((shared ? 0 : w * nb) + (uint32_t)(dig < 0 ? -dig : dig) - 1);
    *payload = (shared ? ((uint32_t)w << 24) | i : i) | (dig < 0 ? 0x80000000u : 0u);
    return true;
}
template <class Fr>
__global__ void __launch_bounds__(256) k_msm_digits_only(const Fr* __restrict__ scalars, size_t n, int c, int nwin, int32_t* __restrict__ digits) {
    const uint32_t nb = 1u << (c - 1);
    const uint32_t mask = (1u << c) - 1;
    for (size_t i = (size_t)blockIdx.x * blockDim.x + threadIdx.x; i < n; i += (size_t)gridDim.x * blockDim.x) {
        Fr s = ld_fp(scalars + i).from_mont();
        uint32_t carry = 0;
        for (int w = 0; w < nwin; w++) {
            uint32_t d = (s.v[0] & mask) + carry;
            _Pragma("unroll") for (int l = 0; l < Fr::N; l++) {
                uint64_t two = ((uint64_t)(l + 1 < Fr::N ? s.v[l + 1] : 0u) << 32) | s.v[l];
                s.v[l] = (uint32_t)(two >> c);
            }
            int32_t dig;
            if (d > nb) { dig = (int32_t)d - (int32_t)(1u << c); carry = 1; } else { dig = (int32_t)d; carry = 0; }
            digits[(size_t)w * n + i] = dig;
        }
    }
}
static __global__ void __launch_bounds__(256) k_part_hist(const int32_t* __restrict__ digits, size_t n, int c, int nwin, int shared, uint32_t nregions,
                                                          uint32_t* __restrict__ region_total) {
    extern __shared__ uint32_t lds_cnt[];
    for (uint32_t r = threadIdx.x; r < nregions; r += 256) lds_cnt[r] = 0;
    __syncthreads();
    const uint32_t nb = 1u << (c - 1);
    const size_t total = (size_t)nwin * n, base = (size_t)blockIdx.x * PART_TILE;
    for (int k = 0; k < PART_TILE / 256; k++) {
        const size_t idx = base + (size_t)k * 256 + threadIdx.x;
        if (idx >= total) break;
        const size_t w = idx / n; uint32_t bucket, payload;
        if (part_decode(digits[idx], w, (uint32_t)(idx - w * n), nb, shared, &bucket, &payload)) atomicAdd(&lds_cnt[bucket >> PART_REGION_LOG], 1u);
    }
    __syncthreads();
    for (uint32_t r = threadIdx.x; r < nregions; r += 256) { const uint32_t v = lds_cnt[r]; if (v) atomicAdd(&region_total[r], v); }
}
static __global__ void __launch_bounds__(1024) k_part_region_scan(const uint32_t* __restrict__ region_total, uint32_t nregions, uint32_t* __restrict__ region_cursor,
                                                                  uint32_t* __restrict__ total_items) {
    __shared__ uint32_t part[1024];
    const uint32_t per = (nregions + 1023) / 1024;
    uint32_t v[4] = {0, 0, 0, 0}, mine = 0;
    for (uint32_t k = 0; k < per; k++) { const uint32_t r = threadIdx.x * per + k; if (r < nregions) { v[k] = region_total[r]; mine += v[k]; } }
    part[threadIdx.x] = mine;
    __syncthreads();
    for (int off = 1; off < 1024; off <<= 1) {
        uint32_t t = threadIdx.x >= (unsigned)off ? part[threadIdx.x - off] : 0;
        __syncthreads();
        part[threadIdx.x] += t;
        __syncthreads();
    }
    uint32_t run = threadIdx.x ? part[threadIdx.x - 1] : 0;
    if (threadIdx.x == 1023) *total_items = part[1023];
    for (uint32_t k = 0; k < per; k++) { const uint32_t r = threadIdx.x * per + k; if (r < nregions) { region_cursor[r] = run; run += v[k]; } }
}
static __global__ void __launch_bounds__(256) k_part_scatter(const int32_t* __restrict__ digits, size_t n, int c, int nwin, int shared, uint32_t nregions,
                                                             uint32_t* __restrict__ region_cursor, uint64_t* __restrict__ items) {
    extern __shared__ uint32_t lds_cnt[];
    for (uint32_t r = threadIdx.x; r < nregions; r += 256) lds_cnt[r] = 0;
    __syncthreads();
    const uint32_t nb = 1u << (c - 1);
    const size_t total = (size_t)nwin * n, base = (size_t)blockIdx.x * PART_TILE;
    for (int k = 0; k < PART_TILE / 256; k++) {
        const size_t idx = base + (size_t)k * 256 + threadIdx.x;
        if (idx >= total) break;
        const size_t w = idx / n; uint32_t bucket, payload;
        if (part_decode(digits[idx], w, (uint32_t)(idx - w * n), nb, shared, &bucket, &payload)) atomicAdd(&lds_cnt[bucket >> PART_REGION_LOG], 1u);
    }
    __syncthreads();
    for (uint32_t r = threadIdx.x; r < nregions; r += 256) { const uint32_t v = lds_cnt[r]; lds_cnt[r] = v ? atomicAdd(&region_cursor[r], v) : 0u; }
    __syncthreads();
    for (int k = 0; k < PART_TILE / 256; k++) {
        const size_t idx = base + (size_t)k * 256 + threadIdx.x;
        if (idx >= total) break;
        const size_t w = idx / n; uint32_t bucket, payload;
        if (part_decode(digits[idx], w, (uint32_t)(idx - w * n), nb, shared, &bucket, &payload)) {
            const uint32_t pos = atomicAdd(&lds_cnt[bucket >> PART_REGION_LOG], 1u);
            items[pos] = ((uint64_t)bucket << 32) | payload;
        }
    }
}
constexpr int ITEM_TILE = 16384;
constexpr uint32_t ITEM_WINDOW = 2048;
__device__ __forceinline__ uint32_t xcd_tile(uint32_t block, uint32_t nblocks) {
    const uint32_t per = (nblocks + 7) / 8;
    return (block & 7u) * per + (block >> 3);
}
static __global__ void __launch_bounds__(256) k_items_hist(const uint64_t* __restrict__ items, const uint32_t* __restrict__ total_items, uint32_t* __restrict__ counts) {
    __shared__ uint32_t cnt[ITEM_WINDOW];
    const size_t total = *total_items, base = (size_t)xcd_tile(blockIdx.x, gridDim.x) * ITEM_TILE;
    if (base >= total) return;
    for (uint32_t r = threadIdx.x; r < ITEM_WINDOW; r += 256) cnt[r] = 0;
    const uint32_t b0 = (uint32_t)(items[base] >> 32) & ~((1u << PART_REGION_LOG) - 1);
    __syncthreads();
    for (int k = 0; k < ITEM_TILE / 256; k++) {
        const size_t e = base + (size_t)k * 256 + threadIdx.x;
        if (e >= total) break;
        const uint32_t bucket = (uint32_t)(items[e] >> 32), d = bucket - b0;
        if (d < ITEM_WINDOW) atomicAdd(&cnt[d], 1u); else atomicAdd(&counts[bucket], 1u);
    }
    __syncthreads();
    for (uint32_t r = threadIdx.x; r < ITEM_WINDOW; r += 256) { const uint32_t v = cnt[r]; if (v) atomicAdd(&counts[b0 + r], v); }
}
static __global__ void __launch_bounds__(256) k_items_scatter(const uint64_t* __restrict__ items, const uint32_t* __restrict__ total_items, const uint32_t* __restrict__ offsets,
                                                              uint32_t* __restrict__ cursors, uint32_t* __restrict__ sorted) {
    __shared__ uint32_t cnt[ITEM_WINDOW];
    const size_t total = *total_items, base = (size_t)xcd_tile(blockIdx.x, gridDim.x) * ITEM_TILE;
    if (base >= total) return;
    for (uint32_t r = threadIdx.x; r < ITEM_WINDOW; r += 256) cnt[r] = 0;
    const uint32_t b0 = (uint32_t)(items[base] >> 32) & ~((1u << PART_REGION_LOG) - 1);
    __syncthreads();
    for (int k = 0; k < ITEM_TILE / 256; k++) {
        const size_t e = base + (size_t)k * 256 + threadIdx.x;
        if (e >= total) break;
        const uint32_t d = (uint32_t)(items[e] >> 32) - b0;
        if (d < ITEM_WINDOW) atomicAdd(&cnt[d], 1u);
    }
    __syncthreads();
    for (uint32_t r = threadIdx.x; r < ITEM_WINDOW; r += 256) { const uint32_t v = cnt[r]; cnt[r] = v ? offsets[b0 + r] + atomicAdd(&cursors[b0 + r], v) : 0u; }
    __syncthreads();
    for (int k = 0; k < ITEM_TILE / 256; k++) {
        const size_t e = base + (size_t)k * 256 + threadIdx.x;
        if (e >= total) break;
        const uint64_t it = items[e];
        const uint32_t bucket = (uint32_t)(it >> 32), d = bucket - b0;
        const uint32_t pos = d < ITEM_WINDOW ? atomicAdd(&cnt[d], 1u) : offsets[bucket] + atomicAdd(&cursors[bucket], 1u);
        sorted[pos] = (uint32_t)it;
    }
}

constexpr int STAGE_THREADS = 1024;
constexpr int STAGE_PER_LANE = PART_TILE / STAGE_THREADS;
constexpr uint32_t STAGE_MAX_REGIONS = 2048;
inline size_t part_staged_lds(uint32_t nregions) { return (size_t)(2 * nregions + 32) * 4 + (size_t)PART_TILE * 8; }
constexpr size_t ITEMS_STAGED_LDS = (size_t)(2 * ITEM_WINDOW + 32) * 4 + (size_t)ITEM_TILE * 6;
__device__ __forceinline__ uint32_t stage_block_scan(uint32_t v, uint32_t* scratch, uint32_t* total) {
    const int lane = threadIdx.x & 63, wave = threadIdx.x >> 6;
    uint32_t inc = v;
    _Pragma("unroll") for (int off = 1; off < 64; off <<= 1) { const uint32_t t = __shfl_up(inc, off, 64); if (lane >= off) inc += t; }
    if (lane == 63) scratch[wave] = inc;
    __syncthreads();
    if (wave == 0) {
        uint32_t w = lane < STAGE_THREADS / 64 ? scratch[lane] : 0, winc = w;
        _Pragma("unroll") for (int off = 1; off < STAGE_THREADS / 64; off <<= 1) { const uint32_t t = __shfl_up(winc, off, 64); if (lane >= off) winc += t; }
        if (lane < STAGE_THREADS / 64) scratch[lane] = winc - w;
        if (lane == STAGE_THREADS / 64 - 1) scratch[STAGE_THREADS / 64] = winc;
    }
    __syncthreads();
    const uint32_t r = scratch[wave] + inc - v;
    *total = scratch[STAGE_THREADS / 64];
    __syncthreads();
    return r;
}
static __global__ void __launch_bounds__(STAGE_THREADS) k_part_scatter_staged(const int32_t* __restrict__ digits, size_t n, int c, int nwin, int shared, uint32_t nregions,
                                                                            uint32_t* __restrict__ region_cursor, uint64_t* __restrict__ items) {
    extern __shared__ uint32_t lds_u32[];
    uint32_t* cnt = lds_u32;
    uint32_t* delta = cnt + nregions;
    uint32_t* scratch = delta + nregions;
    uint64_t* stage = reinterpret_cast<uint64_t*>(scratch + 32);
    for (uint32_t r = threadIdx.x; r < nregions; r += STAGE_THREADS) cnt[r] = 0;
    const uint32_t nb = 1u << (c - 1);
    const size_t total = (size_t)nwin * n, base = (size_t)blockIdx.x * PART_TILE;
    int32_t dig[STAGE_PER_LANE];
    _Pragma("unroll") for (int k = 0; k < STAGE_PER_LANE; k++) {
        const size_t idx = base + (size_t)k * STAGE_THREADS + threadIdx.x;
        dig[k] = idx < total ? digits[idx] : 0;
    }
    __syncthreads();
    uint32_t bucket[STAGE_PER_LANE], payload[STAGE_PER_LANE], rank[STAGE_PER_LANE];
    _Pragma("unroll") for (int k = 0; k < STAGE_PER_LANE; k++) {
        const size_t idx = base + (size_t)k * STAGE_THREADS + threadIdx.x;
        const size_t w = idx / n;
        bucket[k] = 0xffffffffu; payload[k] = 0; rank[k] = 0;
        if (part_decode(dig[k], w, (uint32_t)(idx - w * n), nb, shared, &bucket[k], &payload[k])) rank[k] = atomicAdd(&cnt[bucket[k] >> PART_REGION_LOG], 1u);
        else bucket[k] = 0xffffffffu;
    }
    __syncthreads();
    const uint32_t per = (nregions + STAGE_THREADS - 1) / STAGE_THREADS;
    uint32_t v[2] = {0, 0}, mine = 0;
    for (uint32_t j = 0; j < per; j++) { const uint32_t r = threadIdx.x * per + j; if (r < nregions) { v[j] = cnt[r]; mine += v[j]; } }
    uint32_t tile_items;
    uint32_t run = stage_block_scan(mine, scratch, &tile_items);
    for (uint32_t j = 0; j < per; j++) {
        const uint32_t r = threadIdx.x * per + j;
        if (r < nregions) { cnt[r] = run; delta[r] = (v[j] ? atomicAdd(&region_cursor[r], v[j]) : 0u) - run; run += v[j]; }
    }
    __syncthreads();
    _Pragma("unroll") for (int k = 0; k < STAGE_PER_LANE; k++)
        if (bucket[k] != 0xffffffffu) stage[cnt[bucket[k] >> PART_REGION_LOG] + rank[k]] = ((uint64_t)bucket[k] << 32) | payload[k];
    __syncthreads();
    for (uint32_t s = threadIdx.x; s < tile_items; s += STAGE_THREADS) {
        const uint64_t it = stage[s];
        items[delta[(uint32_t)(it >> 32) >> PART_REGION_LOG] + s] = it;
    }
}
static __global__ void __launch_bounds__(STAGE_THREADS) k_items_scatter_staged(const uint64_t* __restrict__ items, const uint32_t* __restrict__ total_items,
                                                                             const uint32_t* __restrict__ offsets, uint32_t* __restrict__ cursors, uint32_t* __restrict__ sorted) {
    extern __shared__ uint32_t lds_u32[];
    uint32_t* cnt = lds_u32;
    uint32_t* delta = cnt + ITEM_WINDOW;
    uint32_t* scratch = delta + ITEM_WINDOW;
    uint32_t* stage = scratch + 32;
    uint16_t* slot = reinterpret_cast<uint16_t*>(stage + ITEM_TILE);
    const size_t total = *total_items, base = (size_t)xcd_tile(blockIdx.x, gridDim.x) * ITEM_TILE;
    if (base >= total) return;
    for (uint32_t r = threadIdx.x; r < ITEM_WINDOW; r += STAGE_THREADS) cnt[r] = 0;
    uint64_t it[STAGE_PER_LANE];
    _Pragma("unroll") for (int k = 0; k < STAGE_PER_LANE; k++) {
        const size_t e = base + (size_t)k * STAGE_THREADS + threadIdx.x;
        it[k] = e < total ? items[e] : ~(uint64_t)0;
    }
    const uint32_t b0 = (uint32_t)(items[base] >> 32) & ~((1u << PART_REGION_LOG) - 1);
    __syncthreads();
    uint32_t rank[STAGE_PER_LANE];
    _Pragma("unroll") for (int k = 0; k < STAGE_PER_LANE; k++) {
        rank[k] = 0;
        if (it[k] == ~(uint64_t)0) continue;
        const uint32_t bucket = (uint32_t)(it[k] >> 32), d = bucket - b0;
        if (d < ITEM_WINDOW) rank[k] = atomicAdd(&cnt[d], 1u);
        else { sorted[offsets[bucket] + atomicAdd(&cursors[bucket], 1u)] = (uint32_t)it[k]; it[k] = ~(uint64_t)0; }
    }
    __syncthreads();
    constexpr uint32_t per = ITEM_WINDOW / STAGE_THREADS;
    uint32_t v[per], mine = 0;
    _Pragma("unroll") for (uint32_t j = 0; j < per; j++) { v[j] = cnt[threadIdx.x * per + j]; mine += v[j]; }
    uint32_t tile_items;
    uint32_t run = stage_block_scan(mine, scratch, &tile_items);
    _Pragma("unroll") for (uint32_t j = 0; j < per; j++) {
        const uint32_t r = threadIdx.x * per + j;
        cnt[r] = run;
        delta[r] = (v[j] ? offsets[b0 + r] + atomicAdd(&cursors[b0 + r], v[j]) : 0u) - run;
        run += v[j];
    }
    __syncthreads();
    _Pragma("unroll") for (int k = 0; k < STAGE_PER_LANE; k++) {
        if (it[k] == ~(uint64_t)0) continue;
        const uint32_t d = (uint32_t)(it[k] >> 32) - b0, at = cnt[d] + rank[k];
        stage[at] = (uint32_t)it[k]; slot[at] = (uint16_t)d;
    }
    __syncthreads();
    for (uint32_t s = threadIdx.x; s < tile_items; s += STAGE_THREADS) sorted[delta[slot[s]] + s] = stage[s];
}

template <class Fr>
__global__ void __launch_bounds__(256) k_msm_scatter_direct(const Fr* __restrict__ scalars, size_t n, int c, int nwin, int shared, uint32_t cap,
                                                            uint32_t* __restrict__ counts, uint32_t* __restrict__ sorted, uint32_t* __restrict__ overflow) {
    const uint32_t nb = 1u << (c - 1);
    const uint32_t mask = (1u << c) - 1;
    for (size_t i = (size_t)blockIdx.x * blockDim.x + threadIdx.x; i < n; i += (size_t)gridDim.x * blockDim.x) {
        Fr s = ld_fp(scalars + i).from_mont();
        uint32_t carry = 0;
        for (int w = 0; w < nwin; w++) {
            uint32_t d = (s.v[0] & mask) + carry;
            _Pragma("unroll") for (int l = 0; l < Fr::N; l++) {
                uint64_t two = ((uint64_t)(l + 1 < Fr::N ? s.v[l + 1] : 0u) << 32) | s.v[l];
                s.v[l] = (uint32_t)(two >> c);
            }
            int32_t dig;
            if (d > nb) { dig = (int32_t)d - (int32_t)(1u << c); carry = 1; } else { dig = (int32_t)d; carry = 0; }
            if (dig == 0) continue;
            const size_t bucket = (shared ? 0 : (size_t)w * nb) + (uint32_t)(dig < 0 ? -dig : dig) - 1;
            const uint32_t pos = atomicAdd(&counts[bucket], 1u);
            if (pos < cap) sorted[bucket * cap + pos] = (shared ? ((uint32_t)w << 24) | (uint32_t)i : (uint32_t)i) | (dig < 0 ? 0x80000000u : 0u);
            else *overflow = 1u;
        }
    }
}

}
```

Measured before the change: 61.59 million constraints/s.

## Fuse scalar recoding into partition sort kernels and drop bucket memsets

The partition sort path no longer writes a digits array. The histogram and scatter kernels now recode scalars on the fly through a shared msm_recode helper, which saves a kernel launch and a full read/write of nwin*n digits, and the scratch size shrinks to match. The per-set bucket memset in accumulation is replaced by having the merge kernel write infinity into empty buckets. A new reduce-batch mode 4 flushes G1 reductions once per component. In exchange, recoding runs twice per scalar (once for counting, once for scattering), and correctness now depends on the merge kernel covering every bucket.

```diff
diff --git a/collaborative-circom_amd/csrc/capi.hip b/collaborative-circom_amd/csrc/capi.hip
--- a/collaborative-circom_amd/csrc/capi.hip
+++ b/collaborative-circom_amd/csrc/capi.hip
@@ -300,7 +300,7 @@
         case CG_OPT_MSM_TABLE_ORDER: if (value < 0 || value > 2) break; ctx->table_order = (int)value; return 0;
         case CG_OPT_MSM_G2_AFTER: if (value < -1 || value > 64) break; ctx->g2_after = (int)value; return 0;
         case CG_OPT_MSM_G2_SLICES: if (value < 0 || value > 1) break; ctx->g2_slices = (int)value; return 0;
-        case CG_OPT_MSM_REDUCE_BATCH: if (value < 0 || value > 3) break; ctx->red_batch = (int)value; return 0;
+        case CG_OPT_MSM_REDUCE_BATCH: if (value < 0 || value > 4) break; ctx->red_batch = (int)value; return 0;
         case CG_OPT_MSM_ACC_SLOTS: if (value < 2 || value > cg_ctx::ACC_SLOTS_MAX) break; ctx->acc_slots = (int)value; return 0;
         case CG_OPT_MSM_WIDE_SMALL: if (value < 0 || value > 30 || (value > 1 && value < 10)) break; ctx->wide_small = (int)value; return 0;
         case CG_OPT_MSM_ONE_STREAM_LOG: if (value < 0 || value > 30) break; ctx->one_stream_log = (int)value; return 0;
diff --git a/collaborative-circom_amd/csrc/capi_msm.hip b/collaborative-circom_amd/csrc/capi_msm.hip
--- a/collaborative-circom_amd/csrc/capi_msm.hip
+++ b/collaborative-circom_amd/csrc/capi_msm.hip
@@ -186,6 +186,9 @@
         const int red_batch = ctx->red_batch;
         const uint64_t wide_max = ctx->wide_small == 0 ? 0 : (uint64_t)1 << (ctx->wide_small == 1 ? 20 : ctx->wide_small);
         const bool small_call = k <= 2 && (uint64_t)nwin * n <= wide_max;
+        bool whole_tables = nb > 1;
+        for (int b = 0; b < nb; b++) whole_tables = whole_tables && (offsets ? offsets[b] : 0) == 0 && n == bases[b]->n;
+        const bool g1_per_comp = red_batch == 4 && k == 2 && (uint64_t)nwin * n > wide_max && whole_tables;
         bool single_field = true;
         for (int b = 1; b < nb; b++) single_field = single_field && bases[b]->group == bases[0]->group;
         const int acc_slots = red_batch || small_call ? std::min((int)cg_ctx::ACC_SLOTS_MAX, std::max(acc_slots_min, red_batch >= 2 || small_call ? nb * k : nb + 1)) : acc_slots_min;
@@ -335,15 +338,17 @@
             const size_t at = ctx->g2_after < 0 ? g1o.size() : std::min<size_t>((size_t)ctx->g2_after, g1o.size());
             order.insert(order.end(), g1o.begin(), g1o.begin() + at); order.insert(order.end(), g2o.begin(), g2o.end()); order.insert(order.end(), g1o.begin() + at, g1o.end());
             bool waited[2] = {false, false};
-            int left[2] = {(int)g1o.size(), (int)g2o.size()}, left_sched[2] = {0, 0};
+            int left[2] = {(int)g1o.size(), (int)g2o.size()}, left_sched[2] = {0, 0}, left_comp_g1[2] = {0, 0};
             for (auto& pr : order) left_sched[pr.second]++;
+            for (auto& pr : g1o) left_comp_g1[pr.second]++;
             for (size_t i = 0; i < order.size(); i++) {
                 const int b = order[i].first, j = order[i].second, gi = bases[b]->group == CG_G1 ? 0 : 1;
                 if (!waited[j]) { HIPCHK(hipStreamWaitEvent(ctx->stream, ctx->ev_sorted[j], 0)); waited[j] = true; }
                 { int rc = do_acc(b, j); if (rc) return rc; }
                 const bool last_of_field = --left[gi] == 0;
                 const bool comp_changes = i + 1 == order.size() || order[i + 1].second != j || (bases[order[i + 1].first]->group == CG_G1 ? 0 : 1) != gi;
-                if (red_batch == 0 || (red_batch == 1 && comp_changes) || (last_of_field && red_batch != 3) || (int)pend[gi].size() == RED_MAX_SETS) { int rc3 = flush(gi); if (rc3) return rc3; }
+                const bool comp_g1_done = g1_per_comp && gi == 0 && --left_comp_g1[j] == 0;
+                if (red_batch == 0 || (red_batch == 1 && comp_changes) || (last_of_field && red_batch != 3) || comp_g1_done || (int)pend[gi].size() == RED_MAX_SETS) { int rc3 = flush(gi); if (rc3) return rc3; }
                 if (--left_sched[j] == 0) HIPCHK(hipEventRecord(ctx->ev_sched_free[j], ctx->stream));
             }
         } else
@@ -356,7 +361,7 @@
                 const int gi = bases[b]->group == CG_G1 ? 0 : 1;
                 { int rc = do_acc(b, j); if (rc) return rc; }
                 const bool last_here = --left_in_comp[gi] == 0;
-                if (red_batch == 0 || (red_batch == 1 && last_here) || (last_here && j == k - 1 && red_batch != 3) || (int)pend[gi].size() == RED_MAX_SETS) { int rc3 = flush(gi); if (rc3) return rc3; }
+                if (red_batch == 0 || (red_batch == 1 && last_here) || (last_here && j == k - 1 && red_batch != 3) || (g1_per_comp && gi == 0 && last_here) || (int)pend[gi].size() == RED_MAX_SETS) { int rc3 = flush(gi); if (rc3) return rc3; }
             }
             HIPCHK(hipEventRecord(ctx->ev_sched_free[j % nsched], ctx->stream));
             if (j + 2 < k && nsched == 2) {
diff --git a/collaborative-circom_amd/csrc/capi_streams.hip b/collaborative-circom_amd/csrc/capi_streams.hip
--- a/collaborative-circom_amd/csrc/capi_streams.hip
+++ b/collaborative-circom_amd/csrc/capi_streams.hip
@@ -209,7 +209,7 @@
     {
         auto seed = [](const char* name, int lo, int hi, int& field) { if (const char* e = tune_env(name)) { const int v = atoi(e); if (v >= lo && v <= hi) field = v; } };
         seed("CG_MSM_TABLE_ORDER", 0, 2, c->table_order); seed("CG_MSM_G2_AFTER", -1, 64, c->g2_after); seed("CG_MSM_G2_SLICES", 0, 1, c->g2_slices);
-        seed("CG_MSM_REDUCE_BATCH", 0, 3, c->red_batch); seed("CG_MSM_ACC_SLOTS", 2, cg_ctx::ACC_SLOTS_MAX, c->acc_slots); seed("CG_MSM_WIDE_SMALL", 0, 30, c->wide_small); seed("CG_MSM_ONE_STREAM_LOG", 0, 30, c->one_stream_log); seed("CG_MSM_OFF_MAIN_LOG", 0, 30, c->off_main_log); seed("CG_MSM_SOLO_LOG", 0, 30, c->solo_log);
+        seed("CG_MSM_REDUCE_BATCH", 0, 4, c->red_batch); seed("CG_MSM_ACC_SLOTS", 2, cg_ctx::ACC_SLOTS_MAX, c->acc_slots); seed("CG_MSM_WIDE_SMALL", 0, 30, c->wide_small); seed("CG_MSM_ONE_STREAM_LOG", 0, 30, c->one_stream_log); seed("CG_MSM_OFF_MAIN_LOG", 0, 30, c->off_main_log); seed("CG_MSM_SOLO_LOG", 0, 30, c->solo_log);
     }
     if (flags & 1u) { c->prio_main = 1; c->prio_copy = 1; c->prio_side = 0; }
     else if (flags & 2u) { static const int bulk_cls = tune_env("CG_BULK_CLASS") ? atoi(tune_env("CG_BULK_CLASS")) : -1; c->prio_main = bulk_cls; c->prio_side = 0; }
diff --git a/collaborative-circom_amd/csrc/fr_impl.hpp b/collaborative-circom_amd/csrc/fr_impl.hpp
--- a/collaborative-circom_amd/csrc/fr_impl.hpp
+++ b/collaborative-circom_amd/csrc/fr_impl.hpp
@@ -222,15 +222,7 @@
                                         int force) {
     if (force != 0 && force != CG_MSM_PATH_GENERAL && force != CG_MSM_PATH_SMALL && force != CG_MSM_PATH_PARTITION) return fail(CG_ERR_ARG, "msm_sort_launch: not a path of the dense schedule");
     const size_t nbuckets = (size_t)(shared ? 1 : nwin) << (c - 1);
-    size_t off = 0;
-    auto take = [&](size_t bytes) { void* p = scratch + off; off += align_up(bytes); return p; };
-    int32_t* digits = (int32_t*)take((size_t)nwin * n * 4);
-    uint32_t* sorted = (uint32_t*)take((size_t)nwin * n * 4);
-    uint32_t* counts = (uint32_t*)take(nbuckets * 4);
-    uint32_t* cursors = (uint32_t*)take(nbuckets * 4);
-    uint32_t* offsets = (uint32_t*)take(nbuckets * 4);
     const size_t ntiles = (nbuckets + SCAN_TILE - 1) / SCAN_TILE;
-    uint32_t* tile_sums = (uint32_t*)take(ntiles * 4);
     const size_t entries = (size_t)nwin * n;
     const bool no_small = !global_option(CG_GOPT_SORT_SMALL);
     const bool small_fits = shared && nbuckets <= SORT_SMALL_MAX_BUCKETS && entries <= SORT_SMALL_MAX_ENTRIES && n <= (1u << 24);
@@ -246,6 +238,14 @@
     const bool small = may_small && !small_unavailable.load(std::memory_order_relaxed) && small_fits;
     if (force == CG_MSM_PATH_SMALL && !small) return fail(CG_ERR_HIP, "the one-workgroup schedule is not available on this device");
     const bool partition = !small && (force == CG_MSM_PATH_PARTITION || (force == 0 && msm_sort_use_partition(n, c, nwin, shared)));
+    size_t off = 0;
+    auto take = [&](size_t bytes) { void* p = scratch + off; off += align_up(bytes); return p; };
+    int32_t* digits = small || partition ? nullptr : (int32_t*)take(entries * 4);
+    uint32_t* sorted = (uint32_t*)take(entries * 4);
+    uint32_t* counts = (uint32_t*)take(nbuckets * 4);
+    uint32_t* cursors = (uint32_t*)take(nbuckets * 4);
+    uint32_t* offsets = (uint32_t*)take(nbuckets * 4);
+    uint32_t* tile_sums = (uint32_t*)take(ntiles * 4);
     uint64_t* items = nullptr; uint32_t* region_total = nullptr; uint32_t* region_cursor = nullptr; uint32_t* total_items = nullptr;
     if (partition) {
         items = (uint64_t*)take(entries * 8);
@@ -265,24 +265,24 @@
     }
     HIPCHK(hipMemsetAsync(counts, 0, align_up(nbuckets * 4) * 2, st));
     if (partition) {
-        const size_t ptiles = (entries + PART_TILE - 1) / PART_TILE;
+        const uint32_t tile_scalars = part_tile_scalars(nwin);
+        const size_t ptiles = (n + tile_scalars - 1) / tile_scalars;
         const uint32_t nregions = (uint32_t)((nbuckets + ((size_t)1 << PART_REGION_LOG) - 1) >> PART_REGION_LOG);
         const unsigned itiles = (unsigned)(((entries + ITEM_TILE - 1) / ITEM_TILE + 7) / 8 * 8);
         HIPCHK(hipMemsetAsync(region_total, 0, nregions * 4, st));
-        hipLaunchKernelGGL((k_msm_digits_only<Fr>), dim3(grid_for(n)), dim3(256), 0, st, d_scalars, n, c, nwin, digits);
-        hipLaunchKernelGGL(k_part_hist, dim3((unsigned)ptiles), dim3(256), nregions * 4, st, digits, n, c, nwin, shared, nregions, region_total);
+        hipLaunchKernelGGL((k_part_hist<Fr>), dim3((unsigned)ptiles), dim3(256), nregions * 4, st, d_scalars, n, c, nwin, shared, nregions, tile_scalars, region_total);
         hipLaunchKernelGGL(k_part_region_scan, dim3(1), dim3(1024), 0, st, region_total, nregions, region_cursor, total_items);
         const bool staged = global_option(CG_GOPT_SORT_STAGING) != 0;
         if (staged && nregions <= STAGE_MAX_REGIONS) {
             static PerDeviceOnce attr_set;
             if (attr_set.pending()) {
-                HIPCHK(hipFuncSetAttribute((const void*)k_part_scatter_staged, hipFuncAttributeMaxDynamicSharedMemorySize, (int)part_staged_lds(STAGE_MAX_REGIONS)));
+                HIPCHK(hipFuncSetAttribute((const void*)k_part_scatter_staged<Fr>, hipFuncAttributeMaxDynamicSharedMemorySize, (int)part_staged_lds(STAGE_MAX_REGIONS)));
                 HIPCHK(hipFuncSetAttribute((const void*)k_items_scatter_staged, hipFuncAttributeMaxDynamicSharedMemorySize, (int)ITEMS_STAGED_LDS));
                 attr_set.mark();
             }
-            hipLaunchKernelGGL(k_part_scatter_staged, dim3((unsigned)ptiles), dim3(STAGE_THREADS), part_staged_lds(nregions), st, digits, n, c, nwin, shared, nregions, region_cursor, items);
+            hipLaunchKernelGGL((k_part_scatter_staged<Fr>), dim3((unsigned)ptiles), dim3(STAGE_THREADS), part_staged_lds(nregions), st, d_scalars, n, c, nwin, shared, nregions, tile_scalars, region_cursor, items);
         } else
-        hipLaunchKernelGGL(k_part_scatter, dim3((unsigned)ptiles), dim3(256), nregions * 4, st, digits, n, c, nwin, shared, nregions, region_cursor, items);
+        hipLaunchKernelGGL((k_part_scatter<Fr>), dim3((unsigned)ptiles), dim3(256), nregions * 4, st, d_scalars, n, c, nwin, shared, nregions, tile_scalars, region_cursor, items);
         hipLaunchKernelGGL(k_items_hist, dim3(itiles), dim3(256), 0, st, items, total_items, counts);
         hipLaunchKernelGGL(k_scan_tile_sums, dim3((unsigned)ntiles), dim3(256), 0, st, counts, tile_sums, nbuckets, 0xffffffffu);
         hipLaunchKernelGGL(k_scan_exclusive, dim3(1), dim3(1024), 0, st, tile_sums, tile_sums, ntiles);
diff --git a/collaborative-circom_amd/csrc/launchers.hpp b/collaborative-circom_amd/csrc/launchers.hpp
--- a/collaborative-circom_amd/csrc/launchers.hpp
+++ b/collaborative-circom_amd/csrc/launchers.hpp
@@ -23,7 +23,7 @@
 inline size_t msm_sort_scratch_bytes(size_t n, int c, int nwin) {
     const size_t nbuckets = (size_t)nwin << (c - 1);
     const size_t entries = (size_t)nwin * n;
-    return 2 * align_up(entries * 4) + 3 * align_up(nbuckets * 4) + align_up(((nbuckets + SCAN_TILE - 1) / SCAN_TILE) * 4) +
+    return align_up(entries * 4) + 3 * align_up(nbuckets * 4) + align_up(((nbuckets + SCAN_TILE - 1) / SCAN_TILE) * 4) +
            align_up(entries * 8) + 2 * align_up(PART_MAX_REGIONS * 4) + 256;
 }
 inline size_t msm_sort_direct_scratch_bytes(size_t n, int c, int nwin, int shared, uint32_t cap) {
diff --git a/collaborative-circom_amd/csrc/msm_impl.hpp b/collaborative-circom_amd/csrc/msm_impl.hpp
--- a/collaborative-circom_amd/csrc/msm_impl.hpp
+++ b/collaborative-circom_amd/csrc/msm_impl.hpp
@@ -45,7 +45,6 @@
 int msm_accumulate_batch(hipStream_t st, const MsmAccSet* sets, int nsets, size_t n, int c, int nwin, bool shared, uint32_t cap, hipEvent_t* evs, uint32_t chunk_request, bool g2_slices) {
     if (nsets < 1 || nsets > ACC_MAX_SETS) return fail(CG_ERR_ARG, "internal: accumulation batch size");
     const MsmGeom g = msm_geom_of<F>(n, c, nwin, shared, chunk_request);
-    typedef typename BucketOf<F>::type B;
     AccSets<F> S{};
     for (int i = 0; i < nsets; i++) {
         const AccScratch<F> sc(sets[i].scratch, g);
@@ -53,11 +52,10 @@
         S.buckets[i] = sc.buckets; S.cont[i] = sc.cont; S.cont_bucket[i] = sc.cont_bucket;
         S.table_stride[i] = (uint32_t)sets[i].table_stride; S.may_have_inf[i] = sets[i].may_have_inf ? 1u : 0u;
     }
-    const ptrdiff_t stride = nsets > 1 ? sets[1].scratch - sets[0].scratch : 0;
-    bool one_fill = stride > 0 && (size_t)(nsets - 1) * (size_t)stride + g.nbuckets * sizeof(B) <= ((size_t)8 << 20);
-    for (int i = 2; i < nsets && one_fill; i++) one_fill = sets[i].scratch - sets[i - 1].scratch == stride;
-    if (one_fill) HIPCHK(hipMemsetAsync(S.buckets[0], 0, (size_t)(nsets - 1) * (size_t)stride + g.nbuckets * sizeof(B), st));
-    else for (int i = 0; i < nsets; i++) HIPCHK(hipMemsetAsync(S.buckets[i], 0, g.nbuckets * sizeof(B), st));
+#ifdef CG_DEBUG_KNOBS
+    static const bool fill_sets = getenv("CG_DEBUG_NO_REDUCE") && atoi(getenv("CG_DEBUG_NO_REDUCE")) == 1;
+    if (fill_sets) for (int i = 0; i < nsets; i++) HIPCHK(hipMemsetAsync(S.buckets[i], 0, g.nbuckets * sizeof(typename BucketOf<F>::type), st));
+#endif
     if (evs) HIPCHK(hipEventRecord(evs[0], st));
     auto launch_acc = [&](auto kern, int T, size_t lds) -> int {
         if (lds > 0) { if (int rc = ensure_dynamic_lds((const void*)kern, lds)) return rc; }
diff --git a/collaborative-circom_amd/csrc/msm_kernels.hpp b/collaborative-circom_amd/csrc/msm_kernels.hpp
--- a/collaborative-circom_amd/csrc/msm_kernels.hpp
+++ b/collaborative-circom_amd/csrc/msm_kernels.hpp
@@ -357,7 +357,7 @@
     const uint32_t b = blockIdx.x * blockDim.x + threadIdx.x;
     if (b >= nbuckets) return;
     const uint32_t cnt = cap ? min(counts[b], cap) : counts[b];
-    if (cnt == 0) return;
+    if (cnt == 0) { st_struct(buckets + b, bk_inf<B>()); return; }
     const uint32_t first = offsets[b], last = first + cnt - 1;
     const uint32_t q0 = first / chunk_len + 1, q1 = last / chunk_len;
     if (q0 > q1 || q1 - q0 >= MERGE_DIRECT_MAX || q1 >= nchunks) return;
diff --git a/collaborative-circom_amd/csrc/msm_sort_kernels.hpp b/collaborative-circom_amd/csrc/msm_sort_kernels.hpp
--- a/collaborative-circom_amd/csrc/msm_sort_kernels.hpp
+++ b/collaborative-circom_amd/csrc/msm_sort_kernels.hpp
@@ -5,26 +5,32 @@
 
 namespace cg {
 
+template <class Fr, class Fn>
+__device__ __forceinline__ void msm_recode(Fr s, int c, int nwin, Fn&& f) {
+    const uint32_t nb = 1u << (c - 1);
+    const uint32_t mask = (1u << c) - 1;
+    uint32_t carry = 0;
+    for (int w = 0; w < nwin; w++) {
+        const uint32_t d = (s.v[0] & mask) + carry;
+        _Pragma("unroll") for (int l = 0; l < Fr::N; l++) {
+            const uint64_t two = ((uint64_t)(l + 1 < Fr::N ? s.v[l + 1] : 0u) << 32) | s.v[l];
+            s.v[l] = (uint32_t)(two >> c);
+        }
+        int32_t dig;
+        if (d > nb) { dig = (int32_t)d - (int32_t)(1u << c); carry = 1; } else { dig = (int32_t)d; carry = 0; }
+        f(w, dig);
+    }
+}
+
 template <class Fr>
 __global__ void __launch_bounds__(256) k_msm_digits(const Fr* __restrict__ scalars, size_t n, int c, int nwin, int shared,
                                                     int32_t* __restrict__ digits, uint32_t* __restrict__ counts) {
     const uint32_t nb = 1u << (c - 1);
-    const uint32_t mask = (1u << c) - 1;
-    for (size_t i = (size_t)blockIdx.x * blockDim.x + threadIdx.x; i < n; i += (size_t)gridDim.x * blockDim.x) {
-        Fr s = ld_fp(scalars + i).from_mont();
-        uint32_t carry = 0;
-        for (int w = 0; w < nwin; w++) {
-            uint32_t d = (s.v[0] & mask) + carry;
-            _Pragma("unroll") for (int l = 0; l < Fr::N; l++) {
-                uint64_t two = ((uint64_t)(l + 1 < Fr::N ? s.v[l + 1] : 0u) << 32) | s.v[l];
-                s.v[l] = (uint32_t)(two >> c);
-            }
-            int32_t dig;
-            if (d > nb) { dig = (int32_t)d - (int32_t)(1u << c); carry = 1; } else { dig = (int32_t)d; carry = 0; }
+    for (size_t i = (size_t)blockIdx.x * blockDim.x + threadIdx.x; i < n; i += (size_t)gridDim.x * blockDim.x)
+        msm_recode(ld_fp(scalars + i).from_mont(), c, nwin, [&](int w, int32_t dig) {
             digits[(size_t)w * n + i] = dig;
             if (dig != 0) atomicAdd(&counts[(shared ? 0 : (size_t)w * nb) + (uint32_t)(dig < 0 ? -dig : dig) - 1], 1u);
-        }
-    }
+        });
 }
 
 static __global__ void __launch_bounds__(256) k_scan_tile_sums(const uint32_t* __restrict__ in, uint32_t* __restrict__ tile_sums, size_t total, uint32_t cap) {
@@ -91,22 +97,12 @@
 __global__ void __launch_bounds__(1024) k_msm_sort_small(const Fr* __restrict__ scalars, uint32_t n, int c, int nwin,
                                                          uint32_t* __restrict__ counts, uint32_t* __restrict__ offsets, uint32_t* __restrict__ sorted) {
     extern __shared__ uint32_t sort_lds[];
-    const uint32_t nb = 1u << (c - 1), mask = (1u << c) - 1, t = threadIdx.x;
+    const uint32_t nb = 1u << (c - 1), t = threadIdx.x;
     uint32_t* cnt = sort_lds; uint32_t* cur = sort_lds + nb; uint32_t* part = sort_lds + 2 * nb;
     for (uint32_t b = t; b < nb; b += 1024) cnt[b] = 0;
     __syncthreads();
     auto digits_of = [&](uint32_t i, auto&& f) {
-        Fr s = ld_fp(scalars + i).from_mont();
-        uint32_t carry = 0;
-        for (int w = 0; w < nwin; w++) {
-            const uint32_t d = (s.v[0] & mask) + carry;
-            _Pragma("unroll") for (int l = 0; l < Fr::N; l++) {
-                const uint64_t two = ((uint64_t)(l + 1 < Fr::N ? s.v[l + 1] : 0u) << 32) | s.v[l];
-                s.v[l] = (uint32_t)(two >> c);
-            }
-            if (d > nb) { carry = 1; if (d != (1u << c)) f((uint32_t)w, (1u << c) - d - 1, true); }
-            else { carry = 0; if (d) f((uint32_t)w, d - 1, false); }
-        }
+        msm_recode(ld_fp(scalars + i).from_mont(), c, nwin, [&](int w, int32_t dig) { if (dig) f((uint32_t)w, (uint32_t)(dig < 0 ? -dig : dig) - 1, dig < 0); });
     };
     for (uint32_t i = t; i < n; i += 1024) digits_of(i, [&](uint32_t, uint32_t b, bool) { atomicAdd(&cnt[b], 1u); });
     __syncthreads();
@@ -135,37 +131,22 @@
     *payload = (shared ? ((uint32_t)w << 24) | i : i) | (dig < 0 ? 0x80000000u : 0u);
     return true;
 }
-template <class Fr>
-__global__ void __launch_bounds__(256) k_msm_digits_only(const Fr* __restrict__ scalars, size_t n, int c, int nwin, int32_t* __restrict__ digits) {
-    const uint32_t nb = 1u << (c - 1);
-    const uint32_t mask = (1u << c) - 1;
-    for (size_t i = (size_t)blockIdx.x * blockDim.x + threadIdx.x; i < n; i += (size_t)gridDim.x * blockDim.x) {
-        Fr s = ld_fp(scalars + i).from_mont();
-        uint32_t carry = 0;
-        for (int w = 0; w < nwin; w++) {
-            uint32_t d = (s.v[0] & mask) + carry;
-            _Pragma("unroll") for (int l = 0; l < Fr::N; l++) {
-                uint64_t two = ((uint64_t)(l + 1 < Fr::N ? s.v[l + 1] : 0u) << 32) | s.v[l];
-                s.v[l] = (uint32_t)(two >> c);
-            }
-            int32_t dig;
-            if (d > nb) { dig = (int32_t)d - (int32_t)(1u << c); carry = 1; } else { dig = (int32_t)d; carry = 0; }
-            digits[(size_t)w * n + i] = dig;
-        }
-    }
-}
-static __global__ void __launch_bounds__(256) k_part_hist(const int32_t* __restrict__ digits, size_t n, int c, int nwin, int shared, uint32_t nregions,
-                                                          uint32_t* __restrict__ region_total) {
+inline uint32_t part_tile_scalars(int nwin) { return (uint32_t)std::min<size_t>((size_t)PART_TILE / (size_t)nwin, 2048); }
+template <class Fr>
+__global__ void __launch_bounds__(256) k_part_hist(const Fr* __restrict__ scalars, size_t n, int c, int nwin, int shared, uint32_t nregions, uint32_t tile_scalars,
+                                                   uint32_t* __restrict__ region_total) {
     extern __shared__ uint32_t lds_cnt[];
     for (uint32_t r = threadIdx.x; r < nregions; r += 256) lds_cnt[r] = 0;
     __syncthreads();
     const uint32_t nb = 1u << (c - 1);
-    const size_t total = (size_t)nwin * n, base = (size_t)blockIdx.x * PART_TILE;
-    for (int k = 0; k < PART_TILE / 256; k++) {
-        const size_t idx = base + (size_t)k * 256 + threadIdx.x;
-        if (idx >= total) break;
-        const size_t w = idx / n; uint32_t bucket, payload;
-        if (part_decode(digits[idx], w, (uint32_t)(idx - w * n), nb, shared, &bucket, &payload)) atomicAdd(&lds_cnt[bucket >> PART_REGION_LOG], 1u);
+    const size_t base = (size_t)blockIdx.x * tile_scalars;
+    for (uint32_t k = threadIdx.x; k < tile_scalars; k += 256) {
+        const size_t i = base + k;
+        if (i >= n) break;
+        msm_recode(ld_fp(scalars + i).from_mont(), c, nwin, [&](int w, int32_t dig) {
+            uint32_t bucket, payload;
+            if (part_decode(dig, (size_t)w, (uint32_t)i, nb, shared, &bucket, &payload)) atomicAdd(&lds_cnt[bucket >> PART_REGION_LOG], 1u);
+        });
     }
     __syncthreads();
     for (uint32_t r = threadIdx.x; r < nregions; r += 256) { const uint32_t v = lds_cnt[r]; if (v) atomicAdd(&region_total[r], v); }
@@ -188,31 +169,29 @@
     if (threadIdx.x == 1023) *total_items = part[1023];
     for (uint32_t k = 0; k < per; k++) { const uint32_t r = threadIdx.x * per + k; if (r < nregions) { region_cursor[r] = run; run += v[k]; } }
 }
-static __global__ void __launch_bounds__(256) k_part_scatter(const int32_t* __restrict__ digits, size_t n, int c, int nwin, int shared, uint32_t nregions,
-                                                             uint32_t* __restrict__ region_cursor, uint64_t* __restrict__ items) {
+template <class Fr>
+__global__ void __launch_bounds__(256) k_part_scatter(const Fr* __restrict__ scalars, size_t n, int c, int nwin, int shared, uint32_t nregions, uint32_t tile_scalars,
+                                                      uint32_t* __restrict__ region_cursor, uint64_t* __restrict__ items) {
     extern __shared__ uint32_t lds_cnt[];
     for (uint32_t r = threadIdx.x; r < nregions; r += 256) lds_cnt[r] = 0;
     __syncthreads();
     const uint32_t nb = 1u << (c - 1);
-    const size_t total = (size_t)nwin * n, base = (size_t)blockIdx.x * PART_TILE;
-    for (int k = 0; k < PART_TILE / 256; k++) {
-        const size_t idx = base + (size_t)k * 256 + threadIdx.x;
-        if (idx >= total) break;
-        const size_t w = idx / n; uint32_t bucket, payload;
-        if (part_decode(digits[idx], w, (uint32_t)(idx - w * n), nb, shared, &bucket, &payload)) atomicAdd(&lds_cnt[bucket >> PART_REGION_LOG], 1u);
-    }
+    const size_t base = (size_t)blockIdx.x * tile_scalars;
+    auto entries = [&](auto&& f) {
+        for (uint32_t k = threadIdx.x; k < tile_scalars; k += 256) {
+            const size_t i = base + k;
+            if (i >= n) break;
+            msm_recode(ld_fp(scalars + i).from_mont(), c, nwin, [&](int w, int32_t dig) {
+                uint32_t bucket, payload;
+                if (part_decode(dig, (size_t)w, (uint32_t)i, nb, shared, &bucket, &payload)) f(bucket, payload);
+            });
+        }
+    };
+    entries([&](uint32_t bucket, uint32_t) { atomicAdd(&lds_cnt[bucket >> PART_REGION_LOG], 1u); });
     __syncthreads();
     for (uint32_t r = threadIdx.x; r < nregions; r += 256) { const uint32_t v = lds_cnt[r]; lds_cnt[r] = v ? atomicAdd(&region_cursor[r], v) : 0u; }
     __syncthreads();
-    for (int k = 0; k < PART_TILE / 256; k++) {
-        const size_t idx = base + (size_t)k * 256 + threadIdx.x;
-        if (idx >= total) break;
-        const size_t w = idx / n; uint32_t bucket, payload;
-        if (part_decode(digits[idx], w, (uint32_t)(idx - w * n), nb, shared, &bucket, &payload)) {
-            const uint32_t pos = atomicAdd(&lds_cnt[bucket >> PART_REGION_LOG], 1u);
-            items[pos] = ((uint64_t)bucket << 32) | payload;
-        }
-    }
+    entries([&](uint32_t bucket, uint32_t payload) { items[atomicAdd(&lds_cnt[bucket >> PART_REGION_LOG], 1u)] = ((uint64_t)bucket << 32) | payload; });
 }
 constexpr int ITEM_TILE = 16384;
 constexpr uint32_t ITEM_WINDOW = 2048;
@@ -286,8 +265,9 @@
     __syncthreads();
     return r;
 }
-static __global__ void __launch_bounds__(STAGE_THREADS) k_part_scatter_staged(const int32_t* __restrict__ digits, size_t n, int c, int nwin, int shared, uint32_t nregions,
-                                                                            uint32_t* __restrict__ region_cursor, uint64_t* __restrict__ items) {
+template <class Fr>
+__global__ void __launch_bounds__(STAGE_THREADS) k_part_scatter_staged(const Fr* __restrict__ scalars, size_t n, int c, int nwin, int shared, uint32_t nregions, uint32_t tile_scalars,
+                                                                     uint32_t* __restrict__ region_cursor, uint64_t* __restrict__ items) {
     extern __shared__ uint32_t lds_u32[];
     uint32_t* cnt = lds_u32;
     uint32_t* delta = cnt + nregions;
@@ -295,21 +275,25 @@
     uint64_t* stage = reinterpret_cast<uint64_t*>(scratch + 32);
     for (uint32_t r = threadIdx.x; r < nregions; r += STAGE_THREADS) cnt[r] = 0;
     const uint32_t nb = 1u << (c - 1);
-    const size_t total = (size_t)nwin * n, base = (size_t)blockIdx.x * PART_TILE;
-    int32_t dig[STAGE_PER_LANE];
-    _Pragma("unroll") for (int k = 0; k < STAGE_PER_LANE; k++) {
-        const size_t idx = base + (size_t)k * STAGE_THREADS + threadIdx.x;
-        dig[k] = idx < total ? digits[idx] : 0;
-    }
-    __syncthreads();
-    uint32_t bucket[STAGE_PER_LANE], payload[STAGE_PER_LANE], rank[STAGE_PER_LANE];
-    _Pragma("unroll") for (int k = 0; k < STAGE_PER_LANE; k++) {
-        const size_t idx = base + (size_t)k * STAGE_THREADS + threadIdx.x;
-        const size_t w = idx / n;
-        bucket[k] = 0xffffffffu; payload[k] = 0; rank[k] = 0;
-        if (part_decode(dig[k], w, (uint32_t)(idx - w * n), nb, shared, &bucket[k], &payload[k])) rank[k] = atomicAdd(&cnt[bucket[k] >> PART_REGION_LOG], 1u);
-        else bucket[k] = 0xffffffffu;
-    }
+    const size_t base = (size_t)blockIdx.x * tile_scalars;
+    Fr s[2];
+    _Pragma("unroll") for (int k = 0; k < 2; k++) {
+        const uint32_t ls = (uint32_t)k * STAGE_THREADS + threadIdx.x;
+        const bool have = ls < tile_scalars && base + ls < n;
+        s[k] = ld_fp(scalars + (have ? base + ls : 0)).from_mont();
+        if (!have) { _Pragma("unroll") for (int l = 0; l < Fr::N; l++) s[k].v[l] = 0; }
+    }
+    __syncthreads();
+    auto entries = [&](auto&& f) {
+        _Pragma("unroll") for (int k = 0; k < 2; k++) {
+            const uint32_t i = (uint32_t)(base + (uint32_t)k * STAGE_THREADS + threadIdx.x);
+            msm_recode(s[k], c, nwin, [&](int w, int32_t dig) {
+                uint32_t bucket, payload;
+                if (part_decode(dig, (size_t)w, i, nb, shared, &bucket, &payload)) f(bucket, payload);
+            });
+        }
+    };
+    entries([&](uint32_t bucket, uint32_t) { atomicAdd(&cnt[bucket >> PART_REGION_LOG], 1u); });
     __syncthreads();
     const uint32_t per = (nregions + STAGE_THREADS - 1) / STAGE_THREADS;
     uint32_t v[2] = {0, 0}, mine = 0;
@@ -321,12 +305,11 @@
         if (r < nregions) { cnt[r] = run; delta[r] = (v[j] ? atomicAdd(&region_cursor[r], v[j]) : 0u) - run; run += v[j]; }
     }
     __syncthreads();
-    _Pragma("unroll") for (int k = 0; k < STAGE_PER_LANE; k++)
-        if (bucket[k] != 0xffffffffu) stage[cnt[bucket[k] >> PART_REGION_LOG] + rank[k]] = ((uint64_t)bucket[k] << 32) | payload[k];
-    __syncthreads();
-    for (uint32_t s = threadIdx.x; s < tile_items; s += STAGE_THREADS) {
-        const uint64_t it = stage[s];
-        items[delta[(uint32_t)(it >> 32) >> PART_REGION_LOG] + s] = it;
+    entries([&](uint32_t bucket, uint32_t payload) { stage[atomicAdd(&cnt[bucket >> PART_REGION_LOG], 1u)] = ((uint64_t)bucket << 32) | payload; });
+    __syncthreads();
+    for (uint32_t s_at = threadIdx.x; s_at < tile_items; s_at += STAGE_THREADS) {
+        const uint64_t it = stage[s_at];
+        items[delta[(uint32_t)(it >> 32) >> PART_REGION_LOG] + s_at] = it;
     }
 }
 static __global__ void __launch_bounds__(STAGE_THREADS) k_items_scatter_staged(const uint64_t* __restrict__ items, const uint32_t* __restrict__ total_items,
@@ -381,25 +364,14 @@
 __global__ void __launch_bounds__(256) k_msm_scatter_direct(const Fr* __restrict__ scalars, size_t n, int c, int nwin, int shared, uint32_t cap,
                                                             uint32_t* __restrict__ counts, uint32_t* __restrict__ sorted, uint32_t* __restrict__ overflow) {
     const uint32_t nb = 1u << (c - 1);
-    const uint32_t mask = (1u << c) - 1;
-    for (size_t i = (size_t)blockIdx.x * blockDim.x + threadIdx.x; i < n; i += (size_t)gridDim.x * blockDim.x) {
-        Fr s = ld_fp(scalars + i).from_mont();
-        uint32_t carry = 0;
-        for (int w = 0; w < nwin; w++) {
-            uint32_t d = (s.v[0] & mask) + carry;
-            _Pragma("unroll") for (int l = 0; l < Fr::N; l++) {
-                uint64_t two = ((uint64_t)(l + 1 < Fr::N ? s.v[l + 1] : 0u) << 32) | s.v[l];
-                s.v[l] = (uint32_t)(two >> c);
-            }
-            int32_t dig;
-            if (d > nb) { dig = (int32_t)d - (int32_t)(1u << c); carry = 1; } else { dig = (int32_t)d; carry = 0; }
-            if (dig == 0) continue;
+    for (size_t i = (size_t)blockIdx.x * blockDim.x + threadIdx.x; i < n; i += (size_t)gridDim.x * blockDim.x)
+        msm_recode(ld_fp(scalars + i).from_mont(), c, nwin, [&](int w, int32_t dig) {
+            if (dig == 0) return;
             const size_t bucket = (shared ? 0 : (size_t)w * nb) + (uint32_t)(dig < 0 ? -dig : dig) - 1;
             const uint32_t pos = atomicAdd(&counts[bucket], 1u);
             if (pos < cap) sorted[bucket * cap + pos] = (shared ? ((uint32_t)w << 24) | (uint32_t)i : (uint32_t)i) | (dig < 0 ? 0x80000000u : 0u);
             else *overflow = 1u;
-        }
-    }
-}
-
-}
+        });
+}
+
+}
```

Result: slower. 59.18 million constraints/s (-3.9%).
